# Icelk/fractal-renderer

Hardware: AMD Instinct MI355X
Metric: pixel_iterations_per_sec (higher is better)
Workload: dtype f64

## Files before the change

fractal-renderer_amd/_native.py:

```python
import ctypes as C
import os

PKG_DIR = os.path.dirname(os.path.abspath(__file__))
LIB_PATH = os.path.join(PKG_DIR, "libfractal_hip.so")

FR_OK, FR_ERR_INVALID_ARGUMENT, FR_ERR_BUFFER_TOO_SMALL, FR_ERR_NO_DEVICE, FR_ERR_HIP = 0, 1, 2, 3, 4
STATUS_NAMES = {
    1: "FR_ERR_INVALID_ARGUMENT",
    2: "FR_ERR_BUFFER_TOO_SMALL",
    3: "FR_ERR_NO_DEVICE",
    4: "FR_ERR_HIP",
    5: "FR_ERR_UNSUPPORTED_ALGO",
}


class FractalHipError(RuntimeError):
    def __init__(self, code, message):
        super().__init__("%s: %s" % (STATUS_NAMES.get(code, "fr_status %d" % code), message))
        self.code = code


class Imaginary(C.Structure):

    _fields_ = [("re", C.c_double), ("im", C.c_double)]
# ... 30 lines not shown
        ("limit", C.c_double),
        ("stable_limit", C.c_double),
        ("pos", Imaginary),
        ("scale", Imaginary),
        ("exposure", C.c_double),
        ("inside", C.c_uint8),
        ("smooth", C.c_uint8),
        ("primary_color", RGB),
        ("secondary_color", RGB),
        ("color_weight", C.c_double),
        ("julia_set", Imaginary),
    ]


class fr_render_opts(C.Structure):

    _fields_ = [
        ("size", C.c_uint32),
        ("tile", C.c_int32),
        ("loop_mode", C.c_int32),
        ("palette", C.c_int32),
        ("cycle_shortcut", C.c_int32),
        ("refill_minrun", C.c_int32),
        ("refill_quit16", C.c_int32),
        ("colour_filter", C.c_int32),
    ]


FR_MAX_DEVICES = 16
FR_GATHER_PEER_COPY, FR_GATHER_RCCL = 0, 1


class fr_multi_stats(C.Structure):
    _fields_ = [
        ("n_devices", C.c_uint32),
        ("kernels", C.c_uint32 * FR_MAX_DEVICES),
        ("kernel_ms", C.c_float * FR_MAX_DEVICES),
        ("rows", C.c_uint64 * FR_MAX_DEVICES),
        ("wall_ms", C.c_double),
        ("transfer_span_ms", C.c_float * FR_MAX_DEVICES),
        ("job_ms", C.c_double * FR_MAX_DEVICES),
        ("bytes_moved", C.c_uint64 * FR_MAX_DEVICES),
    ]


class fr_wide_centre(C.Structure):

    _fields_ = [("n_words", C.c_uint32), ("re", C.POINTER(C.c_uint64)), ("im", C.POINTER(C.c_uint64))]


FR_WIDE_MAX_WORDS = 16
FR_BLA_DEFAULT_BITS = 40
_OPTS = C.POINTER(fr_render_opts)
_WIDE = C.POINTER(fr_wide_centre)

PROTOTYPES = {
    "fr_abi_version": (C.c_int, []),
    "fr_build_id": (C.c_char_p, []),
    "fr_render_opts_init": (None, [_OPTS]),
    "fr_render_rows_rgb8_device_opts": (
        C.c_int,
        [C.POINTER(fr_config), C.c_int, C.c_uint32, C.c_uint32, C.c_void_p, C.c_size_t, C.c_void_p, _OPTS],
    ),
    "fr_render_rows_rgba8_device_opts": (
        C.c_int,
        [C.POINTER(fr_config), C.c_int, C.c_uint32, C.c_uint32, C.c_void_p, C.c_size_t, C.c_void_p, _OPTS],
    ),
    "fr_render_rows_rgb8_opts": (
        C.c_int, [C.POINTER(fr_config), C.c_int, C.c_uint32, C.c_uint32, C.c_void_p, C.c_size_t, _OPTS]),
    "fr_render_block_cyclic_range_rgb8_device_opts": (
        C.c_int,
        [C.POINTER(fr_config), C.c_int, C.c_uint32, C.c_uint32, C.c_uint32, C.c_uint32, C.c_int, C.c_void_p, C.c_size_t,
         C.c_void_p, C.POINTER(C.c_uint64), _OPTS],
    ),
    "fr_render_fern_rgb8": (C.c_int, [C.POINTER(fr_config), C.c_uint32, C.c_uint64, C.c_uint32, C.c_void_p, C.c_size_t]),
    "fr_init_devices": (C.c_int, [C.POINTER(C.c_int), C.c_int]),
    "fr_multi_device_count": (C.c_int, [C.POINTER(C.c_int)]),
    "fr_set_multi_root_share": (C.c_int, [C.c_int]),
    "fr_render_rgb8_multi": (C.c_int, [C.POINTER(fr_config), C.c_int, C.c_uint32, C.c_void_p, C.c_size_t]),
    "fr_render_rgb8_multi_device": (
        C.c_int, [C.POINTER(fr_config), C.c_int, C.c_uint32, C.c_int, C.c_void_p, C.c_size_t]),
    "fr_multi_last_stats": (C.c_int, [C.POINTER(fr_multi_stats)]),
    "fr_debug_rccl_selftest": (C.c_int, [C.c_size_t]),
    "fr_debug_rccl_probe": (C.c_int, []),
    "fr_set_dispatch_sampling": (C.c_int, [C.c_int]),
    "fr_debug_sample_view": (C.c_int, [C.POINTER(fr_config), C.c_int, C.POINTER(C.c_double)]),
    "fr_debug_view_choice": (C.c_int, [C.POINTER(fr_config), C.c_int, C.c_uint32, C.c_uint32, C.POINTER(C.c_int),
                                       C.POINTER(C.c_int), C.POINTER(C.c_uint32)]),
    "fr_debug_inject_multi_failure": (C.c_int, [C.c_int, C.c_int]),
    "fr_pin_host_buffer": (C.c_int, [C.c_void_p, C.c_size_t]),
    "fr_unpin_host_buffer": (C.c_int, [C.c_void_p]),
    "fr_last_kernel_name": (C.c_int, [C.c_char_p, C.c_size_t]),
    "fr_set_colour_filter": (C.c_int, [C.c_int]),
    "fr_init": (C.c_int, [C.c_int]),
    "fr_shutdown": (C.c_int, []),
    "fr_device_count": (C.c_int, [C.POINTER(C.c_int)]),
    "fr_device_name": (C.c_int, [C.c_char_p, C.c_size_t]),
    "fr_last_error": (C.c_char_p, []),
    "fr_config_new": (None, [C.POINTER(fr_config), C.c_uint32]),
    "fr_render_rgb8": (C.c_int, [C.POINTER(fr_config), C.c_void_p, C.c_size_t]),
    "fr_render_rows_rgb8": (C.c_int, [C.POINTER(fr_config), C.c_int, C.c_uint32, C.c_uint32, C.c_void_p, C.c_size_t]),
    "fr_render_rows_rgb8_device": (
        C.c_int,
        [C.POINTER(fr_config), C.c_int, C.c_uint32, C.c_uint32, C.c_void_p, C.c_size_t, C.c_void_p],
    ),
    "fr_render_rows_rgba8": (C.c_int, [C.POINTER(fr_config), C.c_int, C.c_uint32, C.c_uint32, C.c_void_p, C.c_size_t]),
    "fr_render_rows_rgba8_device": (
        C.c_int,
        [C.POINTER(fr_config), C.c_int, C.c_uint32, C.c_uint32, C.c_void_p, C.c_size_t, C.c_void_p],
    ),
    "fr_render_block_cyclic_rgb8_device": (
        C.c_int,
        [C.POINTER(fr_config), C.c_int, C.c_uint32, C.c_uint32, C.c_uint32, C.c_void_p, C.c_size_t, C.c_void_p,
         C.POINTER(C.c_uint64)],
    ),
    "fr_render_block_cyclic_range_rgb8_device": (
        C.c_int,
        [C.POINTER(fr_config), C.c_int, C.c_uint32, C.c_uint32, C.c_uint32, C.c_uint32, C.c_int, C.c_void_p, C.c_size_t,
         C.c_void_p, C.POINTER(C.c_uint64)],
    ),
    "fr_render_block_cyclic_rgb8": (
        C.c_int,
        [C.POINTER(fr_config), C.c_int, C.c_uint32, C.c_uint32, C.c_uint32, C.c_void_p, C.c_size_t,
         C.POINTER(C.c_uint64)],
    ),
    "fr_block_cyclic_rows": (C.c_uint64, [C.c_uint32, C.c_uint32, C.c_uint32, C.c_uint32]),
    "fr_pixel": (C.c_int, [C.POINTER(fr_config), C.c_uint32, C.c_uint32, C.POINTER(RGB)]),
    "fr_pixel_p": (C.c_int, [C.POINTER(fr_config), C.c_int, C.c_uint32, C.c_uint32, C.POINTER(RGB)]),
    "fr_recursive": (
        C.c_int,
        [C.c_uint32, Imaginary, Imaginary, C.c_double, C.POINTER(Imaginary), C.POINTER(C.c_uint32)],
    ),
    "fr_recursive_batch": (
        C.c_int,
        [C.c_uint32, C.c_void_p, C.c_void_p, C.c_size_t, C.c_double, C.c_int, C.c_void_p, C.c_void_p],
    ),
    "fr_escape_rows": (C.c_int, [C.POINTER(fr_config), C.c_int, C.c_uint32, C.c_uint32, C.c_void_p, C.c_void_p]),
    "fr_render_rows_dd": (
        C.c_int, [C.POINTER(fr_config), C.POINTER(Imaginary), C.c_uint32, C.c_uint32, C.c_int, C.c_void_p, C.c_size_t]),
    "fr_render_rows_dd_device": (
        C.c_int,
        [C.POINTER(fr_config), C.POINTER(Imaginary), C.c_uint32, C.c_uint32, C.c_int, C.c_void_p, C.c_size_t, C.c_void_p],
    ),
    "fr_escape_rows_dd": (
        C.c_int, [C.POINTER(fr_config), C.POINTER(Imaginary), C.c_uint32, C.c_uint32, C.c_void_p, C.c_void_p]),
    "fr_render_rows_pt": (
        C.c_int, [C.POINTER(fr_config), C.POINTER(Imaginary), C.c_uint32, C.c_uint32, C.c_int, C.c_void_p, C.c_size_t]),
    "fr_render_rows_pt_device": (
        C.c_int,
        [C.POINTER(fr_config), C.POINTER(Imaginary), C.c_uint32, C.c_uint32, C.c_int, C.c_void_p, C.c_size_t, C.c_void_p],
    ),
    "fr_escape_rows_pt": (
        C.c_int, [C.POINTER(fr_config), C.POINTER(Imaginary), C.c_uint32, C.c_uint32, C.c_void_p, C.c_void_p]),
    "fr_debug_reference_orbit": (
        C.c_int, [C.POINTER(fr_config), C.POINTER(Imaginary), C.c_int, C.c_void_p, C.c_size_t, C.POINTER(C.c_uint32)]),
    "fr_ss_workspace_bytes": (
        C.c_int, [C.POINTER(fr_config), C.c_uint32, C.c_uint32, C.c_uint32, C.POINTER(C.c_size_t), C.POINTER(C.c_size_t)]),
    "fr_render_rows_ss_device": (
        C.c_int,
        [C.POINTER(fr_config), C.c_int, C.POINTER(Imaginary), C.c_uint32, C.c_uint32, C.c_uint32, C.c_int, C.c_void_p,
         C.c_size_t, C.c_void_p, C.c_size_t, C.c_void_p, _OPTS],
    ),
    "fr_render_rows_ss": (
        C.c_int,
        [C.POINTER(fr_config), C.c_int, C.POINTER(Imaginary), C.c_uint32, C.c_uint32, C.c_uint32, C.c_int, C.c_void_p,
         C.c_size_t, _OPTS],
    ),
    "fr_box_filter_rgb8": (
        C.c_int, [C.c_void_p, C.c_uint32, C.c_uint32, C.c_uint32, C.c_int, C.c_void_p, C.c_size_t]),
    "fr_box_filter_rgb8_device": (
        C.c_int, [C.c_void_p, C.c_uint32, C.c_uint32, C.c_uint32, C.c_int, C.c_void_p, C.c_size_t, C.c_void_p]),
    "fr_colour_rgb8": (C.c_int, [C.POINTER(fr_config), C.c_void_p, C.c_void_p, C.c_size_t, C.c_void_p, C.c_size_t]),
    "fr_colour_rgb8_device": (
        C.c_int, [C.POINTER(fr_config), C.c_void_p, C.c_void_p, C.c_size_t, C.c_void_p, C.c_size_t, C.c_void_p]),
    "fr_escape_rows_device": (
        C.c_int,
        [C.POINTER(fr_config), C.c_int, C.POINTER(Imaginary), C.c_uint32, C.c_uint32, C.c_int, C.c_void_p, C.c_void_p,
         C.c_void_p, _OPTS],
    ),
    "fr_escape_extend_device": (
        C.c_int,
        [C.POINTER(fr_config), C.c_int, C.POINTER(Imaginary), C.c_uint32, C.c_uint32, C.c_uint32, C.c_int, C.c_void_p,
         C.c_void_p, C.c_void_p, _OPTS],
    ),
    "fr_escape_extend": (
        C.c_int,
        [C.POINTER(fr_config), C.c_int, C.POINTER(Imaginary), C.c_uint32, C.c_uint32, C.c_uint32, C.c_int, C.c_void_p,
         C.c_void_p],
    ),
    "fr_escape_rows_pt_state_device": (
        C.c_int,
        [C.POINTER(fr_config), C.POINTER(Imaginary), C.c_uint32, C.c_uint32, C.c_void_p, C.c_void_p, C.c_void_p, C.c_void_p,
         C.c_void_p],
    ),
    "fr_escape_extend_pt_device": (
        C.c_int,
        [C.POINTER(fr_config), C.POINTER(Imaginary), C.c_uint32, C.c_uint32, C.c_uint32, C.c_void_p, C.c_void_p, C.c_void_p,
         C.c_void_p, C.c_void_p],
    ),
    "fr_escape_rows_pt_state": (
        C.c_int,
        [C.POINTER(fr_config), C.POINTER(Imaginary), C.c_uint32, C.c_uint32, C.c_void_p, C.c_void_p, C.c_void_p, C.c_void_p],
    ),
    "fr_escape_extend_pt": (
        C.c_int,
        [C.POINTER(fr_config), C.POINTER(Imaginary), C.c_uint32, C.c_uint32, C.c_uint32, C.c_void_p, C.c_void_p, C.c_void_p,
         C.c_void_p],
    ),
    "fr_debug_pt_orbit_cache": (C.c_int, [C.POINTER(C.c_uint32)]),
    "fr_wide_from_double": (C.c_int, [C.c_double, C.c_void_p, C.c_uint32]),
    "fr_wide_add_double": (C.c_int, [C.c_void_p, C.c_uint32, C.c_double]),
    "fr_wide_to_double": (C.c_int, [C.c_void_p, C.c_uint32, C.POINTER(C.c_double), C.POINTER(C.c_double)]),
    "fr_wide_from_decimal": (C.c_int, [C.c_char_p, C.c_void_p, C.c_uint32]),
    "fr_render_rows_pt_wide": (
        C.c_int, [C.POINTER(fr_config), _WIDE, C.c_uint32, C.c_uint32, C.c_int, C.c_void_p, C.c_size_t]),
    "fr_render_rows_pt_wide_device": (
        C.c_int, [C.POINTER(fr_config), _WIDE, C.c_uint32, C.c_uint32, C.c_int, C.c_void_p, C.c_size_t, C.c_void_p]),
    "fr_escape_rows_pt_wide": (C.c_int, [C.POINTER(fr_config), _WIDE, C.c_uint32, C.c_uint32, C.c_void_p, C.c_void_p]),
    "fr_escape_rows_pt_wide_state_device": (
        C.c_int,
        [C.POINTER(fr_config), _WIDE, C.c_uint32, C.c_uint32, C.c_void_p, C.c_void_p, C.c_void_p, C.c_void_p, C.c_void_p],
    ),
    "fr_escape_extend_pt_wide_device": (
        C.c_int,
        [C.POINTER(fr_config), _WIDE, C.c_uint32, C.c_uint32, C.c_uint32, C.c_void_p, C.c_void_p, C.c_void_p, C.c_void_p,
         C.c_void_p],
    ),
    "fr_escape_rows_pt_wide_state": (
        C.c_int, [C.POINTER(fr_config), _WIDE, C.c_uint32, C.c_uint32, C.c_void_p, C.c_void_p, C.c_void_p, C.c_void_p]),
    "fr_escape_extend_pt_wide": (
        C.c_int,
        [C.POINTER(fr_config), _WIDE, C.c_uint32, C.c_uint32, C.c_uint32, C.c_void_p, C.c_void_p, C.c_void_p, C.c_void_p],
    ),
    "fr_debug_reference_orbit_wide": (
        C.c_int, [C.POINTER(fr_config), _WIDE, C.c_int, C.c_void_p, C.c_size_t, C.POINTER(C.c_uint32)]),
    "fr_render_rows_pt_bla": (
        C.c_int,
        [C.POINTER(fr_config), C.POINTER(Imaginary), _WIDE, C.c_int, C.c_uint32, C.c_uint32, C.c_int, C.c_void_p, C.c_size_t]),
    "fr_render_rows_pt_bla_device": (
        C.c_int,
        [C.POINTER(fr_config), C.POINTER(Imaginary), _WIDE, C.c_int, C.c_uint32, C.c_uint32, C.c_int, C.c_void_p, C.c_size_t,
         C.c_void_p],
    ),
    "fr_escape_rows_pt_bla": (
        C.c_int, [C.POINTER(fr_config), C.POINTER(Imaginary), _WIDE, C.c_int, C.c_uint32, C.c_uint32, C.c_void_p, C.c_void_p]),
    "fr_escape_rows_pt_bla_device": (
        C.c_int,
        [C.POINTER(fr_config), C.POINTER(Imaginary), _WIDE, C.c_int, C.c_uint32, C.c_uint32, C.c_void_p, C.c_void_p, C.c_void_p],
    ),
    "fr_debug_bla_table": (
        C.c_int,
        [C.POINTER(fr_config), C.POINTER(Imaginary), _WIDE, C.c_int, C.c_int, C.c_uint32, C.c_void_p, C.c_size_t,
         C.POINTER(C.c_uint32)],
    ),
    "fr_debug_bla_count": (
        C.c_int,
        [C.POINTER(fr_config), C.POINTER(Imaginary), _WIDE, C.c_int, C.c_uint32, C.c_uint32, C.POINTER(C.c_uint64),
         C.POINTER(C.c_uint64)],
    ),
    "fr_debug_bla_cache": (C.c_int, [C.POINTER(C.c_uint32)]),
    "fr_render_rows_pt_scaled": (
        C.c_int, [C.POINTER(fr_config), _WIDE, C.c_int, C.c_uint32, C.c_uint32, C.c_int, C.c_void_p, C.c_size_t]),
    "fr_render_rows_pt_scaled_device": (
        C.c_int, [C.POINTER(fr_config), _WIDE, C.c_int, C.c_uint32, C.c_uint32, C.c_int, C.c_void_p, C.c_size_t, C.c_void_p]),
    "fr_escape_rows_pt_scaled": (C.c_int, [C.POINTER(fr_config), _WIDE, C.c_int, C.c_uint32, C.c_uint32, C.c_void_p, C.c_void_p]),
    "fr_escape_rows_pt_scaled_device": (
        C.c_int, [C.POINTER(fr_config), _WIDE, C.c_int, C.c_uint32, C.c_uint32, C.c_void_p, C.c_void_p, C.c_void_p]),
    "fr_debug_bla_table_scaled": (
        C.c_int, [C.POINTER(fr_config), _WIDE, C.c_int, C.c_int, C.c_uint32, C.c_void_p, C.c_size_t, C.POINTER(C.c_uint32)]),
    "fr_debug_pt_scaled_count": (
        C.c_int, [C.POINTER(fr_config), _WIDE, C.c_int, C.c_uint32, C.c_uint32, C.POINTER(C.c_uint64), C.POINTER(C.c_uint64)]),
    "fr_escape_rows_pt_scaled_state_device": (
        C.c_int,
        [C.POINTER(fr_config), _WIDE, C.c_uint32, C.c_uint32, C.c_void_p, C.c_void_p, C.c_void_p, C.c_void_p, C.c_void_p],
    ),
    "fr_escape_extend_pt_scaled_device": (
        C.c_int,
        [C.POINTER(fr_config), _WIDE, C.c_uint32, C.c_uint32, C.c_uint32, C.c_void_p, C.c_void_p, C.c_void_p, C.c_void_p,
         C.c_void_p],
    ),
    "fr_escape_rows_pt_scaled_state": (
        C.c_int, [C.POINTER(fr_config), _WIDE, C.c_uint32, C.c_uint32, C.c_void_p, C.c_void_p, C.c_void_p, C.c_void_p]),
    "fr_escape_extend_pt_scaled": (
        C.c_int,
        [C.POINTER(fr_config), _WIDE, C.c_uint32, C.c_uint32, C.c_uint32, C.c_void_p, C.c_void_p, C.c_void_p, C.c_void_p],
    ),
    "fr_colour_rows_device": (
        C.c_int,
        [C.POINTER(fr_config), C.c_void_p, C.c_int, C.c_void_p, C.c_size_t, C.c_int, C.c_void_p, C.c_size_t, C.c_void_p],
    ),
    "fr_count_iterations": (
        C.c_int,
        [C.POINTER(fr_config), C.c_int, C.c_uint32, C.c_uint32, C.c_uint32, C.c_uint32, C.POINTER(C.c_uint64),
         C.POINTER(C.c_uint64)],
    ),
    "fr_set_profiling": (C.c_int, [C.c_int]),
    "fr_last_kernel_ms": (C.c_int, [C.POINTER(C.c_float)]),
    "fr_set_tile": (C.c_int, [C.c_int]),
    "fr_set_loop_mode": (C.c_int, [C.c_int]),
    "fr_debug_loop_plan": (C.c_int, [C.POINTER(fr_config), C.c_int, C.POINTER(C.c_uint32), C.POINTER(C.c_double),
                                     C.POINTER(C.c_uint32)]),
    "fr_debug_set_spec_maxlen": (C.c_int, [C.c_uint32]),
    "fr_debug_spec_maxlen": (C.c_int, [C.POINTER(fr_config), C.c_int, C.POINTER(C.c_uint32)]),
    "fr_set_palette": (C.c_int, [C.c_int]),
    "fr_set_cycle_shortcut": (C.c_int, [C.c_int]),
    "fr_set_refill_policy": (C.c_int, [C.c_int, C.c_int]),
    "fr_debug_math": (C.c_int, [C.c_int, C.c_void_p, C.c_void_p, C.c_size_t]),
    "fr_debug_set_queue_trace": (C.c_int, [C.c_void_p]),
    "fr_debug_set_two_pass_capacity": (C.c_int, [C.c_uint32]),
}

_lib = None


def load():
    global _lib
    if _lib is not None:
        return _lib
    if not os.path.exists(LIB_PATH):
        raise ImportError(
            "%s is missing — build it first (python -c 'import __graft_entry__ as g; g.build()'); "
            "this package has no CPU fallback" % LIB_PATH
        )
    lib = C.CDLL(LIB_PATH)
    for name, (restype, argtypes) in PROTOTYPES.items():
        fn = getattr(lib, name)
        fn.restype = restype
        fn.argtypes = argtypes
    _lib = lib
    return lib


def check(rc):
    if rc != FR_OK:
        msg = load().fr_last_error()
        raise FractalHipError(rc, msg.decode() if msg else "")
```

fractal-renderer_amd/build.py:

```python
import hashlib
import os
import shutil
import subprocess

PKG_DIR = os.path.dirname(os.path.abspath(__file__))
CSRC = os.path.join(PKG_DIR, "csrc")
LIB_PATH = os.path.join(PKG_DIR, "libfractal_hip.so")
ID_PATH = LIB_PATH + ".id"
KERNEL_SOURCES = ["fr_kernels.hip", "fr_bla.hip", "fr_scaled.hip"]
SOURCES = KERNEL_SOURCES + ["fr_dispatch.hip", "fr_api.hip", "fr_host.hip", "fr_multi.hip", "fr_fern.hip",
                            "fr_dd.hip", "fr_pt.hip", "fr_wide.hip", "fr_ss.hip"]
DEPS = SOURCES + ["fr_kernels.h", "fr_launch.h", "fr_ctx.h", "fr_wide.h", "fr_bla.h", "fr_math.h", "fr_colour.h", "fr_log2_table.inc",
                  os.path.join("..", "..", "include", "fractal_hip.h")]
HIPCC_FLAGS = [
    "--offload-arch=gfx950",
    "-O3",
    "-std=c++17",
    "-ffp-contract=off",
    "-fno-fast-math",
    "-fPIC",
    "-shared",
    "-Wall",
    "-Wextra",
    "-pthread",
]
LINK_FLAGS = ["-ldl"]


def find_hipcc():
    for cand in (os.environ.get("HIPCC"), "/opt/rocm/bin/hipcc", shutil.which("hipcc")):
        if cand and os.path.exists(cand):
            return cand
    raise RuntimeError("hipcc not found (set HIPCC or install ROCm under /opt/rocm)")


def source_id():
    h = hashlib.sha256()
    h.update(" ".join(HIPCC_FLAGS + LINK_FLAGS).encode())
    for d in DEPS:
        h.update(d.encode())
        with open(os.path.join(CSRC, d), "rb") as f:
            h.update(f.read())
    return h.hexdigest()[:16]


def built_id():
    try:
        with open(ID_PATH) as f:
            return f.read().strip()
    except OSError:
        return None


def is_stale():
    return not os.path.exists(LIB_PATH) or built_id() != source_id()


def build_extension(force=False, verbose=False):
    if not force and not is_stale():
        return LIB_PATH
    sid = source_id()
    cmd = ([find_hipcc()] + HIPCC_FLAGS + ['-DFR_BUILD_ID="%s"' % sid, "-o", LIB_PATH]
           + [os.path.join(CSRC, s) for s in SOURCES] + LINK_FLAGS)
    if verbose:
        print(" ".join(cmd))
    if os.path.exists(ID_PATH):
        os.remove(ID_PATH)
    subprocess.run(cmd, check=True, cwd=CSRC)
    with open(ID_PATH, "w") as f:
        f.write(sid + "\n")
    return LIB_PATH


if __name__ == "__main__":
    print(build_extension(force=True, verbose=True))
```

fractal-renderer_amd/csrc/fr_api.hip:

```cpp
#include <hip/hip_runtime.h>

#include <atomic>
#include <cmath>
#include <cstddef>
#include <cstdint>
#include <cstdio>
#include <cstdlib>
#include <cstring>
#include <mutex>
#include <shared_mutex>
#include <string>
#include <vector>

#include "fr_ctx.h"

static_assert(sizeof(fr_config) == 104 && offsetof(fr_config, limit) == 16 && offsetof(fr_config, inside) == 72 &&
                  offsetof(fr_config, primary_color) == 74 && offsetof(fr_config, color_weight) == 80 &&
                  offsetof(fr_config, julia_set) == 88,
              "fr_config must stay the #[repr(C)] image of calc::Config");
static_assert(sizeof(fr_render_opts) == 32, "fr_render_opts is part of the ABI");

namespace fr {

namespace {
// ... 1453 lines not shown
                         uint32_t from_iterations, double *d_z, uint32_t *d_iters, hipStream_t stream) {
    const Centre c{pos_lo, nullptr};
    fr_kparams p;
    rows_params(cfg, o, y0, y1, 0, p);
    int rc = prof_begin(stream);
    if (rc != FR_OK) return rc;
    const char *kname = "";
    if (precision == FR_PRECISION_DD) {
        HIP_TRY(fr_launch_escape_extend_dd(p, c.lo_re(), c.lo_im(), from_iterations, d_z, d_iters, stream, &kname));
    } else {
        plan_loop(cfg, precision, o, p);
        HIP_TRY(fr_launch_escape_extend(p, precision, from_iterations, d_z, d_iters, stream, &kname));
    }
    return prof_end(stream, kname);
}

int fr_escape_extend_device(const fr_config *cfg, int precision, const fr_imaginary *pos_lo, uint32_t y0, uint32_t y1,
                            uint32_t from_iterations, int z_width, void *d_z, void *d_iters, void *hip_stream,
                            const fr_render_opts *opts) {
    Opts o;
    bool work;
    int rc = check_extend(cfg, precision, pos_lo, y0, y1, from_iterations, z_width, d_z, d_iters, opts, o, &work);
    if (rc != FR_OK || !work) return rc;
    LifeShared ls;
    Ctx *ctx;
    rc = primary(&ctx);
    if (rc != FR_OK) return rc;
    return extend_launch(cfg, precision, pos_lo, o, y0, y1, from_iterations, static_cast<double *>(d_z),
                         static_cast<uint32_t *>(d_iters), static_cast<hipStream_t>(hip_stream));
}

int fr_escape_extend(const fr_config *cfg, int precision, const fr_imaginary *pos_lo, uint32_t y0, uint32_t y1,
                     uint32_t from_iterations, int z_width, double *z, uint32_t *iters) {
    Opts o;
    bool work;
    int rc = check_extend(cfg, precision, pos_lo, y0, y1, from_iterations, z_width, z, iters, nullptr, o, &work);
    if (rc != FR_OK || !work) return rc;
    const size_t npx = (size_t)cfg->width * (size_t)(y1 - y0);
    const size_t zb = npx * (size_t)z_width * sizeof(double), ib = npx * sizeof(uint32_t);
    return host_raw(z, zb, iters, ib, nullptr, nullptr, true, [&](Ctx &, double *d_z, uint32_t *d_iters, double *, uint32_t *, hipStream_t stream) {
        return extend_launch(cfg, precision, pos_lo, o, y0, y1, from_iterations, d_z, d_iters, stream);
    });
}

int fr_colour_rows_device(const fr_config *cfg, const void *d_z, int z_width, const void *d_iters, size_t n, int channels,
                          void *d_out, size_t out_len, void *hip_stream) {
    if (!cfg) return fail(FR_ERR_INVALID_ARGUMENT, "cfg is NULL");
    if (z_width != 2 && z_width != 4) return fail(FR_ERR_INVALID_ARGUMENT, "z_width must be 2 (re, im) or 4 (re.hi, re.lo, im.hi, im.lo)");
    const int rc = check_channels(channels);
    if (rc != FR_OK) return rc;
    if (n == 0) return FR_OK;
    if (!d_z || !d_iters || !d_out) return fail(FR_ERR_INVALID_ARGUMENT, "NULL array");
    if (n > SIZE_MAX / 4 || out_len < (size_t)channels * n) return fail(FR_ERR_BUFFER_TOO_SMALL, "out_len < channels*n");
    if ((reinterpret_cast<uintptr_t>(d_z) & 7u) || (reinterpret_cast<uintptr_t>(d_iters) & 3u))
        return fail(FR_ERR_INVALID_ARGUMENT, "d_z must be 8-byte aligned and d_iters 4-byte aligned");
    if (channels == 4 && (reinterpret_cast<uintptr_t>(d_out) & 3u))
        return fail(FR_ERR_INVALID_ARGUMENT, "RGBA8 output must be 4-byte aligned");
    fr_kparams p;
    fill_params(cfg, default_opts(), p);
    HIP_TRY(fr_launch_colour_rows(p, static_cast<const double *>(d_z), (uint32_t)z_width, static_cast<const uint32_t *>(d_iters), n,
                                  (uint32_t)channels, d_out, static_cast<hipStream_t>(hip_stream)));
    return FR_OK;
}

int fr_colour_rgb8(const fr_config *cfg, const double *z_re_im, const uint32_t *iters, size_t n, uint8_t *out,
                   size_t out_len) {
    if (!cfg) return fail(FR_ERR_INVALID_ARGUMENT, "cfg is NULL");
    if (n == 0) return FR_OK;
    if (!z_re_im || !iters || !out) return fail(FR_ERR_INVALID_ARGUMENT, "NULL array");
    if (out_len < 3 * n) return fail(FR_ERR_BUFFER_TOO_SMALL, "out_len < 3*n");
    LifeShared ls;
    Ctx *ctx;
    int rc = primary(&ctx);
    if (rc != FR_OK) return rc;
    std::lock_guard<std::mutex> lk(ctx->mu);
    rc = ctx->reserve(ctx->z, n * 2 * sizeof(double));
    if (rc == FR_OK) rc = ctx->reserve(ctx->iters, n * sizeof(uint32_t));
    if (rc == FR_OK) rc = ctx->reserve(ctx->rgb, 3 * n);
    if (rc != FR_OK) return rc;
    fr_kparams p;
    fill_params(cfg, default_opts(), p);
    HIP_TRY(hipMemcpyAsync(ctx->z.ptr, z_re_im, n * 2 * sizeof(double), hipMemcpyHostToDevice, ctx->stream));
    HIP_TRY(hipMemcpyAsync(ctx->iters.ptr, iters, n * sizeof(uint32_t), hipMemcpyHostToDevice, ctx->stream));
    HIP_TRY(fr_launch_colour(p, static_cast<const double *>(ctx->z.ptr), static_cast<const uint32_t *>(ctx->iters.ptr), n,
                             static_cast<uint8_t *>(ctx->rgb.ptr), ctx->stream));
    HIP_TRY(hipMemcpyAsync(out, ctx->rgb.ptr, 3 * n, hipMemcpyDeviceToHost, ctx->stream));
    HIP_TRY(hipStreamSynchronize(ctx->stream));
    return FR_OK;
}

int fr_colour_rgb8_device(const fr_config *cfg, const void *d_z_re_im, const void *d_iters, size_t n, void *d_out,
                          size_t out_len, void *hip_stream) {
    if (!cfg) return fail(FR_ERR_INVALID_ARGUMENT, "cfg is NULL");
    if (n == 0) return FR_OK;
    if (!d_z_re_im || !d_iters || !d_out) return fail(FR_ERR_INVALID_ARGUMENT, "NULL array");
    if (out_len < 3 * n) return fail(FR_ERR_BUFFER_TOO_SMALL, "out_len < 3*n");
    fr_kparams p;
    fill_params(cfg, default_opts(), p);
    HIP_TRY(fr_launch_colour(p, static_cast<const double *>(d_z_re_im), static_cast<const uint32_t *>(d_iters), n,
                             static_cast<uint8_t *>(d_out), static_cast<hipStream_t>(hip_stream)));
    return FR_OK;
}

int fr_count_iterations(const fr_config *cfg, int precision, uint32_t y0, uint32_t y1, uint32_t sx, uint32_t sy,
                        uint64_t *total, uint64_t *pixels) {
    int rc = check_rows(cfg, y0, y1);
    if (rc == FR_OK) rc = check_precision_or_deep(cfg, precision);
    if (rc != FR_OK) return rc;
    if (!total) return fail(FR_ERR_INVALID_ARGUMENT, "total is NULL");
    if (sx == 0) sx = 1;
    if (sy == 0) sy = 1;
    *total = 0;
    const Opts o = default_opts();
    fr_kparams p;
    fill_params(cfg, o, p);
    p.ncols = (uint32_t)(((uint64_t)cfg->width + sx - 1) / sx);
    p.x_stride = sx;
    const uint64_t yf = ((uint64_t)y0 + sy - 1) / sy * sy;
    p.nrows = yf < y1 ? (uint32_t)((y1 - 1 - yf) / sy + 1) : 0;
    p.y_first = (uint32_t)yf;
    p.block_rows = 1;
    p.y_stride = sy;
    if (pixels) *pixels = (uint64_t)p.ncols * p.nrows;
    if (p.ncols == 0 || p.nrows == 0) return FR_OK;
    LifeShared ls;
    Ctx *ctx;
    rc = primary(&ctx);
    if (rc != FR_OK) return rc;
    std::lock_guard<std::mutex> lk(ctx->mu);
    const size_t slot_bytes = sizeof(unsigned long long) * FR_COUNT_SLOTS;
    rc = ctx->reserve(ctx->misc, slot_bytes);
    if (rc != FR_OK) return rc;
    HIP_TRY(hipMemsetAsync(ctx->misc.ptr, 0, slot_bytes, ctx->stream));
    fr_kout ko{};
    ko.count = static_cast<unsigned long long *>(ctx->misc.ptr);
    if (precision == FR_PRECISION_DD) {
        HIP_TRY(fr_launch_escape_dd(p, 0.0, 0.0, FR_OUT_COUNT, ko, false, ctx->stream, nullptr));
    } else if (precision == FR_PRECISION_PT) {
        rc = launch_pt(*ctx, cfg, Centre{}, p, FR_OUT_COUNT, ko, ctx->stream, nullptr);
        if (rc != FR_OK) return rc;
    } else {
        plan_loop(cfg, precision, o, p);
        HIP_TRY(fr_launch_escape(p, precision, FR_OUT_COUNT, ko, o.tile, ctx->stream, nullptr));
    }
    std::vector<unsigned long long> host(FR_COUNT_SLOTS);
    HIP_TRY(hipMemcpyAsync(host.data(), ctx->misc.ptr, slot_bytes, hipMemcpyDeviceToHost, ctx->stream));
    HIP_TRY(hipStreamSynchronize(ctx->stream));
    unsigned long long sum = 0;
    for (unsigned long long v : host) sum += v;
    *total = sum;
    return FR_OK;
}

int fr_set_profiling(int enabled) {
    Profiling &pr = profiling();
    pr.enabled = enabled != 0;
    if (!enabled) {
        pr.have = false;
        if (pr.e0) {
            (void)hipEventDestroy(pr.e0);
            (void)hipEventDestroy(pr.e1);
            pr.e0 = pr.e1 = nullptr;
        }
    }
    return FR_OK;
}

int fr_last_kernel_ms(float *ms) {
    if (!ms) return fail(FR_ERR_INVALID_ARGUMENT, "ms is NULL");
    Profiling &pr = profiling();
    if (!pr.have) return fail(FR_ERR_INVALID_ARGUMENT, "no profiled kernel on this thread");
    HIP_TRY(hipEventSynchronize(pr.e1));
    HIP_TRY(hipEventElapsedTime(ms, pr.e0, pr.e1));
    return FR_OK;
}

int fr_last_kernel_name(char *buf, size_t buf_len) {
    if (!buf || buf_len == 0) return fail(FR_ERR_INVALID_ARGUMENT, "buf is NULL or empty");
    Profiling &pr = profiling();
    if (!pr.have) return fail(FR_ERR_INVALID_ARGUMENT, "no profiled kernel on this thread");
    snprintf(buf, buf_len, "%s", pr.kernel);
    return FR_OK;
}

int fr_set_tile(int tile) {
    if (!valid_tile(tile)) return fail(FR_ERR_INVALID_ARGUMENT, "tile must be 0, 1, 2, 4, 8, 9, 10 ... 16, 6401, 3202, 1604 or 808");
    g_tile.store(tile);
    return FR_OK;
}

int fr_set_refill_policy(int minrun, int quit16) {
    if (minrun < -1 || quit16 < -1 || quit16 == 0 || quit16 > 16)
        return fail(FR_ERR_INVALID_ARGUMENT, "minrun >= 0, 1 <= quit16 <= 16 (or -1: the kernel's default)");
    g_refill_minrun.store(minrun);
    g_refill_quit16.store(quit16);
    return FR_OK;
}

int fr_set_cycle_shortcut(int enabled) {
    g_cycle_shortcut.store(enabled ? 1 : 0);
    return FR_OK;
}

int fr_set_palette(int enabled) {
    g_palette_enabled.store(enabled ? 1 : 0);
    return FR_OK;
}

int fr_set_colour_filter(int enabled) {
    g_colour_filter.store(enabled == 2 ? 2 : enabled ? 1 : 0);
    return FR_OK;
}

int fr_set_loop_mode(int mode) {
    if (mode != -1 && mode != 0 && mode != 2 && mode != 4 && mode != 5)
        return fail(FR_ERR_INVALID_ARGUMENT, "loop mode must be -1 (auto), 0, 2, 4 or 5");
    g_loop_mode.store(mode);
    return FR_OK;
}

int fr_set_dispatch_sampling(int enabled) {
    g_dispatch_sampling.store(enabled ? 1 : 0);
    return FR_OK;
}

int fr_debug_sample_view(const fr_config *cfg, int precision, double out[8]) {
    if (!cfg || !out) return fail(FR_ERR_INVALID_ARGUMENT, "cfg or out is NULL");
    int rc = check_precision(precision);
    if (rc != FR_OK) return rc;
    LifeShared ls;
    Ctx *ctx;
    rc = primary(&ctx);
    if (rc != FR_OK) return rc;
    fr_kparams p;
    rows_params(cfg, default_opts(), 0, cfg->height, 0, p);
    if (p.ncols == 0 || p.nrows == 0) return fail(FR_ERR_INVALID_ARGUMENT, "empty image");
    double st[7];
    rc = sample_view(*ctx, p, precision, Ctx::kViewChoices, st);
    if (rc != FR_OK) return rc;
    for (int k = 0; k < 6; k++) out[k] = st[k];
    out[6] = st[1] > 0.0 ? st[0] / st[1] : 0.0;
    out[7] = st[6];
    return FR_OK;
}

int fr_debug_loop_plan(const fr_config *cfg, int precision, uint32_t *loop_mode, double *skip_t, uint32_t *spec_quiet) {
    if (!cfg || !loop_mode || !skip_t || !spec_quiet) return fail(FR_ERR_INVALID_ARGUMENT, "NULL argument");
    int rc = check_precision(precision);
    if (rc != FR_OK) return rc;
    const Opts o = default_opts();
    fr_kparams p;
    rows_params(cfg, o, 0, cfg->height, 0, p);
    plan_loop(cfg, precision, o, p);
    *loop_mode = p.loop_mode;
    *skip_t = p.skip_t;
    *spec_quiet = p.loop_spec;
    return FR_OK;
}

int fr_debug_view_choice(const fr_config *cfg, int precision, uint32_t y0, uint32_t y1, int *state, int *choice,
                         uint32_t *strip_tiles) {
    if (!cfg || !state || !choice || !strip_tiles) return fail(FR_ERR_INVALID_ARGUMENT, "NULL argument");
    int rc = check_rows(cfg, y0, y1);
    if (rc == FR_OK) rc = check_precision(precision);
    if (rc != FR_OK) return rc;
    LifeShared ls;
    Ctx *ctx;
    rc = primary(&ctx);
    if (rc != FR_OK) return rc;
    fr_kparams p;
    rows_params(cfg, default_opts(), y0, y1, 0, p);
    const uint64_t key = view_key(cfg, p, precision);
    *state = 0, *choice = -1, *strip_tiles = 0;
    std::lock_guard<std::mutex> lk(ctx->sample_mu);
    for (int k = 0; k < Ctx::kViewChoices; k++) {
        const Ctx::ViewChoice &v = ctx->view_choices[k];
        if (v.key != key || v.state == 0) continue;
        *state = v.state;
        if (v.state == 1 && __atomic_load_n(ctx->sample_result + 8 * k + 7, __ATOMIC_ACQUIRE) == key) *state = 3;
        *choice = v.two_pass;
        *strip_tiles = v.strip_tiles;
        break;
    }
    return FR_OK;
}

int fr_debug_set_spec_maxlen(uint32_t maxlen) {
    g_spec_maxlen.store(maxlen);
    return FR_OK;
}

int fr_debug_spec_maxlen(const fr_config *cfg, int precision, uint32_t *maxlen) {
    if (!cfg || !maxlen) return fail(FR_ERR_INVALID_ARGUMENT, "NULL argument");
    int rc = check_precision(precision);
    if (rc != FR_OK) return rc;
    const Opts o = default_opts();
    fr_kparams p;
    rows_params(cfg, o, 0, cfg->height, 0, p);
    plan_loop(cfg, precision, o, p);
    *maxlen = p.loop_spec_max;
    return FR_OK;
}

int fr_debug_set_queue_trace(void *d_trace) {
    g_queue_trace.store(static_cast<unsigned long long *>(d_trace));
    return FR_OK;
}

int fr_debug_set_two_pass_capacity(uint32_t entries_per_list) {
    g_two_pass_list_entries.store(entries_per_list);
    return FR_OK;
}

int fr_debug_math(int which, const double *in, double *out, size_t n) {
    if (n == 0) return FR_OK;
    if (!in || !out) return fail(FR_ERR_INVALID_ARGUMENT, "NULL array");
    LifeShared ls;
    Ctx *ctx;
    int rc = primary(&ctx);
    if (rc != FR_OK) return rc;
    std::lock_guard<std::mutex> lk(ctx->mu);
    rc = ctx->reserve(ctx->z, 2 * n * sizeof(double));
    if (rc != FR_OK) return rc;
    double *d_in = static_cast<double *>(ctx->z.ptr), *d_out = d_in + n;
    if (which == 4) {
        if (n < 2) return fail(FR_ERR_INVALID_ARGUMENT, "which == 4 needs n >= 2");
        HIP_TRY(fr_launch_nu_scan((uint32_t)in[0], (uint32_t)in[1], d_out, ctx->stream));
        HIP_TRY(hipMemcpyAsync(out, d_out, sizeof(double), hipMemcpyDeviceToHost, ctx->stream));
        HIP_TRY(hipStreamSynchronize(ctx->stream));
        return FR_OK;
    }
    if (which == 6) {
        if (n < 2) return fail(FR_ERR_INVALID_ARGUMENT, "which == 6 needs n >= 2");
        HIP_TRY(fr_launch_cast_scan((uint32_t)in[0], (uint32_t)in[1], d_out, ctx->stream));
        unsigned long long bad = 0;
        HIP_TRY(hipMemcpyAsync(&bad, d_out, sizeof bad, hipMemcpyDeviceToHost, ctx->stream));
        HIP_TRY(hipStreamSynchronize(ctx->stream));
        out[0] = (double)bad;
        return FR_OK;
    }
    HIP_TRY(hipMemcpyAsync(d_in, in, n * sizeof(double), hipMemcpyHostToDevice, ctx->stream));
    HIP_TRY(fr_launch_math_probe(which, d_in, d_out, n, ctx->stream));
    HIP_TRY(hipMemcpyAsync(out, d_out, n * sizeof(double), hipMemcpyDeviceToHost, ctx->stream));
    HIP_TRY(hipStreamSynchronize(ctx->stream));
    return FR_OK;
}

}
```

fractal-renderer_amd/csrc/fr_dispatch.hip:

```cpp
#include "fr_kernels.h"

#include <cmath>

#include "fr_launch.h"

namespace {

#define FR_KNAME(base, k) (precision == 1 ? base "<float, " k ">" : base "<double, " k ">")

const char *first_pass_name(const fr_kparams &p, int precision) {
    const bool spec = fr_first_pass_speculates(p);
#define FR_FIRST_NAMES(SUFFIX)                                                                                                       \
    (p.strip_tiles == 4                                                                                                              \
         ? (p.first_only ? FR_KNAME("escape_first_kernel", "4-tile strips in episodes, every tile finished in place" SUFFIX)         \
                         : FR_KNAME("escape_first_kernel + escape_second_kernel",                                                    \
                                    "4-tile strips, then persistent waves over the survivor lists" SUFFIX))                          \
         : (p.first_only ? FR_KNAME("escape_first_kernel", "7-tile strips in episodes, every tile finished in place" SUFFIX)         \
                         : FR_KNAME("escape_first_kernel + escape_second_kernel",                                                    \
                                    "7-tile strips, then persistent waves over the survivor lists" SUFFIX)))
    return spec ? FR_FIRST_NAMES("; speculative blocks in the later episodes") : FR_FIRST_NAMES("");
#undef FR_FIRST_NAMES
}

bool two_pass_ready(const fr_kparams &p, int mode) {
    return mode == FR_OUT_RGB && p.first_cap != 0 && (p.first_only || (p.surv_counts && p.work_counter));
}

hipError_t run_two_pass(const fr_kparams &p, int precision, int tile, const fr_kout &out, hipStream_t stream, const char *&name) {
    name = tile == 12   ? FR_KNAME("escape_first_v1_kernel + escape_queue_kernel", "round 2's first pass, then persistent waves over the survivor lists")
           : tile == 14 ? FR_KNAME("escape_first_kernel + escape_queue_kernel", "7-tile strips, then round 2's persistent waves over the survivor lists")
                        : first_pass_name(p, precision);
    if (p.ncols == 0 || p.nrows == 0) return hipSuccess;
    const hipError_t e = fr_launch_first_pass(p, precision, tile == 12, out, stream);
    if (e != hipSuccess) return e;
    if (p.first_only) return hipSuccess;
    if (p.debug_ablate & 2u) return hipSuccess;
    return fr_launch_queue(p, precision, 1, out, stream);
}

hipError_t run_strips(const fr_kparams &p, int precision, int mode, uint32_t k_len, const fr_kout &out, hipStream_t stream,
                      const char *&name) {
    const int k = k_len >= 7u ? 7 : k_len >= 4u ? 4 : k_len >= 2u ? 2 : 1;
    name = k == 7   ? FR_KNAME("escape_strip_kernel", "7 tiles")
           : k == 4 ? FR_KNAME("escape_strip_kernel", "4 tiles")
           : k == 2 ? FR_KNAME("escape_strip_kernel", "2 tiles")
                    : FR_KNAME("escape_strip_kernel", "1 tile");
    return fr_launch_strips(p, precision, mode, k, out, stream);
}

hipError_t run_refill(const fr_kparams &p, int precision, int mode, const fr_kout &out, hipStream_t stream, const char *&name) {
    name = FR_KNAME("escape_refill_kernel", "7x2-tile patches");
    return fr_launch_refill(p, precision, mode, out, stream);
}

hipError_t run_refill_or_strips(const fr_kparams &p, int precision, int mode, const fr_kout &out, hipStream_t stream,
                                const char *&name) {
    if (p.algo != 0 && p.algo != 2) return run_strips(p, precision, mode, 7u, out, stream, name);
    return run_refill(p, precision, mode, out, stream, name);
}

hipError_t launch_precision(const fr_kparams &p, int precision, int mode, const fr_kout &out, int tile, hipStream_t stream,
                            const char *&name) {
    if (p.out_in_place && tile > 16) tile = 0;
    switch (tile) {
    case 6401:
    case 3202:
    case 1604:
    case 808:
        name = tile == 6401   ? FR_KNAME("escape_kernel", "64x1")
               : tile == 3202 ? FR_KNAME("escape_kernel", "32x2")
               : tile == 1604 ? FR_KNAME("escape_kernel", "16x4")
                              : FR_KNAME("escape_kernel", "8x8");
        return fr_launch_tile(p, precision, mode, tile, out, stream);
    case 0: {
        const uint64_t tiles = (((uint64_t)p.ncols + 7) / 8) * (((uint64_t)p.nrows + 7) / 8);
        if (two_pass_ready(p, mode)) return run_two_pass(p, precision, 0, out, stream, name);
        if (tiles >= 262144 && ((p.algo == 2 && mode != FR_OUT_RGB) || p.cycle_shortcut)) return run_refill(p, precision, mode, out, stream, name);
        const uint32_t k_len = (mode == FR_OUT_RGB && p.strip_tiles) ? p.strip_tiles : tiles >= 524288 ? 7u : 1u;
        return run_strips(p, precision, mode, k_len, out, stream, name);
    }
    case 1:
    case 2:
    case 4:
    case 8:
        return run_strips(p, precision, mode, (uint32_t)tile, out, stream, name);
    case 13:
    case 16:
    case 12:
    case 14:
    case 15:
    case 11:
        if (two_pass_ready(p, mode)) return run_two_pass(p, precision, tile, out, stream, name);
        return run_refill_or_strips(p, precision, mode, out, stream, name);
    case 10:
        if (mode == FR_OUT_RGB && p.work_counter && fr_wants_work_queue(p, 10)) {
            name = FR_KNAME("escape_queue_kernel", "persistent waves, 64x32-px patches");
            return fr_launch_queue(p, precision, 0, out, stream);
        }
        [[fallthrough]];
    case 9:
        return run_refill_or_strips(p, precision, mode, out, stream, name);
    default:
        return hipErrorInvalidValue;
    }
}

}

hipError_t fr_launch_escape(const fr_kparams &p, int precision, int mode, const fr_kout &out, int tile,
                            hipStream_t stream, const char **kernel_name) {
    const char *name = "";
    const hipError_t e = launch_precision(p, precision, mode, out, tile, stream, name);
    if (kernel_name) *kernel_name = name;
    return e;
}

bool fr_wants_work_queue(const fr_kparams &p, int tile) {
    if (p.cycle_shortcut || (p.algo != 0 && p.algo != 2)) return false;
    if (p.loop_mode == 0 || p.iterations >= (1u << 24)) return false;
    return tile == 10;
}

bool fr_wants_two_pass(fr_kparams &p, int precision, int tile, int hint) {
    p.first_cap = 0;
    p.first_only = 0;
    if (p.cycle_shortcut || (p.algo != 0 && p.algo != 2)) return false;
    if (p.loop_mode == 0 || p.iterations >= (1u << 24)) return false;
    if (p.ncols == 0 || p.nrows == 0 || (uint64_t)p.ncols * p.nrows > 0xFFF00000ull) return false;
    if (p.algo == 2 && tile == 0) {
        const double lo = precision == 1 ? 0x1p-30 : 0x1p-300, hi = precision == 1 ? 0x1p30 : 0x1p400;
        const double jr = precision == 1 ? std::fabs((double)(float)p.julia_re) : std::fabs(p.julia_re);
        const double ji = precision == 1 ? std::fabs((double)(float)p.julia_im) : std::fabs(p.julia_im);
        if (!(jr >= lo && jr <= hi && ji >= lo && ji <= hi)) return false;
    }
    if (tile == 0) {
        const uint64_t tiles = (((uint64_t)p.ncols + 7) / 8) * (((uint64_t)p.nrows + 7) / 8);
        if (tiles < 262144 && hint < 1) return false;
        if (tiles < 4096) return false;
        if (hint == 0 || (hint < 0 && p.algo != 2)) return false;
        if (hint < 0 && p.iterations < 512u) return false;
        p.first_only = hint == 2 ? 1u : 0u;
    } else if (tile == 13 || tile == 16) {
        p.first_only = 1u;
    } else if (tile != 11 && tile != 12 && tile != 14 && tile != 15) {
        return false;
    }
    if (tile == 15 || tile == 16) p.strip_tiles = 4u;
    uint32_t k1 = p.two_pass_cap ? p.two_pass_cap : 64u;
    k1 = (k1 + 3u) & ~3u;
    if (k1 + 8u > p.iterations) return false;
    p.first_cap = k1;
    if (p.first_keep == 0 || p.first_keep > 64) p.first_keep = 48;
    return true;
}

fr_two_pass_layout fr_two_pass_bytes(const fr_kparams &p, int precision, uint32_t sub_capacity) {
    const size_t entries = (size_t)sub_capacity * FR_SURV_QUEUES;
    const size_t pair = precision == 1 ? 8 : 16;
    auto up = [](size_t v) { return (v + 255) & ~(size_t)255; };
    fr_two_pass_layout l{};
    l.z_off = 0;
    l.pos_off = up(entries * pair);
    l.cnt_off = l.pos_off + up(entries * 8);
    l.c_off = l.cnt_off + up(entries * 4);
    l.counts_off = l.c_off + (p.algo == 2 ? 0 : up(entries * pair));
    l.total = l.counts_off + FR_SURV_QUEUES * FR_SURV_COUNT_STRIDE * sizeof(uint32_t);
    return l;
}
```

fractal-renderer_amd/csrc/fr_kernels.h:

```cpp
#ifndef FR_KERNELS_H
#define FR_KERNELS_H

#include <hip/hip_runtime.h>
#include <stdint.h>

struct fr_kparams {
    uint32_t algo;
    uint32_t width, height;
    uint32_t iterations;
    double limit, stable_limit;
    double pos_re, pos_im, scale_re, scale_im;
    double exposure;
    double julia_re, julia_im;
    uint32_t inside, smooth;
    uint32_t prim[3], sec[3];
    double prim_f[3], sec_f[3];
    double iterations_f64, inv_iterations;
    uint32_t ncols, nrows;
    uint32_t x_first, x_stride;
    uint32_t block_rows, y_first, y_stride;
    uint32_t out_in_place;
    uint32_t out_rgba;
    uint32_t loop_mode;
    double skip_t;
    uint32_t loop_spec;
    uint32_t loop_spec_max;
    uint32_t first_no_spec;
    const uint32_t *palette;
    uint32_t palette_entries;
    uint32_t refill_minrun, refill_quit16;
    uint32_t queue_minrun, queue_want;
    uint32_t cycle_shortcut;
    uint32_t colour_filter;
    uint32_t *work_counter;
    double filt_k;
    double filt_d[3];
    uint32_t colour_filter32;
    float filt_k32;
    float filt_c32;
    float filt_d32[3];
    float prim32[3];
    float filt_lo32;
    uint32_t first_cap;
    uint32_t first_keep;
    uint32_t two_pass_cap;
    uint32_t first_only;
    uint32_t second_v1;
    uint32_t first_one_band;
    uint32_t strip_tiles;
    uint32_t debug_ablate;
    uint32_t surv_sub_capacity;
    void *surv_z;
    uint32_t *surv_pos;
    uint32_t *surv_cnt;
    void *surv_c;
    uint32_t *surv_counts;
};

constexpr uint32_t FR_SURV_QUEUES = 64;
constexpr uint32_t FR_SURV_COUNT_STRIDE = 32;
constexpr uint32_t FR_SURV_CHUNK = 64;

constexpr double FR_NU_BRACKET = 0x1p-18;

enum fr_out_mode {
    FR_OUT_RGB = 0,
    FR_OUT_ESCAPE = 1,
    FR_OUT_COUNT = 2
};

constexpr uint32_t FR_COUNT_SLOTS = 512;

struct fr_kout {
    uint8_t *rgb;
    double *z;
    uint32_t *iters;
    unsigned long long *count;
    unsigned long long *trace;
};

hipError_t fr_launch_escape(const fr_kparams &p, int precision, int mode, const fr_kout &out, int tile,
                            hipStream_t stream, const char **kernel_name);

hipError_t fr_launch_escape_dd(const fr_kparams &p, double pos_lo_re, double pos_lo_im, int mode, const fr_kout &out,
                               bool with_lo, hipStream_t stream, const char **kernel_name);

bool fr_wants_work_queue(const fr_kparams &p, int tile);

bool fr_wants_two_pass(fr_kparams &p, int precision, int tile, int hint = -1);
struct fr_two_pass_layout {
    size_t z_off, pos_off, cnt_off, c_off, counts_off, total;
};
fr_two_pass_layout fr_two_pass_bytes(const fr_kparams &p, int precision, uint32_t sub_capacity);

hipError_t fr_launch_view_sample(const fr_kparams &p, int precision, uint32_t side, uint32_t cap_s, uint32_t episode, uint32_t keep,
                                 unsigned long long *counters, unsigned long long *result, unsigned long long tag,
                                 hipStream_t stream);

hipError_t fr_launch_copy_out(const void *src, void *dst, size_t bytes, unsigned int *counter, unsigned long long *flag,
                              unsigned long long seq, hipStream_t stream);

constexpr uint32_t FR_MAX_PALETTE_ENTRIES = 1280;

hipError_t fr_launch_palette(const fr_kparams &p, uint32_t *palette, hipStream_t stream);

hipError_t fr_launch_colour(const fr_kparams &p, const double *z, const uint32_t *iters, size_t n, uint8_t *rgb,
                            hipStream_t stream);

hipError_t fr_launch_escape_extend(const fr_kparams &p, int precision, uint32_t from_iterations, double *z, uint32_t *iters,
                                   hipStream_t stream, const char **kernel_name);
hipError_t fr_launch_escape_extend_dd(const fr_kparams &p, double pos_lo_re, double pos_lo_im, uint32_t from_iterations,
                                      double *z, uint32_t *iters, hipStream_t stream, const char **kernel_name);

hipError_t fr_launch_colour_rows(const fr_kparams &p, const double *z, uint32_t z_width, const uint32_t *iters, size_t n,
                                 uint32_t channels, void *out, hipStream_t stream);

hipError_t fr_launch_box_filter(const void *src, uint32_t width, uint64_t rows, uint32_t s, uint32_t bpp, void *dst,
                                hipStream_t stream);

hipError_t fr_launch_recursive_batch(uint32_t iterations, const double *start, const double *c, size_t n,
                                     double limit, int precision, double *out_pos, uint32_t *out_iters,
                                     hipStream_t stream);

hipError_t fr_launch_math_probe(int which, const double *in, double *out, size_t n, hipStream_t stream);

hipError_t fr_launch_nu_scan(uint32_t lo_bits, uint32_t hi_bits, double *out, hipStream_t stream);

hipError_t fr_launch_cast_scan(uint32_t lo_bits, uint32_t hi_bits, double *out, hipStream_t stream);

#endif
```

fractal-renderer_amd/csrc/fr_kernels.hip:

```cpp
#include "fr_kernels.h"

#include <cmath>

#include <cstdlib>

#include "fr_launch.h"
#include "fr_math.h"

namespace {

#include "fr_colour.h"

constexpr int kWaves = 4;



#define FR_ORBIT_IT_R(SFX, S, D)                           \
    "v_add_" SFX " %[t], %[r2" S "], -%[i2" S "]\n"        \
    "v_add_" SFX " %[x], %[re" S "], %[re" S "]\n"         \
    "v_add_" SFX " %[re" D "], %[t], %[cre]\n"             \
    "v_mul_" SFX " %[x], %[x], %[im" S "]\n"               \
    "v_add_" SFX " %[im" D "], %[x], %[cim]\n"             \
    "v_mul_" SFX " %[r2" D "], %[re" D "], %[re" D "]\n"   \
    "v_mul_" SFX " %[i2" D "], %[im" D "], %[im" D "]\n"
// ... 99 lines not shown
    "s_mov_b32 %[sspec], %[n]\n"                                                   \
    "s_cmp_lt_u32 %[si], %[n]\n"                                                   \
    "s_cbranch_scc1 .Lmain_%=\n"                                                   \
    "s_branch .Ldone_%=\n"                                                         \
    ".LrbB_%=:\n" FR_ORBIT_SPEC_MOVS(MOV)                                          \
    ".LrbA_%=:\n"                                                                  \
    "s_lshl_b32 %[specq], %[specq], 1\n"                                           \
    "s_min_u32 %[specq], %[specq], 0x8000\n"                                       \
    "s_add_u32 %[sspec], %[si], %[specq]\n"                                        \
    "s_cselect_b32 %[sspec], -1, %[sspec]\n"                                       \
    "s_min_u32 %[sspec], %[sspec], %[n]\n"                                         \
    "s_branch .Lmain_%=\n"                                                         \
    FR_ORBIT_RECORD_A("R", "0") FR_ORBIT_RECORD_A("A", "0") FR_ORBIT_RECORD_A("B", "1") \
    FR_ORBIT_RECORD_A("C", "2") FR_ORBIT_RECORD_A("D", "3")                         \
    ".Ldone_%=:\n"                                                                 \
    "s_mov_b64 exec, %[sorig]\n"

template <typename T>
struct UBits {
    typedef uint32_t type;
};
template <>
struct UBits<double> {
    typedef uint64_t type;
};
template <typename T>
__device__ __forceinline__ typename UBits<T>::type uniform_bits(T v) {
    if constexpr (sizeof(T) == 8) {
        const uint64_t b = fr_bits_of(v);
        return (uint64_t)(uint32_t)__builtin_amdgcn_readfirstlane((uint32_t)b) |
               ((uint64_t)(uint32_t)__builtin_amdgcn_readfirstlane((uint32_t)(b >> 32)) << 32);
    } else {
        return (uint32_t)__builtin_amdgcn_readfirstlane(__builtin_bit_cast(uint32_t, v));
    }
}

struct EpisodeCtl {
    uint32_t thr, minrun;
};

template <typename T>
__device__ __forceinline__ uint32_t orbit_run(uint32_t iterations, T &re, T &im, T cre, T cim, T squared, T &r2,
                                              T &i2, EpisodeCtl ctl, uint32_t &completed, uint32_t spec_quiet = 0u) {
    uint32_t it;
    T t, x;
    T re1, im1, r21, i21;
    unsigned long long sorig, sprev, sdiff;
    uint32_t si, stmp, nrem, scnt, sspec;
    uint32_t specq = __builtin_amdgcn_readfirstlane(spec_quiet ? spec_quiet : 0xFFFFFFFFu);
    const uint32_t n = __builtin_amdgcn_readfirstlane(iterations);
    const uint32_t thr = __builtin_amdgcn_readfirstlane(ctl.thr), minrun = __builtin_amdgcn_readfirstlane(ctl.minrun);
#define FR_ORBIT_OPERANDS                                                                                          \
    : [re] "+v"(re), [im] "+v"(im), [r2] "+v"(r2), [i2] "+v"(i2), [it] "=&v"(it), [t] "=&v"(t), [x] "=&v"(x),      \
      [sorig] "=&s"(sorig), [sprev] "=&s"(sprev), [sdiff] "=&s"(sdiff), [si] "=&s"(si), [stmp] "=&s"(stmp),        \
      [nrem] "=&s"(nrem), [scnt] "=&s"(scnt), [re1] "=&v"(re1), [im1] "=&v"(im1), [r21] "=&v"(r21),                \
      [i21] "=&v"(i21), [sspec] "=&s"(sspec), [specq] "+&s"(specq)                                                 \
    : [cre] "v"(cre), [cim] "v"(cim), [lim2] "s"(lim2), [n] "s"(n), [thr] "s"(thr), [minrun] "s"(minrun)           \
    : "vcc", "scc"
    const auto lim2 = uniform_bits<T>(squared);
    if constexpr (sizeof(T) == 8)
        asm volatile(FR_ORBIT_ASM("f64", "v_mov_b64") FR_ORBIT_OPERANDS);
    else
        asm volatile(FR_ORBIT_ASM("f32", "v_mov_b32") FR_ORBIT_OPERANDS);
    (void)re1, (void)im1, (void)r21, (void)i21, (void)sspec;
    completed = si;
    return it;
}

template <typename T>
__device__ __forceinline__ uint32_t orbit(uint32_t iterations, T &re, T &im, T cre, T cim, T squared,
                                          T &r2, T &i2, uint32_t spec_quiet = 0u) {
    r2 = re * re;
    i2 = im * im;
    uint32_t completed;
    return orbit_run<T>(iterations, re, im, cre, cim, squared, r2, i2, EpisodeCtl{0, 0}, completed, spec_quiet);
}

#define FR_SC_IT_R(SFX, S, D)                              \
    "v_add_" SFX " %[t], %[A" S "], -%[B" S "]\n"          \
    "v_mul_" SFX " %[q], %[X" S "], %[Y" S "]\n"           \
    "v_fma_" SFX " %[X" D "], %[t], 0.5, %[c2re]\n"        \
    "v_add_" SFX " %[Y" D "], %[q], %[c2im]\n"             \
    "v_mul_" SFX " %[A" D "], %[X" D "], %[X" D "]\n"      \
    "v_mul_" SFX " %[B" D "], %[Y" D "], %[Y" D "]\n"
#define FR_SC_IT(SFX) FR_SC_IT_R(SFX, "", "")
#define FR_SC_IT_R5(SFX, S) FR_SC_IT_R(SFX, S, S) FR_SC_IT_R(SFX, S, S) FR_SC_IT_R(SFX, S, S) FR_SC_IT_R(SFX, S, S) FR_SC_IT_R(SFX, S, S)
#define FR_SC_ITS2(SFX) FR_SC_IT(SFX) FR_SC_IT(SFX)
#define FR_SC_ITS4(SFX) FR_SC_ITS2(SFX) FR_SC_ITS2(SFX)
#define FR_SC_BY_T_M(STMT)                                 \
    if constexpr (sizeof(T) == 8 && M == 4)                \
        STMT("f64", FR_SC_ITS4("f64"), "4.0");             \
    else if constexpr (sizeof(T) == 8)                     \
        STMT("f64", FR_SC_ITS2("f64"), "2.0");             \
    else if constexpr (M == 4)                             \
        STMT("f32", FR_SC_ITS4("f32"), "4.0");             \
    else                                                   \
        STMT("f32", FR_SC_ITS2("f32"), "2.0")

#define FR_SC_SPEC_ENTRY(MSTR)                                                     \
    "s_cmp_lt_u32 %[si], %[sspec]\n"                                               \
    "s_cbranch_scc1 .Lfast_%=\n"                                                   \
    "s_cmp_lt_u32 %[si], %[n]\n"                                                   \
    "s_cbranch_scc0 .Ldone_%=\n"                                                   \
    "s_sub_u32 %[stmp], %[n], %[si]\n"                                             \
    "s_cmp_ge_u32 %[stmp], " MSTR "\n"                                             \
    "s_cbranch_scc1 .Lspec_%=\n"                                                   \
    "s_mov_b32 %[sspec], %[n]\n"                                                   \
    "s_branch .Lfast_%=\n"
#define FR_SC_NOSPEC_ENTRY                                                         \
    "s_cmp_lt_u32 %[si], %[n]\n"                                                   \
    "s_cbranch_scc1 .Lfast_%=\n"                                                   \
    "s_branch .Ldone_%=\n"
#define FR_SC_SPEC_ARM                                                             \
    "s_add_u32 %[sspec], %[si], %[specq]\n"                                        \
    "s_cselect_b32 %[sspec], -1, %[sspec]\n"                                       \
    "s_min_u32 %[sspec], %[sspec], %[n]\n"
#define FR_SC_SPEC_BLOCK(SFX, MSTR, REST, TAG, S, D, RB, NEXT, EXIT)               \
    ".Lblk" TAG "_%=:\n" FR_SC_IT_R(SFX, S, D)                                     \
    "s_mov_b32 %[stmp], %[nrem]\n"                                                 \
    ".Lmid" TAG "_%=:\n" REST(SFX, D)                                              \
    "s_sub_u32 %[stmp], %[stmp], " MSTR "\n"                                       \
    "s_cmp_lt_u32 %[stmp], " MSTR "\n"                                             \
    "s_cbranch_scc1 .Ltst" TAG "_%=\n"                                             \
    FR_SC_IT_R(SFX, D, D)                                                          \
    "s_branch .Lmid" TAG "_%=\n"                                                   \
    ".Ltst" TAG "_%=:\n"                                                           \
    "v_add_" SFX " %[t], %[A" D "], %[B" D "]\n"                                   \
    "v_cmp_nge_" SFX " vcc, %[t4lim], %[t]\n"                                      \
    "s_cbranch_vccnz " RB "\n"                                                     \
    "s_add_u32 %[si], %[si], %[nrem]\n"                                            \
    "s_lshl_b32 %[nrem], %[nrem], 1\n"                                             \
    "s_min_u32 %[nrem], %[nrem], %[lcap]\n"                                        \
    "s_sub_u32 %[stmp], %[n], %[si]\n"                                             \
    ".Lfit" TAG "_%=:\n"                                                           \
    "s_cmp_le_u32 %[nrem], %[stmp]\n"                                              \
    "s_cbranch_scc1 " NEXT "\n"                                                    \
    "s_lshr_b32 %[nrem], %[nrem], 1\n"                                             \
    "s_cmp_ge_u32 %[nrem], " MSTR "\n"                                             \
    "s_cbranch_scc1 .Lfit" TAG "_%=\n"                                             \
    "s_branch " EXIT "\n"
#define FR_SC_SPEC_BODY(SFX, MOV, MSTR, REST)                                      \
    ".Lspec_%=:\n"                                                                 \
    "s_mov_b32 %[nrem], " MSTR "\n"                                                \
    FR_SC_SPEC_BLOCK(SFX, MSTR, REST, "A", "", "1", ".LrbA_%=", ".LblkB_%=", ".LexA_%=") \
    FR_SC_SPEC_BLOCK(SFX, MSTR, REST, "B", "1", "", ".LrbB_%=", ".LblkA_%=", ".Lspecout_%=") \
    ".LexA_%=:\n"                                                                  \
    MOV " %[X], %[X1]\n" MOV " %[Y], %[Y1]\n" MOV " %[A], %[A1]\n" MOV " %[B], %[B1]\n" \
    ".Lspecout_%=:\n"                                                              \
    "s_mov_b32 %[sspec], %[n]\n"                                                   \
    "s_cmp_lt_u32 %[si], %[n]\n"                                                   \
    "s_cbranch_scc1 .Lfast_%=\n"                                                   \
    "s_branch .Ldone_%=\n"                                                         \
    ".LrbB_%=:\n"                                                                  \
    MOV " %[X], %[X1]\n" MOV " %[Y], %[Y1]\n" MOV " %[A], %[A1]\n" MOV " %[B], %[B1]\n" \
    ".LrbA_%=:\n"                                                                  \
    "s_mov_b32 %[lcap], " MSTR "\n"                                                \
    "s_lshl_b32 %[specq], %[specq], 1\n"                                           \
    "s_min_u32 %[specq], %[specq], 0x8000\n"                                       \
    FR_SC_SPEC_ARM                                                                 \
    "s_branch .Lfast_%=\n"

#define FR_SC_CHECKED_STEP(SFX, TAG)               \
    FR_SC_IT(SFX)                                  \
    "v_add_" SFX " %[t], %[A], %[B]\n"             \
    "s_mov_b64 %[sprev], exec\n"                   \
    "v_cmpx_nlt_" SFX " %[lim4], %[t]\n"           \
    "s_xor_b64 %[sdiff], %[sprev], exec\n"         \
    "s_cbranch_scc1 .Lrec" TAG "_%=\n"             \
    ".Lcont" TAG "_%=:\n"

#define FR_SC_ASM(SFX, MSTR, FAST_ITS, SLOW_STEPS, SLOW_RECORDS, CYC_F, CYC_S, CYC_H, SP_INIT, SP_ARM, SP_ENTRY, SP_BODY)  \
    "s_mov_b64 %[sorig], exec\n"                                                   \
    "v_mov_b32 %[it], %[n]\n"                                                      \
    "s_mov_b32 %[si], 0\n"                                                         \
    SP_INIT                                                                        \
    "s_cbranch_execz .Ldone_%=\n"                                                  \
    "v_add_" SFX " %[t], %[A], %[B]\n"                                                         \
    "s_and_b32 %[nrem], %[n], " MSTR "-1\n"                                        \
    "s_cbranch_scc0 .Lmodesel_%=\n"                                                \
    ".Lrem_%=:\n" FR_SC_CHECKED_STEP(SFX, "R")                                     \
    "s_add_u32 %[si], %[si], 1\n"                                                  \
    "s_cmp_lt_u32 %[si], %[nrem]\n"                                                \
    "s_cbranch_scc1 .Lrem_%=\n"                                                    \
    ".Lmodesel_%=:\n"                                                              \
    "s_cmp_lt_u32 %[si], %[n]\n"                                                   \
    "s_cbranch_scc0 .Ldone_%=\n"                                                   \
    "v_cmp_lt_" SFX " vcc, %[t4lim], %[t]\n"                                       \
    "s_cbranch_vccnz .Lslow_%=\n"                                                  \
    ".Lfast_%=:\n" FAST_ITS                                                        \
    "v_add_" SFX " %[t], %[A], %[B]\n"                                             \
    "v_cmp_lt_" SFX " vcc, %[t4lim], %[t]\n"                                       \
    "s_add_u32 %[si], %[si], " MSTR "\n"                                           \
    "s_cbranch_vccnz .Lfastexit_%=\n"                                              \
    CYC_F                                                                          \
    SP_ENTRY                                                                       \
    ".Lfastexit_%=:\n"                                                             \
    SP_ARM                                                                         \
    "s_mov_b64 %[sprev], exec\n"                                                   \
    "v_cmpx_nlt_" SFX " %[lim4], %[t]\n"                                           \
    "s_xor_b64 %[sdiff], %[sprev], exec\n"                                         \
    "s_cbranch_scc0 .Lfxnorec_%=\n"                                                \
    "s_sub_u32 %[stmp], %[si], 1\n"                                                \
    "s_mov_b64 %[sprev], exec\n"                                                   \
    "s_mov_b64 exec, %[sdiff]\n"                                                   \
    "v_mov_b32 %[it], %[stmp]\n"                                                   \
    "s_mov_b64 exec, %[sprev]\n"                                                   \
    "s_cbranch_execz .Ldone_%=\n"                                                  \
    "s_bcnt1_i32_b64 %[scnt], exec\n"                                              \
    "s_cmp_gt_u32 %[scnt], %[thr]\n"                                               \
    "s_cbranch_scc1 .Lfxnorec_%=\n"                                                \
    "s_cmp_lt_u32 %[si], %[minrun]\n"                                              \
    "s_cbranch_scc0 .Ldone_%=\n"                                                   \
    ".Lfxnorec_%=:\n"                                                              \
    "s_cmp_lt_u32 %[si], %[n]\n"                                                   \
    "s_cbranch_scc0 .Ldone_%=\n"                                                   \
    ".Lslow_%=:\n" SLOW_STEPS                                                      \
    "s_add_u32 %[si], %[si], " MSTR "\n"                                           \
    "s_cmp_lt_u32 %[si], %[n]\n"                                                   \
    "s_cbranch_scc0 .Ldone_%=\n"                                                   \
    CYC_S                                                                          \
    "v_cmp_lt_" SFX " vcc, %[t4lim], %[t]\n"                                       \
    "s_cbranch_vccnz .Lslow_%=\n"                                                  \
    SP_ARM                                                                         \
    "s_branch .Lfast_%=\n"                                                         \
    FR_ORBIT_RECORD("R", "0") SLOW_RECORDS CYC_H SP_BODY                           \
    ".Ldone_%=:\n"                                                                 \
    "s_mov_b64 exec, %[sorig]\n"

#define FR_SC_CYC_CHECK(EQ, TAG)                   \
    EQ " %[scyc], %[X], %[Xs]\n"                   \
    EQ " vcc, %[Y], %[Ys]\n"                       \
    "s_and_b64 %[scyc], %[scyc], vcc\n"            \
    "s_cbranch_scc1 .Lcyc" TAG "_%=\n"             \
    ".Lcyccont" TAG "_%=:\n"                       \
    "s_cmp_ge_u32 %[si], %[snext]\n"               \
    "s_cbranch_scc1 .Lsave" TAG "_%=\n"            \
    ".Lsavecont" TAG "_%=:\n"

#define FR_SC_CYC_SAVE(MOV, TAG)                   \
    ".Lsave" TAG "_%=:\n"                          \
    MOV " %[Xs], %[X]\n"                           \
    MOV " %[Ys], %[Y]\n"                           \
    "v_mov_b32 %[vsaved], %[si]\n"                 \
    "s_lshl_b32 %[snext], %[snext], 1\n"           \
    "s_branch .Lsavecont" TAG "_%=\n"

#define FR_SC_CYC_HANDLER(TAG)                     \
    ".Lcyc" TAG "_%=:\n"                           \
    "s_or_b32 %[stmp], %[si], 0x80000000\n"        \
    "s_mov_b64 %[sprev], exec\n"                   \
    "s_mov_b64 exec, %[scyc]\n"                    \
    "v_mov_b32 %[it], %[stmp]\n"                   \
    "s_andn2_b64 exec, %[sprev], %[scyc]\n"        \
    "s_cbranch_execz .Ldone_%=\n"                  \
    "s_bcnt1_i32_b64 %[scnt], exec\n"              \
    "s_cmp_gt_u32 %[scnt], %[thr]\n"               \
    "s_cbranch_scc1 .Lcyccont" TAG "_%=\n"         \
    "s_cmp_lt_u32 %[si], %[minrun]\n"              \
    "s_cbranch_scc1 .Lcyccont" TAG "_%=\n"         \
    "s_branch .Ldone_%=\n"

#define FR_SC_ASM_M4_(SFX, CYC_F, CYC_S, CYC_H, SP_INIT, SP_ARM, SP_ENTRY, SP_BODY)                 \
    FR_SC_ASM(SFX, "4", FR_SC_ITS4(SFX),                    \
              FR_SC_CHECKED_STEP(SFX, "A") FR_SC_CHECKED_STEP(SFX, "B") FR_SC_CHECKED_STEP(SFX, "C") \
                  FR_SC_CHECKED_STEP(SFX, "D"),                                                     \
              FR_ORBIT_RECORD("A", "0") FR_ORBIT_RECORD("B", "1") FR_ORBIT_RECORD("C", "2")         \
                  FR_ORBIT_RECORD("D", "3"),                                                        \
              CYC_F, CYC_S, CYC_H, SP_INIT, SP_ARM, SP_ENTRY, SP_BODY)
#define FR_SC_ASM_M2_(SFX, CYC_F, CYC_S, CYC_H)                                            \
    FR_SC_ASM(SFX, "2", FR_SC_ITS2(SFX),                                        \
              FR_SC_CHECKED_STEP(SFX, "A") FR_SC_CHECKED_STEP(SFX, "B"),                    \
              FR_ORBIT_RECORD("A", "0") FR_ORBIT_RECORD("B", "1"), CYC_F, CYC_S, CYC_H, "", "", FR_SC_NOSPEC_ENTRY, "")
#define FR_SC_ASM_M4(SFX) FR_SC_ASM_M4_(SFX, "", "", "", "", "", FR_SC_NOSPEC_ENTRY, "")
#define FR_SC_ASM_M2(SFX) FR_SC_ASM_M2_(SFX, "", "", "")
#define FR_SC_ASM_M4_SPEC(SFX, MOV)                                                                 \
    FR_SC_ASM_M4_(SFX, "", "", "", "s_min_u32 %[sspec], %[specq], %[n]\n" "s_max_u32 %[lcap], %[lcap], " FR_SPEC_MSTR "\n", FR_SC_SPEC_ARM, FR_SC_SPEC_ENTRY(FR_SPEC_MSTR), \
                  FR_SC_SPEC_BODY(SFX, MOV, FR_SPEC_MSTR, FR_SC_SPEC_REST))
#define FR_SC_CYC_HANDLERS(MOV) \
    FR_SC_CYC_HANDLER("F") FR_SC_CYC_HANDLER("S") FR_SC_CYC_SAVE(MOV, "F") FR_SC_CYC_SAVE(MOV, "S")
#define FR_SC_ASM_M4_CYC(SFX, EQ, MOV) \
    FR_SC_ASM_M4_(SFX, FR_SC_CYC_CHECK(EQ, "F"), FR_SC_CYC_CHECK(EQ, "S"), FR_SC_CYC_HANDLERS(MOV), "", "", FR_SC_NOSPEC_ENTRY, "")
#define FR_SC_ASM_M2_CYC(SFX, EQ, MOV) \
    FR_SC_ASM_M2_(SFX, FR_SC_CYC_CHECK(EQ, "F"), FR_SC_CYC_CHECK(EQ, "S"), FR_SC_CYC_HANDLERS(MOV))

template <typename T>
struct ScalableRange;
template <>
struct ScalableRange<double> {
    static constexpr double lo = 0x1p-300, hi = 0x1p400;
};
template <>
struct ScalableRange<float> {
    static constexpr float lo = 0x1p-30f, hi = 0x1p30f;
};

template <typename T>
__device__ __forceinline__ bool lane_is_scalable(T re0, T im0, T cre, T cim) {
    constexpr T lo = ScalableRange<T>::lo, hi = ScalableRange<T>::hi;
    auto c_ok = [=](T v) { return __builtin_fabs(v) >= lo && __builtin_fabs(v) <= hi; };
    auto s_ok = [=](T v) { return v == (T)0 || c_ok(v); };
    return c_ok(cre) && c_ok(cim) && s_ok(re0) && s_ok(im0);
}

template <typename T, int M, bool CYC>
__device__ __forceinline__ uint32_t orbit_scaled_run(uint32_t iterations, T &X, T &Y, T &A, T &B, T c2re, T c2im,
                                                     T squared, T skip_t, EpisodeCtl ctl, uint32_t &completed,
                                                     T *pXs = nullptr, T *pYs = nullptr,
                                                     uint32_t *saved_index = nullptr, uint32_t spec_quiet = 0u,
                                                     uint32_t spec_maxlen = 0u) {
    uint32_t it;
    T t, q;
    T X1, Y1, A1, B1;
    uint32_t sspec;
    uint32_t specq = __builtin_amdgcn_readfirstlane(spec_quiet ? spec_quiet : 0xFFFFFFFFu);
    uint32_t lcap = __builtin_amdgcn_readfirstlane(spec_maxlen);
    T Xs = CYC ? *pXs : T(0), Ys = CYC ? *pYs : T(0);
    uint32_t vsaved = 0xFFFFFFFFu;
    uint32_t snext = 32u;
    unsigned long long sorig, sprev, sdiff, scyc;
    uint32_t si, stmp, nrem, scnt;
    const uint32_t n = __builtin_amdgcn_readfirstlane(iterations);
    const uint32_t thr = __builtin_amdgcn_readfirstlane(ctl.thr), minrun = __builtin_amdgcn_readfirstlane(ctl.minrun);
    const T lim4_v = (T)4 * squared, t4_v = (T)4 * skip_t;
#define FR_SC_OUTPUTS                                                                                           \
    [X] "+v"(X), [Y] "+v"(Y), [A] "+v"(A), [B] "+v"(B), [it] "=&v"(it), [t] "=&v"(t), [q] "=&v"(q),             \
        [sorig] "=&s"(sorig), [sprev] "=&s"(sprev), [sdiff] "=&s"(sdiff), [si] "=&s"(si), [stmp] "=&s"(stmp),   \
        [nrem] "=&s"(nrem), [scnt] "=&s"(scnt)
#define FR_SC_INPUTS                                                                                            \
    [c2re] "v"(c2re), [c2im] "v"(c2im), [lim4] "s"(lim4), [t4lim] "s"(t4lim), [n] "s"(n), [thr] "s"(thr),       \
        [minrun] "s"(minrun)
#define FR_SC_OPERANDS : FR_SC_OUTPUTS : FR_SC_INPUTS : "vcc", "scc"
#define FR_SC_OPERANDS_SPEC                                                                                     \
    : FR_SC_OUTPUTS, [X1] "=&v"(X1), [Y1] "=&v"(Y1), [A1] "=&v"(A1), [B1] "=&v"(B1), [sspec] "=&s"(sspec),      \
      [specq] "+&s"(specq), [lcap] "+&s"(lcap)                                                                  \
    : FR_SC_INPUTS                                                                                              \
    : "vcc", "scc"
#define FR_SC_OPERANDS_CYC                                                                                      \
    : FR_SC_OUTPUTS, [scyc] "=&s"(scyc), [Xs] "+v"(Xs), [Ys] "+v"(Ys), [vsaved] "+v"(vsaved), [snext] "+s"(snext) \
    : FR_SC_INPUTS                                                                                              \
    : "vcc", "scc"
    const auto lim4 = uniform_bits<T>(lim4_v), t4lim = uniform_bits<T>(t4_v);
    if constexpr (sizeof(T) == 8) {
        if constexpr (M == 4 && CYC)
            asm volatile(FR_SC_ASM_M4_CYC("f64", "v_cmp_eq_u64", "v_mov_b64") FR_SC_OPERANDS_CYC);
        else if constexpr (M == 4)
            asm volatile(FR_SC_ASM_M4_SPEC("f64", "v_mov_b64") FR_SC_OPERANDS_SPEC);
        else if constexpr (CYC)
            asm volatile(FR_SC_ASM_M2_CYC("f64", "v_cmp_eq_u64", "v_mov_b64") FR_SC_OPERANDS_CYC);
        else
            asm volatile(FR_SC_ASM_M2("f64") FR_SC_OPERANDS);
    } else {
        if constexpr (M == 4 && CYC)
            asm volatile(FR_SC_ASM_M4_CYC("f32", "v_cmp_eq_u32", "v_mov_b32") FR_SC_OPERANDS_CYC);
        else if constexpr (M == 4)
            asm volatile(FR_SC_ASM_M4_SPEC("f32", "v_mov_b32") FR_SC_OPERANDS_SPEC);
        else if constexpr (CYC)
            asm volatile(FR_SC_ASM_M2_CYC("f32", "v_cmp_eq_u32", "v_mov_b32") FR_SC_OPERANDS_CYC);
        else
            asm volatile(FR_SC_ASM_M2("f32") FR_SC_OPERANDS);
    }
    (void)scyc;
    (void)snext;
    (void)X1, (void)Y1, (void)A1, (void)B1, (void)sspec, (void)specq, (void)lcap;
    if constexpr (CYC) {
        *pXs = Xs;
        *pYs = Ys;
        *saved_index = vsaved;
    }
    completed = si;
    return it;
}

template <typename T, int M>
__device__ __forceinline__ uint32_t orbit_scaled(uint32_t iterations, T &re, T &im, T cre, T cim, T squared,
                                                 T skip_t, T &r2, T &i2, uint32_t spec_quiet = 0u, uint32_t spec_maxlen = 0u) {
    T X = re + re, Y = im + im, A = X * X, B = Y * Y;
    uint32_t completed;
    const uint32_t it = orbit_scaled_run<T, M, false>(iterations, X, Y, A, B, cre + cre, cim + cim, squared, skip_t,
                                               EpisodeCtl{0, 0}, completed, nullptr, nullptr, nullptr, spec_quiet, spec_maxlen);
    re = X * (T)0.5;
    im = Y * (T)0.5;
    r2 = re * re;
    i2 = im * im;
    return it;
}

template <typename T>
__device__ __forceinline__ uint32_t orbit_auto(uint32_t loop_mode, uint32_t iterations, T &re, T &im, T cre, T cim,
                                               T squared, T skip_t, T &r2, T &i2, int strip_scalable = -1,
                                               uint32_t spec_quiet = 0u, uint32_t spec_maxlen = 0u) {
    if (loop_mode != 0 && strip_scalable != 0) {
        bool all_ok = strip_scalable == 1;
        if (strip_scalable < 0) all_ok = __ballot(!lane_is_scalable<T>(re, im, cre, cim)) == 0ull;
        if (all_ok) {
            if (loop_mode == 4) return orbit_scaled<T, 4>(iterations, re, im, cre, cim, squared, skip_t, r2, i2, spec_quiet, spec_maxlen);
            return orbit_scaled<T, 2>(iterations, re, im, cre, cim, squared, skip_t, r2, i2);
        }
    }
    return orbit<T>(iterations, re, im, cre, cim, squared, r2, i2, spec_quiet);
}

__device__ __forceinline__ double coord_to_space(double coord, double max, double offset, double pos,
                                                 double scale) {
    return ((coord / max) - offset) / scale + pos;
}

__device__ __forceinline__ void store_pixel(uint32_t ncols, uint32_t out_rgba, uint8_t *base, uint32_t row, uint32_t col,
                                            const uint8_t rgb[3]) {
    const uint64_t k = (uint64_t)row * ncols + col;
    if (out_rgba) {
        reinterpret_cast<uint32_t *>(base)[k] =
            (uint32_t)rgb[0] | ((uint32_t)rgb[1] << 8) | ((uint32_t)rgb[2] << 16) | 0xFF000000u;
    } else {
        uint8_t *o = base + 3ull * k;
        o[0] = rgb[0];
        o[1] = rgb[1];
        o[2] = rgb[2];
    }
}
__device__ __forceinline__ void store_pixel(const fr_kparams &p, uint8_t *base, uint32_t row, uint32_t col, const uint8_t rgb[3]) {
    store_pixel(p.ncols, p.out_rgba, base, row, col, rgb);
}

typedef const __attribute__((address_space(4))) fr_kparams *KArgs;
#define FR_COLD_PARAMS(NAME)                                                          \
    KArgs NAME = (KArgs)__builtin_amdgcn_kernarg_segment_ptr();  \
    asm volatile("" : "+s"(NAME))

__device__ __forceinline__ unsigned long long ballot64(bool b) { return __builtin_amdgcn_ballot_w64(b); }

__device__ __forceinline__ bool lane_in(unsigned long long m) { return __builtin_amdgcn_inverse_ballot_w64(m); }

struct Filter32 {
    float lo, k, c, p0, p1, p2;
};
__device__ __forceinline__ uint32_t cvt_pk_u8_at(float v, uint32_t acc, int K) {
    return __builtin_amdgcn_cvt_pk_u8_f32(v, (uint32_t)K, acc);
}
__device__ __forceinline__ bool colour_fast32(const Filter32 &f, float d32, float itp1, uint32_t &lo) {
    const float l1 = __builtin_amdgcn_logf(d32);
    const float nu32 = __builtin_amdgcn_logf(l1 * 0.25f);
    const float m = (itp1 - nu32) * f.k;
    const float w = __builtin_fmaf(__builtin_fabsf(m), 0x1p-20f, f.c);
    const float ml = m - w, mh = m + w;
    lo = cvt_pk_u8_at(__builtin_fmaf(f.p2, ml, -0.5f), cvt_pk_u8_at(__builtin_fmaf(f.p1, ml, -0.5f), cvt_pk_u8_at(__builtin_fmaf(f.p0, ml, -0.5f), 0u, 0), 1), 2);
    const uint32_t hi = cvt_pk_u8_at(__builtin_fmaf(f.p2, mh, -0.5f), cvt_pk_u8_at(__builtin_fmaf(f.p1, mh, -0.5f), cvt_pk_u8_at(__builtin_fmaf(f.p0, mh, -0.5f), 0u, 0), 1), 2);
    return lo == hi;
}

__device__ __forceinline__ void store_packed(uint8_t *base, uint32_t off, uint32_t packed, uint32_t bpp) {
    if (bpp == 4u) {
        const uint32_t v = packed | 0xFF000000u;
        asm volatile("s_nop 4\n\tglobal_store_dword %0, %1, %2" : : "v"(off), "v"(v), "s"(base) : "memory");
    } else {
        asm volatile("s_nop 4\n\tglobal_store_short %0, %1, %2\n\tglobal_store_byte_d16_hi %0, %1, %2 offset:2" : : "v"(off), "v"(packed), "s"(base) : "memory");
    }
}

struct TileOut {
    uint8_t *base;
    uint32_t lane_off, bpp;
    bool narrow, fast_colour;
};

template <typename T>
__device__ __forceinline__ uint32_t colour_packed(bool valid, bool fast_colour, T re, T im, T r2, T i2, uint32_t iters,
                                                  const double *lds_tab, const uint32_t *palette) {
    uint32_t packed = 0;
    unsigned long long todo = ballot64(valid);
    if (fast_colour) {
        Filter32 f;
        {
            FR_COLD_PARAMS(kp);
            f.lo = kp->filt_lo32, f.k = kp->filt_k32, f.c = kp->filt_c32;
            f.p0 = kp->prim32[0], f.p1 = kp->prim32[2], f.p2 = kp->prim32[1];
        }
        float d32;
        if constexpr (sizeof(T) == 8)
            d32 = (float)(r2 + i2);
        else
            d32 = r2 + i2;
        const unsigned long long outside = ballot64(valid && d32 >= f.lo);
        if (outside != 0ull) {
            uint32_t pk;
            const bool decided = colour_fast32(f, d32, (float)(iters + 1u), pk);
            const bool ok = lane_in(outside) && d32 <= 0x1.ffffep119f && decided;
            packed = ok ? pk : 0u;
            todo &= ~ballot64(ok);
        }
    }
    if (todo != 0ull) {
        bool inside_done = false;
        if (lane_in(todo)) {
            double dist;
            if constexpr (sizeof(T) == 8) {
                dist = (double)(r2 + i2);
            } else {
                const double zre = (double)re, zim = (double)im;
                dist = zre * zre + zim * zim;
            }
            FR_COLD_PARAMS(kp);
            inside_done = !(dist > kp->stable_limit);
            if (inside_done && kp->inside)
                packed = sat_u8_dev(kp->sec_f[0] * dist) | (sat_u8_dev(kp->sec_f[2] * dist) << 8) | (sat_u8_dev(kp->sec_f[1] * dist) << 16);
        }
        todo &= ~ballot64(inside_done);
    }
    if (todo != 0ull) {
        if (lane_in(todo)) {
            FR_COLD_PARAMS(kp);
            const ColourConsts cc = make_colour_consts(*kp);
            uint8_t rgb[3];
            colour_pixel<T>(cc, re, im, r2, i2, iters, lds_tab, palette, rgb);
            packed = (uint32_t)rgb[0] | ((uint32_t)rgb[1] << 8) | ((uint32_t)rgb[2] << 16);
        }
    }
    return packed;
}

template <typename T, int MODE>
__device__ __forceinline__ void render_pixel(const fr_kparams &p, const fr_kout &out, const double *s_tab,
                                             const uint32_t *s_pal, double sre, double sim, bool valid,
                                             uint32_t cx, uint32_t r, uint32_t lane, uint32_t r_out,
                                             int strip_scalable = -1, const TileOut *to = nullptr) {
    double zre = 0.0, zim = 0.0;
    T tre = 0, tim = 0, tr2 = 0, ti2 = 0;
    uint32_t iters = 0;
    const bool escape_algo = p.algo == 0  || p.algo == 2 ;
    if (valid && escape_algo) {
        const double cre = p.algo == 0 ? sre : p.julia_re;
        const double cim = p.algo == 0 ? sim : p.julia_im;
        if constexpr (sizeof(T) == 8) {
            tre = sre;
            tim = sim;
            iters = orbit_auto<double>(p.loop_mode, p.iterations, tre, tim, cre, cim, p.limit * p.limit, p.skip_t,
                                       tr2, ti2, strip_scalable, p.loop_spec, p.loop_spec_max);
            zre = tre;
            zim = tim;
        } else {
            tre = (float)sre, tim = (float)sim;
            const float lim = (float)p.limit;
            iters = orbit_auto<float>(p.loop_mode, p.iterations, tre, tim, (float)cre, (float)cim, lim * lim,
                                      (float)p.skip_t, tr2, ti2, strip_scalable, p.loop_spec, p.loop_spec_max);
            zre = (double)tre;
            zim = (double)tim;
        }
    }

    if constexpr (MODE == FR_OUT_RGB) {
        if (to != nullptr) {
            uint32_t packed = 0;
            if (escape_algo) packed = colour_packed<T>(valid, to->fast_colour, tre, tim, tr2, ti2, iters, s_tab, s_pal);
            if (valid) {
                if (to->narrow) {
                    store_packed(to->base, to->lane_off, packed, to->bpp);
                } else {
                    const uint8_t rgb[3] = {(uint8_t)packed, (uint8_t)(packed >> 8), (uint8_t)(packed >> 16)};
                    store_pixel(p, out.rgb, r_out, cx, rgb);
                }
            }
        } else if (valid) {
            uint8_t rgb[3] = {0, 0, 0};
            if (escape_algo) {
                const ColourConsts cc = make_colour_consts(p);
                colour_pixel<T>(cc, tre, tim, tr2, ti2, iters, s_tab, s_pal, rgb);
            }
            store_pixel(p, out.rgb, r_out, cx, rgb);
        }
    } else if constexpr (MODE == FR_OUT_ESCAPE) {
        if (valid) {
            const uint64_t k = (uint64_t)r * p.ncols + cx;
            if (out.z) {
                out.z[2 * k] = zre;
                out.z[2 * k + 1] = zim;
            }
            if (out.iters) out.iters[k] = iters;
        }
    } else {
        unsigned long long n = 0;
        if (valid && escape_algo) n = iters < p.iterations ? (unsigned long long)iters + 1ull : p.iterations;
        for (int off = 32; off > 0; off >>= 1) n += __shfl_down(n, off, 64);
        if (lane == 0 && n) atomicAdd(out.count + ((blockIdx.x + 131u * blockIdx.y) % FR_COUNT_SLOTS), n);
    }
}

template <typename T, int TW, int TH, int WX, int WY, int MODE>
__global__ __launch_bounds__(64 * kWaves) void escape_kernel(const fr_kparams p, const fr_kout out) {
    static_assert(TW * TH == 64 && WX * WY == kWaves, "one lane per pixel, 4 waves per workgroup");
    constexpr int BW = TW * WX, BH = TH * WY;
    __shared__ double s_tab[FR_LOG2_N * 3];
    __shared__ double s_re[BW];
    __shared__ double s_im[BH];

    const uint32_t tid = threadIdx.x;
    const uint32_t tiles_x = (p.ncols + BW - 1) / BW;
    const uint32_t bx = blockIdx.x % tiles_x, by = blockIdx.x / tiles_x;
    const uint32_t col0 = bx * BW, row0 = by * BH;

    if (MODE == FR_OUT_RGB) {
        const double *gt = &g_log2_tab[0][0];
        for (uint32_t k = tid; k < FR_LOG2_N * 3; k += 64 * kWaves) s_tab[k] = gt[k];
    }
    if (tid < BW + BH) {
        const double width = (double)p.width, height = (double)p.height;
        if (tid < BW) {
            const uint32_t x = p.x_first + (col0 + tid) * p.x_stride;
            s_re[tid] = coord_to_space((double)x, height, (width / height) / 2.0, p.pos_re, p.scale_re);
        } else {
            const uint32_t r = row0 + (tid - BW);
            const uint32_t y = p.y_first + (r / p.block_rows) * p.y_stride + r % p.block_rows;
            s_im[tid - BW] = coord_to_space((double)y, height, 0.5, p.pos_im, p.scale_im);
        }
    }
    __syncthreads();

    const uint32_t wave = tid >> 6, lane = tid & 63;
    const uint32_t lx = (wave % WX) * TW + lane % TW;
    const uint32_t ly = (wave / WX) * TH + lane / TW;
    const uint32_t cx = col0 + lx, r = row0 + ly;
    const bool valid = cx < p.ncols && r < p.nrows;
    render_pixel<T, MODE>(p, out, s_tab, nullptr, s_re[lx], s_im[ly], valid, cx, r, lane, r);
}

template <typename T>
__device__ __forceinline__ bool coords_admissible(bool julia, double julia_re, double julia_im, double coord, bool relevant) {
    constexpr T lo = ScalableRange<T>::lo, hi = ScalableRange<T>::hi;
    const T v = (T)coord;
    const T av = __builtin_fabs(v);
    const bool in_range = av >= lo && av <= hi;
    bool lane_ok;
    if (julia) {
        const T jr = __builtin_fabs((T)julia_re), ji = __builtin_fabs((T)julia_im);
        lane_ok = (v == (T)0 || in_range) && jr >= lo && jr <= hi && ji >= lo && ji <= hi;
    } else {
        lane_ok = in_range;
    }
    return __ballot(relevant && !lane_ok) == 0ull;
}
template <typename T>
__device__ __forceinline__ bool coords_admissible(const fr_kparams &p, double coord, bool relevant) {
    return coords_admissible<T>(p.algo == 2, p.julia_re, p.julia_im, coord, relevant);
}

template <typename T>
__device__ __forceinline__ bool strip_is_scalable(const fr_kparams &p, double coord_lane, uint32_t tile0, uint32_t row0,
                                                  uint32_t lane) {
    const bool relevant = lane >= 56 ? (row0 + (lane - 56) < p.nrows) : (tile0 * 8u + lane < p.ncols);
    return coords_admissible<T>(p, coord_lane, relevant);
}


template <typename T, int MODE, int kStripTiles>
__global__ __launch_bounds__(64) void escape_strip_kernel(const fr_kparams p, const fr_kout out) {
    __shared__ double s_tab[(FR_LOG2_N * 3 * 8 > FR_MAX_PALETTE_ENTRIES * 4 ? FR_LOG2_N * 3 * 8 : FR_MAX_PALETTE_ENTRIES * 4) / 8];
    const uint32_t tid = threadIdx.x;
    const uint32_t *s_pal = nullptr;
    if (MODE == FR_OUT_RGB) {
        if (p.palette != nullptr) {
            uint32_t *dst = reinterpret_cast<uint32_t *>(s_tab);
            for (uint32_t k = tid; k < p.palette_entries; k += 64) dst[k] = p.palette[k];
            s_pal = dst;
        } else if (p.smooth) {
            const double *gt = &g_log2_tab[0][0];
            for (uint32_t k = tid; k < FR_LOG2_N * 3; k += 64) s_tab[k] = gt[k];
        }
        __syncthreads();
    }
    const uint32_t lane = tid;
    const uint32_t row0 = (blockIdx.y + gridDim.y * blockIdx.z) * 8u;
    if (row0 >= p.nrows) return;
    const uint32_t lx = lane & 7u, ly = lane >> 3;
    const uint32_t r = row0 + ly;
    const double width = (double)p.width, height = (double)p.height;

    static_assert(kStripTiles <= 7, "lanes 56-63 are the row lanes");
    const bool row_lane = lane >= 56;
    const uint32_t tile0 = blockIdx.x * kStripTiles;
    uint32_t coord_u;
    if (row_lane) {
        const uint32_t rr = row0 + (lane - 56);
        coord_u = p.y_first + (rr / p.block_rows) * p.y_stride + rr % p.block_rows;
    } else {
        coord_u = p.x_first + (tile0 * 8u + lane) * p.x_stride;
    }
    const double coord_lane = coord_to_space((double)coord_u, height, row_lane ? 0.5 : (width / height) / 2.0,
                                             row_lane ? p.pos_im : p.pos_re, row_lane ? p.scale_im : p.scale_re);
    const double sim = __shfl(coord_lane, 56 + ly, 64);
    uint32_t out_row0 = row0;
    if (p.out_in_place) out_row0 = p.y_first + (row0 / p.block_rows) * p.y_stride + row0 % p.block_rows;
    const uint32_t r_out = out_row0 + ly;
    const int strip_scalable = (p.loop_mode != 0 && strip_is_scalable<T>(p, coord_lane, tile0, row0, lane)) ? 1 : 0;
    TileOut to;
    to.bpp = p.out_rgba ? 4u : 3u;
    to.narrow = (uint64_t)p.ncols * to.bpp * 8u <= 0xFFFFFFFFull;
    to.lane_off = ly * (p.ncols * to.bpp) + lx * to.bpp;
    to.fast_colour = p.colour_filter32 && p.smooth && p.palette == nullptr;
    uint8_t *const strip_base = MODE == FR_OUT_RGB ? out.rgb + ((uint64_t)out_row0 * p.ncols + (uint64_t)tile0 * 8u) * to.bpp : nullptr;

    for (int k = 0; k < kStripTiles; k++) {
        const uint32_t col0 = (tile0 + k) * 8u;
        if (col0 >= p.ncols) break;
        const double sre = __shfl(coord_lane, k * 8 + lx, 64);
        const uint32_t cx = col0 + lx;
        const bool valid = cx < p.ncols && r < p.nrows;
        to.base = strip_base + (size_t)((uint32_t)k * 8u * to.bpp);
        render_pixel<T, MODE>(p, out, s_tab, s_pal, sre, sim, valid, cx, r, lane, r_out, strip_scalable, MODE == FR_OUT_RGB ? &to : nullptr);
    }
}

__device__ __forceinline__ uint32_t wave_max_u32(uint32_t v) {
    for (int off = 32; off > 0; off >>= 1) {
        const uint32_t o = __shfl_xor(v, off, 64);
        v = o > v ? o : v;
    }
    return v;
}

template <typename T>
struct Pair;
template <>
struct Pair<float> {
    typedef float2 type;
};
template <>
struct Pair<double> {
    typedef double2 type;
};

template <typename T>
__device__ __forceinline__ bool coord_is_scalable(bool julia, double coord) {
    constexpr T lo = ScalableRange<T>::lo, hi = ScalableRange<T>::hi;
    const T v = (T)coord;
    const T av = __builtin_fabs(v);
    const bool in_range = av >= lo && av <= hi;
    return julia ? (v == (T)0 || in_range) : in_range;
}

template <typename T, int M, int kStripTiles, int kBands>
__global__ __launch_bounds__(64) void escape_first_v1_kernel(const fr_kparams p, const fr_kout out) {
    __shared__ uint32_t s_palette[FR_MAX_PALETTE_ENTRIES];
    const double *const s_tab = &g_log2_tab[0][0];
    typedef typename Pair<T>::type T2;
    static_assert(kStripTiles <= 8 && kBands <= 8, "one column / one row coordinate per lane");
    const uint32_t lane = threadIdx.x;
    const uint32_t lx = lane & 7u, ly = lane >> 3;
    const uint32_t *s_pal = nullptr;
    uint32_t row0, tile0, ncols, nrows, bpp, lane_pitch;
    double cols, rows;
    bool cols_scalable;
    unsigned long long bad_rows;
    bool narrow;
    {
        FR_COLD_PARAMS(kp);
        const auto &P = *kp;
        if (P.palette != nullptr) {
            const uint32_t n = P.palette_entries;
            const uint32_t *src = P.palette;
            for (uint32_t k = lane; k < n; k += 64) s_palette[k] = src[k];
            s_pal = s_palette;
            __syncthreads();
        }
        row0 = (blockIdx.y + gridDim.y * blockIdx.z) * (8u * kBands);
        nrows = P.nrows, ncols = P.ncols;
        if (row0 >= nrows) return;
        const double width = (double)P.width, height = (double)P.height;
        tile0 = blockIdx.x * kStripTiles;
        const uint32_t block_rows = P.block_rows;
        const uint32_t x = P.x_first + (tile0 * 8u + lane) * P.x_stride;
        cols = coord_to_space((double)x, height, (width / height) / 2.0, P.pos_re, P.scale_re);
        const uint32_t rr = row0 + lane;
        const uint32_t y = P.y_first + (rr / block_rows) * P.y_stride + rr % block_rows;
        rows = coord_to_space((double)y, height, 0.5, P.pos_im, P.scale_im);
        bpp = P.out_rgba ? 4u : 3u;
        narrow = (uint64_t)ncols * bpp * 8u <= 0xFFFFFFFFull;
        lane_pitch = ly * (ncols * bpp) + lx * bpp;
        const bool is_julia = P.algo == 2;
        bool c_ok = true;
        if (is_julia) {
            constexpr T lo = ScalableRange<T>::lo, hi = ScalableRange<T>::hi;
            const T jr = __builtin_fabs((T)P.julia_re), ji = __builtin_fabs((T)P.julia_im);
            c_ok = jr >= lo && jr <= hi && ji >= lo && ji <= hi;
        }
        const bool col_relevant = lane < 8u * kStripTiles && tile0 * 8u + lane < ncols;
        const bool row_relevant = lane < 8u * kBands && rr < nrows;
        cols_scalable = c_ok && __ballot(col_relevant && !coord_is_scalable<T>(is_julia, cols)) == 0ull;
        bad_rows = __ballot(row_relevant && !coord_is_scalable<T>(is_julia, rows));
    }
    const uint32_t k1 = p.first_cap, cap = p.iterations, keep = p.first_keep;
    const bool julia = p.algo == 2;
    const T jre = (T)p.julia_re, jim = (T)p.julia_im;
    const T squared = sizeof(T) == 8 ? (T)(p.limit * p.limit) : (T)((float)p.limit * (float)p.limit);
    const T skip_t = (T)p.skip_t;

  for (int band = 0; band < kBands; band++) {
    const uint32_t rb = row0 + 8u * (uint32_t)band;
    if (rb >= nrows) break;
    const double sim = __shfl(rows, band * 8 + (int)ly, 64);
    const bool strip_scalable = cols_scalable && ((bad_rows >> (8 * band)) & 0xFFull) == 0ull;
    uint32_t out_row0 = rb;
    {
        FR_COLD_PARAMS(kp);
        if (kp->out_in_place) out_row0 = kp->y_first + (rb / kp->block_rows) * kp->y_stride + rb % kp->block_rows;
    }
    const uint32_t r_out = out_row0 + ly;
    uint8_t *const strip_base = out.rgb + ((uint64_t)out_row0 * ncols + (uint64_t)tile0 * 8u) * bpp;
    const uint32_t off_lane = lane_pitch;
    const uint32_t r = rb + ly;
    const uint32_t list = (blockIdx.x + 5u * (rb >> 3)) & (FR_SURV_QUEUES - 1u);

    for (int k = 0; k < kStripTiles; k++) {
        const uint32_t col0 = (tile0 + k) * 8u;
        if (col0 >= ncols) break;
        const double sre = __shfl(cols, k * 8 + (int)lx, 64);
        const uint32_t cx = col0 + lx;
        const bool valid = cx < ncols && r < nrows;
        T re = (T)sre, im = (T)sim, r2 = 0, i2 = 0;
        const T cre = julia ? jre : re, cim = julia ? jim : im;
        uint32_t iters = 0, start = 0;
        bool slow = valid;
        bool handed_over = false;
        if (strip_scalable) {
            slow = false;
            bool running = valid;
            uint32_t done = 0, len = k1;
            unsigned long long sm;
            for (;;) {
                const uint32_t n = cap - done < len ? cap - done : len;
                if (running) {
                    const uint32_t it = orbit_scaled<T, M>(n, re, im, cre, cim, squared, skip_t, r2, i2);
                    if (it < n) iters = done + it, running = false;
                }
                done += n;
                sm = __ballot(running);
                if (sm == 0ull) break;
                if (done == cap) {
                    if (running) iters = cap;
                    sm = 0ull;
                    break;
                }
                if ((uint32_t)__builtin_popcountll(sm) < keep) break;
                if (done >= 8u * k1 && len < 8u * k1) len += len;
            }
            if (sm != 0ull) {
                FR_COLD_PARAMS(kp);
                const uint32_t sub_cap = kp->surv_sub_capacity;
                uint32_t base = 0;
                if (lane == 0) base = atomicAdd(kp->surv_counts + list * FR_SURV_COUNT_STRIDE, (uint32_t)__builtin_popcountll(sm));
                base = __builtin_amdgcn_readfirstlane(base);
                const uint32_t slot = base + __builtin_amdgcn_mbcnt_hi((uint32_t)(sm >> 32), __builtin_amdgcn_mbcnt_lo((uint32_t)sm, 0u));
                if (running) {
                    if (slot < sub_cap) {
                        const size_t e = (size_t)list * sub_cap + slot;
                        T2 zz;
                        zz.x = re, zz.y = im;
                        static_cast<T2 *>(kp->surv_z)[e] = zz;
                        reinterpret_cast<uint2 *>(kp->surv_pos)[e] = make_uint2(cx, r_out);
                        kp->surv_cnt[e] = done;
                        if (!julia) {
                            T2 cc2;
                            cc2.x = cre, cc2.y = cim;
                            static_cast<T2 *>(kp->surv_c)[e] = cc2;
                        }
                        handed_over = true;
                    } else {
                        slow = true, start = done;
                    }
                }
            }
        }
        if (__ballot(slow) != 0ull && slow) {
            const uint32_t rest = cap - start;
            const uint32_t more = orbit<T>(rest, re, im, cre, cim, squared, r2, i2);
            iters = more < rest ? start + more : cap;
        }
        if (valid && !handed_over) {
            FR_COLD_PARAMS(kp);
            const ColourConsts cc = make_colour_consts(*kp);
            uint8_t rgb[3];
            colour_pixel<T>(cc, re, im, r2, i2, iters, s_tab, s_pal, rgb);
            if (narrow) {
                uint8_t *o = strip_base + (size_t)((uint32_t)k * 8u * bpp) + (size_t)off_lane;
                if (bpp == 4u) {
                    *reinterpret_cast<uint32_t *>(o) = (uint32_t)rgb[0] | ((uint32_t)rgb[1] << 8) | ((uint32_t)rgb[2] << 16) | 0xFF000000u;
                } else {
                    o[0] = rgb[0];
                    o[1] = rgb[1];
                    o[2] = rgb[2];
                }
            } else {
                store_pixel(kp->ncols, kp->out_rgba, out.rgb, r_out, cx, rgb);
            }
        }
    }
  }
}

#define FR_FB_ASM(SFX, BLOCK_ITS, MSHIFT)              \
    "s_mov_b64 %[sorig], exec\n"                       \
    "s_mov_b64 exec, %[mask]\n"                        \
    ".Lfb_%=:\n" BLOCK_ITS                             \
    "v_add_" SFX " %[t], %[A], %[B]\n"                 \
    "s_mov_b64 %[sprev], exec\n"                       \
    "v_cmpx_nlt_" SFX " %[t4lim], %[t]\n"              \
    "s_xor_b64 %[sdiff], %[sprev], exec\n"             \
    "s_cbranch_scc1 .Lfbr_%=\n"                        \
    ".Lfbc_%=:\n"                                      \
    "s_sub_u32 %[k], %[k], 1\n"                        \
    "s_cbranch_scc0 .Lfb_%=\n"                         \
    "s_branch .Lfbd_%=\n"                              \
    ".Lfbr_%=:\n"                                      \
    "s_sub_u32 %[stmp], %[n0], %[k]\n"                 \
    "s_lshl_b32 %[stmp], %[stmp], " MSHIFT "\n"        \
    "s_add_u32 %[stmp], %[stmp], %[base]\n"            \
    "s_mov_b64 %[sprev], exec\n"                       \
    "s_mov_b64 exec, %[sdiff]\n"                       \
    "v_cvt_f32_u32 %[cnt], %[stmp]\n"                  \
    "s_mov_b64 exec, %[sprev]\n"                       \
    "s_cbranch_execnz .Lfbc_%=\n"                      \
    ".Lfbd_%=:\n"                                      \
    "s_mov_b64 %[srun], exec\n"                        \
    "s_mov_b64 exec, %[sorig]\n"

#define FR_FBC_ASM(SFX, BLOCK_ITS, STEP)               \
    "s_mov_b64 %[sorig], exec\n"                       \
    "s_mov_b64 exec, %[mask]\n"                        \
    ".Lfc_%=:\n" BLOCK_ITS                             \
    "v_add_" SFX " %[t], %[A], %[B]\n"                 \
    "v_add_f32 %[cnt], %[cnt], " STEP "\n"             \
    "v_cmpx_nlt_" SFX " %[t4lim], %[t]\n"              \
    "s_cbranch_execz .Lfcd_%=\n"                       \
    "s_sub_u32 %[k], %[k], 1\n"                        \
    "s_cbranch_scc0 .Lfc_%=\n"                         \
    ".Lfcd_%=:\n"                                      \
    "s_mov_b64 %[srun], exec\n"                        \
    "s_mov_b64 exec, %[sorig]\n"

#define FR_FB_SPEC_STRETCH                             \
    "s_min_u32 %[k], %[kend], %[specq]\n"              \
    "s_sub_u32 %[kend], %[kend], %[k]\n"               \
    "s_sub_u32 %[k], %[k], 1\n"                        \
    "s_mov_b64 %[squiet], exec\n"
#define FR_FB_SPEC_MOVS(MOV) MOV " %[X], %[X1]\n" MOV " %[Y], %[Y1]\n" MOV " %[A], %[A1]\n" MOV " %[B], %[B1]\n"
#define FR_FB_SPEC_EVENT(SFX, MOV, REST, KB, COUNT, LOOP, DONE)  \
    "s_cmp_eq_u32 %[kend], 0\n"                               \
    "s_cbranch_scc1 " DONE "\n"                               \
    "s_cmp_eq_u64 %[squiet], exec\n"                          \
    "s_cbranch_scc0 .Lfnew_%=\n"                              \
    "s_cmp_lt_u32 %[kend], " KB "\n"                          \
    "s_cbranch_scc1 .Lfnew_%=\n"                              \
    ".Lfsp_%=:\n" FR_SC_IT_R(SFX, "", "1") REST(SFX, "1")     \
    "v_add_" SFX " %[t], %[A1], %[B1]\n"                      \
    "v_cmp_nge_" SFX " vcc, %[t4lim], %[t]\n"                 \
    "s_cbranch_vccnz .LfrbA_%=\n"                             \
    COUNT                                                     \
    "s_sub_u32 %[kend], %[kend], " KB "\n"                    \
    "s_cmp_lt_u32 %[kend], " KB "\n"                          \
    "s_cbranch_scc1 .LfexA_%=\n"                              \
    FR_SC_IT_R(SFX, "1", "") REST(SFX, "")                    \
    "v_add_" SFX " %[t], %[A], %[B]\n"                        \
    "v_cmp_nge_" SFX " vcc, %[t4lim], %[t]\n"                 \
    "s_cbranch_vccnz .LfrbB_%=\n"                             \
    COUNT                                                     \
    "s_sub_u32 %[kend], %[kend], " KB "\n"                    \
    "s_cmp_lt_u32 %[kend], " KB "\n"                          \
    "s_cbranch_scc0 .Lfsp_%=\n"                               \
    "s_branch .Lfrest_%=\n"                                   \
    ".LfexA_%=:\n" FR_FB_SPEC_MOVS(MOV)                       \
    ".Lfrest_%=:\n"   \
    "s_cmp_eq_u32 %[kend], 0\n"                               \
    "s_cbranch_scc1 " DONE "\n"                               \
    "s_branch .Lfnew_%=\n"                                    \
    ".LfrbB_%=:\n" FR_FB_SPEC_MOVS(MOV)                       \
    ".LfrbA_%=:\n"                                            \
    "s_lshl_b32 %[specq], %[specq], 1\n"                      \
    "s_min_u32 %[specq], %[specq], 0x2000\n"                  \
    ".Lfnew_%=:\n" FR_FB_SPEC_STRETCH                         \
    "s_branch " LOOP "\n"

#define FR_FB_SPEC_ASM(SFX, MOV, BLOCK_ITS, MSHIFT, REST, KB) \
    "s_mov_b64 %[sorig], exec\n"                       \
    "s_mov_b64 exec, %[mask]\n"                        \
    "s_mov_b32 %[kend], %[n0]\n"                       \
    FR_FB_SPEC_STRETCH                                 \
    ".Lfb_%=:\n" BLOCK_ITS                             \
    "v_add_" SFX " %[t], %[A], %[B]\n"                 \
    "s_mov_b64 %[sprev], exec\n"                       \
    "v_cmpx_nlt_" SFX " %[t4lim], %[t]\n"              \
    "s_xor_b64 %[sdiff], %[sprev], exec\n"             \
    "s_cbranch_scc1 .Lfbr_%=\n"                        \
    ".Lfbc_%=:\n"                                      \
    "s_sub_u32 %[k], %[k], 1\n"                        \
    "s_cbranch_scc0 .Lfb_%=\n"                         \
    FR_FB_SPEC_EVENT(SFX, MOV, REST, KB, "", ".Lfb_%=", ".Lfbd_%=") \
    ".Lfbr_%=:\n"   \
    "s_add_u32 %[stmp], %[k], %[kend]\n"               \
    "s_sub_u32 %[stmp], %[n0], %[stmp]\n"              \
    "s_lshl_b32 %[stmp], %[stmp], " MSHIFT "\n"        \
    "s_add_u32 %[stmp], %[stmp], %[base]\n"            \
    "s_mov_b64 %[sprev], exec\n"                       \
    "s_mov_b64 exec, %[sdiff]\n"                       \
    "v_cvt_f32_u32 %[cnt], %[stmp]\n"                  \
    "s_mov_b64 exec, %[sprev]\n"                       \
    "s_cbranch_execnz .Lfbc_%=\n"                      \
    ".Lfbd_%=:\n"                                      \
    "s_mov_b64 %[srun], exec\n"                        \
    "s_mov_b64 exec, %[sorig]\n"

#define FR_FBC_SPEC_ASM(SFX, MOV, BLOCK_ITS, STEP, REST, KB, SPECSTEP) \
    "s_mov_b64 %[sorig], exec\n"                       \
    "s_mov_b64 exec, %[mask]\n"                        \
// ... 1223 lines not shown
        if (take_unit(j)) {
            FR_COLD_PARAMS(kp);
            const uint32_t len = __builtin_amdgcn_readlane(list_len, cur_q);
            const size_t base = (size_t)cur_q * kp->surv_sub_capacity + (size_t)j * FR_SURV_CHUNK;
            nx_n = len - j * FR_SURV_CHUNK < FR_SURV_CHUNK ? len - j * FR_SURV_CHUNK : FR_SURV_CHUNK;
            const size_t e = base + (lane < nx_n ? lane : 0u);
            pf_z = static_cast<const T2 *>(kp->surv_z)[e];
            pf_pos = reinterpret_cast<const uint2 *>(kp->surv_pos)[e];
            pf_cnt = kp->surv_cnt[e];
            if (!julia) pf_c = static_cast<const T2 *>(kp->surv_c)[e];
        }
    };
    prefetch_chunk();

    T X = 0, Y = 0, A = 0, B = 0, c2re = j2re, c2im = j2im;
    float cnt = 0.0f;
    uint32_t px = 0, py = 0;
    bool busy = false;
    uint32_t have_chunk = 0, exhausted = 0, next = 0, chunk_n = 0, chunk_maxcnt = 0;
    uint32_t qcount = 0, upper = 0;

    auto finish_and_colour = [&](uint32_t base, uint32_t count) __attribute__((always_inline)) {
        __syncthreads();
        const bool mine = lane < count;
        const uint32_t e = base + (mine ? lane : 0u);
        const T2 xy = q_xy[e];
        const uint4 meta = q_meta[e];
        T fX = xy.x, fY = xy.y, f2re = j2re, f2im = j2im;
        if (!julia) {
            const T2 c2 = q_c2[e];
            f2re = c2.x, f2im = c2.y;
        }
        T fA = fX * fX, fB = fY * fY, ft = fA + fB;
        float fc = __builtin_bit_cast(float, meta.x);
        const bool escaped0 = mine && fc > 0.0f && ft > lim4v;
        bool lv = mine && !escaped0 && fc < capf;
        unsigned long long esc = ballot64(escaped0), live = ballot64(lv);
        while (live != 0ull) {
            uint32_t nf = 64u;
            if (ballot64(lv && capf - fc < 64.0f) != 0ull) {
                live &= ~ballot64(lv && fc >= capf);
                if (live == 0ull) break;
                nf = cap - __builtin_amdgcn_readfirstlane(wave_max_u32(lane_in(live) ? (uint32_t)fc : 0u));
                nf = nf > 64u ? 64u : nf;
            }
            const unsigned long long still = finish_scaled<T>(live, nf, fX, fY, fA, fB, ft, fc, f2re, f2im, lim4);
            esc |= live & ~still;
            live = still;
            lv = lane_in(live);
        }
        const unsigned long long fin = count >= 64u ? ~0ull : (1ull << count) - 1ull;
        uint32_t packed = 0;
        unsigned long long coloured = 0ull;
        if (fast_colour && esc != 0ull) {
            Filter32 f;
            {
                FR_COLD_PARAMS(kp);
                f.lo = kp->filt_lo32, f.k = kp->filt_k32, f.c = kp->filt_c32;
                f.p0 = kp->prim32[0], f.p1 = kp->prim32[2], f.p2 = kp->prim32[1];
            }
            const float d32 = (float)ft * 0.25f;
            const bool sure = d32 >= f.lo && d32 <= 0x1.ffffep119f;
            const bool decided = colour_fast32(f, d32, fc, packed);
            coloured = ballot64(sure && decided) & esc;
        }
        const unsigned long long stayed = fin & ~esc;
        bool inside_done = false;
        if (stayed != 0ull) {
            if (lane_in(stayed)) {
                double dist;
                if constexpr (sizeof(T) == 8) {
                    const T re = fX * (T)0.5, im = fY * (T)0.5;
                    dist = (double)(re * re + im * im);
                } else {
                    const double zre = (double)(fX * (T)0.5), zim = (double)(fY * (T)0.5);
                    dist = zre * zre + zim * zim;
                }
                FR_COLD_PARAMS(kp);
                inside_done = !(dist > kp->stable_limit);
                if (inside_done) {
                    packed = 0u;
                    if (kp->inside)
                        packed = sat_u8_dev(kp->sec_f[0] * dist) | (sat_u8_dev(kp->sec_f[2] * dist) << 8) | (sat_u8_dev(kp->sec_f[1] * dist) << 16);
                }
            }
        }
        const unsigned long long rest = fin & ~coloured & ~ballot64(inside_done);
        if (rest != 0ull) {
            if (lane_in(rest)) {
                const T re = fX * (T)0.5, im = fY * (T)0.5;
                const T r2 = re * re, i2 = im * im;
                const uint32_t iters = lane_in(esc) ? (uint32_t)fc - 1u : cap;
                FR_COLD_PARAMS(kp);
                const ColourConsts cc = make_colour_consts(*kp);
                uint8_t rgb[3];
                colour_pixel<T>(cc, re, im, r2, i2, iters, tab, s_pal, rgb);
                packed = (uint32_t)rgb[0] | ((uint32_t)rgb[1] << 8) | ((uint32_t)rgb[2] << 16);
            }
        }
        if (mine) {
            if (narrow) {
                store_packed(out.rgb, (meta.z * ncols + meta.y) * bpp, packed, bpp);
            } else {
                uint8_t *o = out.rgb + ((uint64_t)meta.z * ncols + meta.y) * bpp;
                if (bpp == 4u) {
                    *reinterpret_cast<uint32_t *>(o) = packed | 0xFF000000u;
                } else {
                    o[0] = (uint8_t)packed, o[1] = (uint8_t)(packed >> 8), o[2] = (uint8_t)(packed >> 16);
                }
            }
        }
        tr_colour++;
        __syncthreads();
    };
    auto push = [&](bool who) __attribute__((always_inline)) {
        const unsigned long long m = ballot64(who);
        if (m == 0ull) return;
        if (who) {
            const uint32_t slot = qcount + __builtin_amdgcn_mbcnt_hi((uint32_t)(m >> 32), __builtin_amdgcn_mbcnt_lo((uint32_t)m, 0u));
            T2 xy;
            xy.x = X, xy.y = Y;
            q_xy[slot] = xy;
            q_meta[slot] = make_uint4(__builtin_bit_cast(uint32_t, cnt), px, py, 0u);
            if (!julia) {
                T2 c2;
                c2.x = c2re, c2.y = c2im;
                q_c2[slot] = c2;
            }
        }
        qcount += (uint32_t)__builtin_popcountll(m);
        if (qcount >= 64u) {
            finish_and_colour(qcount - 64u, 64u);
            qcount -= 64u;
        }
    };

    for (;;) {
        if (!have_chunk && !exhausted) {
            if (nx_n == 0) {
                exhausted = 1;
            } else {
                __syncthreads();
                T2 xy;
                xy.x = pf_z.x + pf_z.x, xy.y = pf_z.y + pf_z.y;
                s_cxy[lane] = xy;
                s_cmeta[lane] = make_uint4(__builtin_bit_cast(uint32_t, (float)pf_cnt), pf_pos.x, pf_pos.y, pf_cnt);
                if (!julia) {
                    T2 c2;
                    c2.x = pf_c.x + pf_c.x, c2.y = pf_c.y + pf_c.y;
                    s_cc2[lane] = c2;
                }
                chunk_maxcnt = ballot64(lane < nx_n && pf_cnt != first_cap) == 0ull
                                   ? first_cap
                                   : __builtin_amdgcn_readfirstlane(wave_max_u32(lane < nx_n ? pf_cnt : 0u));
                __syncthreads();
                chunk_n = nx_n;
                have_chunk = 1;
                next = 0;
                tr_chunks++;
                prefetch_chunk();
            }
        }
        unsigned long long busy_mask = ballot64(busy);
        if (have_chunk && busy_mask != ~0ull) {
            const unsigned long long free_mask = ~busy_mask;
            const uint32_t pix = next + __builtin_amdgcn_mbcnt_hi((uint32_t)(free_mask >> 32), __builtin_amdgcn_mbcnt_lo((uint32_t)free_mask, 0u));
            bool direct = false;
            if (!busy && pix < chunk_n) {
                const T2 xy = s_cxy[pix];
                const uint4 meta = s_cmeta[pix];
                X = xy.x, Y = xy.y, A = X * X, B = Y * Y;
                if (!julia) {
                    const T2 c2 = s_cc2[pix];
                    c2re = c2.x, c2im = c2.y;
                }
                cnt = __builtin_bit_cast(float, meta.x);
                px = meta.y, py = meta.z;
                if (A + B <= t4v && meta.w + (uint32_t)M <= cap)
                    busy = true;
                else
                    direct = true;
            }
            next += (uint32_t)__builtin_popcountll(free_mask);
            if (next >= chunk_n) have_chunk = 0;
            if (upper < chunk_maxcnt) upper = chunk_maxcnt;
            push(direct);
            busy_mask = ballot64(busy);
        }
        if (!have_chunk && !exhausted && busy_mask != ~0ull) continue;
        if (busy_mask == 0ull) {
            if (!have_chunk && exhausted) break;
            continue;
        }
        if (upper + (uint32_t)M > cap) upper = __builtin_amdgcn_readfirstlane(wave_max_u32(busy ? (uint32_t)cnt : 0u));
        const uint32_t nblocks = (cap - upper) / (uint32_t)M;
        const uint32_t nbusy = (uint32_t)__builtin_popcountll(busy_mask);
        uint32_t thr = 0, minblocks = 0;
        if (have_chunk || !exhausted) {
            thr = __builtin_amdgcn_readfirstlane(nbusy > queue_want ? nbusy - queue_want : 0u);
            minblocks = queue_minblocks;
        }
        unsigned long long running;
        const uint32_t blocks = second_block_run<T, M>(busy_mask, nblocks, X, Y, A, B, c2re, c2im, t4lim, cnt, thr, minblocks, running);
        upper += blocks * (uint32_t)M;
        tr_episodes++;
        tr_iters += blocks * (uint32_t)M;
        unsigned long long leave = busy_mask & ~running;
        if (upper + (uint32_t)M > cap) leave |= ballot64(lane_in(running) && (uint32_t)cnt + (uint32_t)M > cap);
        if (leave != 0ull) {
            const bool lv = lane_in(leave);
            if (lv) busy = false;
            push(lv);
        }
    }
    if (qcount) finish_and_colour(0u, qcount);
    if (out.trace && lane == 0) {
        unsigned long long *t = out.trace + (size_t)blockIdx.x * 16;
        t[0] = t_start, t[1] = __builtin_amdgcn_s_memrealtime(), t[2] = tr_chunks, t[3] = tr_episodes, t[4] = tr_colour, t[5] = tr_iters;
        t[6] = t[7] = t[8] = 0ull;
    }
}

template <typename T, int M, int SRC>
hipError_t launch_queue_form(const fr_kparams &p, const fr_kout &out, hipStream_t stream) {
    const uint64_t npx = SRC == 1 ? ((uint64_t)p.surv_sub_capacity + FR_SURV_CHUNK - 1) / FR_SURV_CHUNK
                                  : ((uint64_t)p.ncols + kQPatchW - 1) / kQPatchW;
    const uint64_t npy = SRC == 1 ? FR_SURV_QUEUES : ((uint64_t)p.nrows + kQPatchH - 1) / kQPatchH;
    if (npx * npy == 0) return hipSuccess;
    if (npx * npy > 0xFFF00000ull) return hipErrorInvalidConfiguration;
    size_t dyn = p.palette ? sizeof(uint32_t) * p.palette_entries : 0;
    if (SRC == 1 && !p.second_v1 && p.algo != 2) dyn += (FR_SURV_CHUNK + kQStack) * (sizeof(T) * 2);
    static thread_local int cached_device = -1, cached_cus = 0;
    int dev = 0;
    hipError_t e = hipGetDevice(&dev);
    if (e != hipSuccess) return e;
    if (dev != cached_device) {
        if ((e = hipDeviceGetAttribute(&cached_cus, hipDeviceAttributeMultiprocessorCount, dev)) != hipSuccess) return e;
        cached_device = dev;
    }
    int per_cu = 0;
    if (SRC == 1 && !p.second_v1)
        e = hipOccupancyMaxActiveBlocksPerMultiprocessor(&per_cu, escape_second_kernel<T, M>, 64, dyn);
    else
        e = hipOccupancyMaxActiveBlocksPerMultiprocessor(&per_cu, escape_queue_kernel<T, M, SRC>, 64, dyn);
    if (e != hipSuccess) return e;
    if (per_cu < 1) per_cu = 1;
    if (per_cu > 32) per_cu = 32;
    uint64_t grid = (uint64_t)per_cu * (uint64_t)cached_cus;
    if (grid > npx * npy) grid = npx * npy;
    if (SRC == 1 && !p.second_v1)
        hipLaunchKernelGGL((escape_second_kernel<T, M>), dim3((uint32_t)grid), dim3(64), dyn, stream, p, out);
    else
        hipLaunchKernelGGL((escape_queue_kernel<T, M, SRC>), dim3((uint32_t)grid), dim3(64), dyn, stream, p, out, (uint32_t)npx,
                           (uint32_t)(npx * npy));
    return hipGetLastError();
}

template <typename T, int M, int K, int BANDS, bool SPEC, bool V1>
void launch_first_form(const fr_kparams &p, const fr_kout &out, dim3 grid, hipStream_t stream) {
    if constexpr (V1)
        hipLaunchKernelGGL((escape_first_v1_kernel<T, M, K, BANDS>), grid, dim3(64), 0, stream, p, out);
    else
        hipLaunchKernelGGL((escape_first_kernel<T, M, K, BANDS, SPEC>), grid, dim3(64), 0, stream, p, out);
}

template <typename T, int M, int K, bool SPEC, bool V1>
void launch_first_bands(const fr_kparams &p, const fr_kout &out, dim3 grid, int bands, hipStream_t stream) {
    if constexpr (K == 7) {
        if (bands == 4) return launch_first_form<T, M, K, 4, SPEC, V1>(p, out, grid, stream);
    }
    launch_first_form<T, M, K, 1, SPEC, V1>(p, out, grid, stream);
}

template <typename T, int K>
hipError_t launch_first_pass(const fr_kparams &p, const fr_kout &out, hipStream_t stream, bool v1) {
    const uint64_t gx = ((uint64_t)p.ncols + 8 * K - 1) / (8 * K);
    const uint64_t row_tiles = ((uint64_t)p.nrows + 7) / 8;
    const int bands = (K == 7 && !p.first_one_band && gx * ((row_tiles + 3) / 4) >= 131072) ? 4 : 1;
    const uint64_t row_blocks = (row_tiles + bands - 1) / bands;
    const uint64_t gy = row_blocks < 32768 ? row_blocks : 32768;
    const uint64_t gz = (row_blocks + gy - 1) / gy;
    if (gx > 0x7FFFFFFFull || gz > 65535) return hipErrorInvalidConfiguration;
    const dim3 grid((uint32_t)gx, (uint32_t)gy, (uint32_t)gz);
    if constexpr (K == 7) {
        if (v1 && p.loop_mode == 4) {
            launch_first_bands<T, 4, K, false, true>(p, out, grid, bands, stream);
            return hipGetLastError();
        }
    }
    if (fr_first_pass_speculates(p))
        launch_first_bands<T, 4, K, true, false>(p, out, grid, bands, stream);
    else if (p.loop_mode == 4)
        launch_first_bands<T, 4, K, false, false>(p, out, grid, bands, stream);
    else
        launch_first_bands<T, 2, K, false, false>(p, out, grid, bands, stream);
    return hipGetLastError();
}

template <typename T>
hipError_t launch_first_pass_len(const fr_kparams &p, bool v1, const fr_kout &out, hipStream_t stream) {
    return (p.strip_tiles == 4 && !v1) ? launch_first_pass<T, 4>(p, out, stream, false) : launch_first_pass<T, 7>(p, out, stream, v1);
}

template <typename T, int kStripTiles>
hipError_t launch_strips(const fr_kparams &p, int mode, const fr_kout &out, hipStream_t stream) {
    if (p.ncols == 0 || p.nrows == 0) return hipSuccess;
    const uint64_t gx = ((uint64_t)p.ncols + 8 * kStripTiles - 1) / (8 * kStripTiles);
    const uint64_t row_tiles = ((uint64_t)p.nrows + 7) / 8;
    const uint64_t gy = row_tiles < 32768 ? row_tiles : 32768;
    const uint64_t gz = (row_tiles + gy - 1) / gy;
    if (gx > 0x7FFFFFFFull || gz > 65535) return hipErrorInvalidConfiguration;
    dim3 grid((uint32_t)gx, (uint32_t)gy, (uint32_t)gz), block(64);
#define FR_K(MODE) escape_strip_kernel<T, MODE, kStripTiles>
    FR_LAUNCH_BY_MODE(FR_K);
#undef FR_K
    return hipGetLastError();
}

template <typename T, int TW, int TH, int WX, int WY>
hipError_t launch_tile(const fr_kparams &p, int mode, const fr_kout &out, hipStream_t stream) {
    constexpr int BW = TW * WX, BH = TH * WY;
    const uint64_t tiles_x = ((uint64_t)p.ncols + BW - 1) / BW;
    const uint64_t tiles_y = ((uint64_t)p.nrows + BH - 1) / BH;
    const uint64_t blocks = tiles_x * tiles_y;
    if (blocks == 0) return hipSuccess;
    if (blocks > 0x7FFFFFFFull) return hipErrorInvalidConfiguration;
    dim3 grid((uint32_t)blocks), block(64 * kWaves);
#define FR_K(MODE) escape_kernel<T, TW, TH, WX, WY, MODE>
    FR_LAUNCH_BY_MODE(FR_K);
#undef FR_K
    return hipGetLastError();
}


template <typename T>
__global__ __launch_bounds__(256) void recursive_batch_kernel(uint32_t iterations, const double *start,
                                                             const double *c, size_t n, double limit,
                                                             double *out_pos, uint32_t *out_iters) {
    const size_t k = (size_t)blockIdx.x * 256 + threadIdx.x;
    if (k >= n) return;
    T re = (T)start[2 * k], im = (T)start[2 * k + 1], r2, i2;
    const T lim = (T)limit;
    const uint32_t it = orbit<T>(iterations, re, im, (T)c[2 * k], (T)c[2 * k + 1], lim * lim, r2, i2);
    out_pos[2 * k] = (double)re;
    out_pos[2 * k + 1] = (double)im;
    out_iters[k] = it;
}

template <typename T>
__global__ __launch_bounds__(64) void view_sample_kernel(const fr_kparams p, uint32_t side, uint32_t cap_s, uint32_t episode, uint32_t keep,
                                                         unsigned long long *counters, unsigned long long *result,
                                                         unsigned long long tag) {
    const uint32_t lane = threadIdx.x, lx = lane & 7u, ly = lane >> 3;
    const uint32_t ti = blockIdx.x % side, tj = blockIdx.x / side;
    const uint32_t col0 = (uint32_t)(((uint64_t)(2u * ti + 1u) * p.ncols) / (2u * side)) & ~7u;
    const uint32_t row0 = (uint32_t)(((uint64_t)(2u * tj + 1u) * p.nrows) / (2u * side)) & ~7u;
    const uint32_t cx = col0 + lx, r = row0 + ly;
    const bool valid = cx < p.ncols && r < p.nrows;
    const double width = (double)p.width, height = (double)p.height;
    const uint32_t x = p.x_first + cx * p.x_stride;
    const uint32_t y = p.y_first + (r / p.block_rows) * p.y_stride + r % p.block_rows;
    const double sre = coord_to_space((double)x, height, (width / height) / 2.0, p.pos_re, p.scale_re);
    const double sim = coord_to_space((double)y, height, 0.5, p.pos_im, p.scale_im);
    uint32_t executed = 0;
    if (valid) {
        T re = (T)sre, im = (T)sim, r2, i2;
        const T cre = p.algo == 2 ? (T)p.julia_re : re, cim = p.algo == 2 ? (T)p.julia_im : im;
        const T lim = (T)p.limit;
        const uint32_t it = orbit<T>(cap_s, re, im, cre, cim, lim * lim, r2, i2);
        executed = it < cap_s ? it + 1u : cap_s;
    }
    const uint32_t mx = wave_max_u32(executed);
    unsigned long long sum = executed;
    for (int off = 32; off > 0; off >>= 1) sum += __shfl_down(sum, off, 64);
    const unsigned long long capped = (unsigned long long)__builtin_popcountll(__ballot(valid && executed == cap_s));
    uint32_t e = episode, len = episode, nrun = 0;
    bool hands_over = false;
    while (e < mx) {
        nrun = (uint32_t)__builtin_popcountll(__ballot(executed > e));
        if (nrun < keep) {
            hands_over = nrun > 0u;
            break;
        }
        if (e >= 8u * episode && len < 16u * episode) len += len;
        e += len;
    }
    unsigned long long rest = executed > e ? executed - e : 0u;
    for (int off = 32; off > 0; off >>= 1) rest += __shfl_down(rest, off, 64);
    if (lane == 0) {
        atomicAdd(counters + 0, sum);
        atomicAdd(counters + 1, 64ull * mx);
        atomicAdd(counters + 2, 1ull);
        atomicAdd(counters + 3, capped);
        if (hands_over) {
            atomicAdd(counters + 4, (unsigned long long)nrun);
            atomicAdd(counters + 5, 64ull * (mx - e) - rest);
            atomicAdd(counters + 6, rest);
        }
        __threadfence();
        const unsigned long long done = atomicAdd(counters + 7, 1ull);
        if (done + 1ull == (unsigned long long)gridDim.x) {
            __threadfence();
            for (int k = 0; k < 7; k++) {
                const unsigned long long v = atomicExch(counters + k, 0ull);
                __hip_atomic_store(result + k, v, __ATOMIC_RELAXED, __HIP_MEMORY_SCOPE_SYSTEM);
            }
            atomicExch(counters + 7, 0ull);
            __threadfence_system();
            __hip_atomic_store(result + 7, tag, __ATOMIC_RELEASE, __HIP_MEMORY_SCOPE_SYSTEM);
        }
    }
}

__global__ __launch_bounds__(256) void palette_kernel(const fr_kparams p, uint32_t *palette) {
    const uint32_t i = blockIdx.x * 256 + threadIdx.x;
    if (i > p.iterations) return;
    const ColourConsts cc = make_colour_consts(p);
    uint8_t rgb[3];
    colour_outside_flat(cc, i, rgb);
    palette[i] = (uint32_t)rgb[0] | ((uint32_t)rgb[1] << 8) | ((uint32_t)rgb[2] << 16);
}

__global__ __launch_bounds__(256) void colour_kernel(const fr_kparams p, const double *z, const uint32_t *iters, size_t n,
                                                   uint8_t *rgb) {
    __shared__ double s_tab[FR_LOG2_N * 3];
    const double *gt = &g_log2_tab[0][0];
    for (uint32_t k = threadIdx.x; k < FR_LOG2_N * 3; k += 256) s_tab[k] = gt[k];
    __syncthreads();
    const size_t k = (size_t)blockIdx.x * 256 + threadIdx.x;
    if (k >= n) return;
    uint8_t out[3] = {0, 0, 0};
    if (p.algo == 0 || p.algo == 2) {
        const ColourConsts cc = make_colour_consts(p);
        const double re = z[2 * k], im = z[2 * k + 1];
        colour_of(cc, re * re + im * im, iters[k], s_tab, nullptr, out);
    }
    rgb[3 * k + 0] = out[0];
    rgb[3 * k + 1] = out[1];
    rgb[3 * k + 2] = out[2];
}

__global__ __launch_bounds__(256) void math_probe_kernel(int which, const double *in, double *out, size_t n) {
    __shared__ double s_tab[FR_LOG2_N * 3];
    const double *gt = &g_log2_tab[0][0];
    for (uint32_t k = threadIdx.x; k < FR_LOG2_N * 3; k += 256) s_tab[k] = gt[k];
    __syncthreads();
    const size_t k = (size_t)blockIdx.x * 256 + threadIdx.x;
    if (k >= n) return;
    const double x = in[k];
    double y;
    if (which == 0)
        y = fr_log2_tab(x, s_tab);
    else if (which == 1)
        y = __builtin_sqrt(x);
    else if (which == 3)
        y = (double)sat_u8_dev(x);
    else if (which == 5)
        y = (double)sat_u8_pack<1>((float)x, 0xAABBCCDDu);
    else
        y = x / in[(k + 1) % n];
    out[k] = y;
}

__global__ __launch_bounds__(256) void cast_scan_kernel(uint32_t lo, uint32_t hi, unsigned long long *count) {
    const uint64_t stride = (uint64_t)gridDim.x * 256;
    unsigned long long bad = 0;
    for (uint64_t b = (uint64_t)lo + (uint64_t)blockIdx.x * 256 + threadIdx.x; b <= hi; b += stride) {
        const float f = __builtin_bit_cast(float, (uint32_t)b);
        const uint32_t want = sat_u8_dev(f);
        const uint32_t got = sat_u8_pack<2>(f, sat_u8_pack<1>(f, sat_u8_pack<0>(f, 0xFF000000u)));
        bad += got != (0xFF000000u | want | (want << 8) | (want << 16));
    }
    if (bad) atomicAdd(count, bad);
}

__global__ __launch_bounds__(256) void nu_scan_kernel(uint32_t lo, uint32_t hi, unsigned long long *worst_bits) {
    __shared__ double s_tab[FR_LOG2_N * 3];
    const double *gt = &g_log2_tab[0][0];
    for (uint32_t k = threadIdx.x; k < FR_LOG2_N * 3; k += 256) s_tab[k] = gt[k];
    __syncthreads();
    const uint64_t stride = (uint64_t)gridDim.x * 256;
    double worst = 0.0;
    for (uint64_t b = (uint64_t)lo + (uint64_t)blockIdx.x * 256 + threadIdx.x; b <= hi; b += stride) {
        const float d = __builtin_bit_cast(float, (uint32_t)b);
        const float nu32 = __builtin_amdgcn_logf(__builtin_amdgcn_logf(d) * 0.25f);
        const double nu = fr_log2_tab(fr_log2_tab(__builtin_sqrt((double)d), s_tab) * 0.5, s_tab);
        const double err = __builtin_fabs((double)nu32 - nu);
        worst = err > worst || err != err ? err : worst;
    }
    atomicMax(worst_bits, (unsigned long long)fr_bits_of(worst));
}

__global__ __launch_bounds__(256) void copy_out_kernel(const uint8_t *src, uint8_t *dst, size_t bytes, unsigned int *counter,
                                                      unsigned long long *flag, unsigned long long seq) {
    const size_t head = (16u - (reinterpret_cast<uintptr_t>(dst) & 15u)) & 15u;
    const size_t h = head < bytes ? head : bytes;
    const size_t units = (bytes - h) / 16;
    const uint4 *s4 = reinterpret_cast<const uint4 *>(src + h);
    uint4 *d4 = reinterpret_cast<uint4 *>(dst + h);
    const size_t stride = (size_t)gridDim.x * 256;
    size_t k = (size_t)blockIdx.x * 256 + threadIdx.x;
    for (; k + 3 * stride < units; k += 4 * stride) {
        const uint4 a = s4[k], b = s4[k + stride], c = s4[k + 2 * stride], d = s4[k + 3 * stride];
        d4[k] = a, d4[k + stride] = b, d4[k + 2 * stride] = c, d4[k + 3 * stride] = d;
    }
    for (; k < units; k += stride) d4[k] = s4[k];
    if (blockIdx.x == 0) {
        for (size_t k = threadIdx.x; k < h; k += 256) dst[k] = src[k];
        const size_t t0 = h + units * 16;
        for (size_t k = t0 + threadIdx.x; k < bytes; k += 256) dst[k] = src[k];
    }
    __threadfence_system();
    __syncthreads();
    if (threadIdx.x == 0) {
        const unsigned int done = atomicAdd(counter, 1u);
        if (done + 1u == gridDim.x) {
            atomicExch(counter, 0u);
            __threadfence_system();
            __hip_atomic_store(flag, seq, __ATOMIC_RELEASE, __HIP_MEMORY_SCOPE_SYSTEM);
        }
    }
}

template <typename T>
__global__ __launch_bounds__(64) void escape_extend_kernel(const fr_kparams p, double *z, uint32_t *iters, const uint32_t from) {
    const uint32_t lane = threadIdx.x;
    const uint32_t row0 = (blockIdx.y + gridDim.y * blockIdx.z) * 8u;
    if (row0 >= p.nrows) return;
    const uint32_t col0 = blockIdx.x * 8u;
    const uint32_t lx = lane & 7u, ly = lane >> 3;
    const uint32_t cx = col0 + lx, r = row0 + ly;
    const bool valid = cx < p.ncols && r < p.nrows;
    const uint64_t k = (uint64_t)r * p.ncols + cx;
    uint32_t done = 0;
    if (valid) done = iters[k];
    const bool running = valid && done == from;
    if (ballot64(running) == 0ull) return;

    double cre = p.julia_re, cim = p.julia_im;
    if (p.algo == 0) {
        const bool row_lane = lane >= 8u;
        uint32_t coord_u;
        if (row_lane) {
            const uint32_t rr = row0 + ((lane - 8u) & 7u);
            coord_u = p.y_first + (rr / p.block_rows) * p.y_stride + rr % p.block_rows;
        } else {
            coord_u = p.x_first + (col0 + lane) * p.x_stride;
        }
        const double width = (double)p.width, height = (double)p.height;
        const double coord_lane = coord_to_space((double)coord_u, height, row_lane ? 0.5 : (width / height) / 2.0,
                                                 row_lane ? p.pos_im : p.pos_re, row_lane ? p.scale_im : p.scale_re);
        cre = __shfl(coord_lane, lx, 64);
        cim = __shfl(coord_lane, 8 + ly, 64);
    }
    if (running) {
        const uint32_t n = p.iterations - from;
        uint32_t it, completed;
        if constexpr (sizeof(T) == 8) {
            double re = z[2 * k], im = z[2 * k + 1];
            double r2 = re * re, i2 = im * im;
            it = orbit_run<double>(n, re, im, cre, cim, p.limit * p.limit, r2, i2, EpisodeCtl{0, 0}, completed, p.loop_spec);
            z[2 * k] = re;
            z[2 * k + 1] = im;
        } else {
            float re = (float)z[2 * k], im = (float)z[2 * k + 1];
            float r2 = re * re, i2 = im * im;
            const float lim = (float)p.limit;
            it = orbit_run<float>(n, re, im, (float)cre, (float)cim, lim * lim, r2, i2, EpisodeCtl{0, 0}, completed, p.loop_spec);
            z[2 * k] = (double)re;
            z[2 * k + 1] = (double)im;
        }
        iters[k] = it >= completed ? p.iterations : from + it;
    }
}

__global__ __launch_bounds__(256) void colour_rows_kernel(const fr_kparams p, const double *z, const uint32_t zw, const uint32_t *iters,
                                                        const size_t n, const uint32_t bpp, uint8_t *out) {
    __shared__ double s_tab[FR_LOG2_N * 3];
    const bool escape_algo = p.algo == 0 || p.algo == 2;
    if (escape_algo && p.smooth) {
        const double *gt = &g_log2_tab[0][0];
        for (uint32_t k = threadIdx.x; k < FR_LOG2_N * 3; k += 256) s_tab[k] = gt[k];
        __syncthreads();
    }
    const uint32_t lane = threadIdx.x & 63u;
    const bool dwords = (reinterpret_cast<uintptr_t>(out) & 3u) == 0;
    const uint32_t im_at = zw >> 1;
    for (size_t base = (size_t)blockIdx.x * 256; base < n; base += (size_t)gridDim.x * 256) {
        const size_t k = base + threadIdx.x;
        const bool valid = k < n;
        uint32_t packed = 0;
        if (valid && escape_algo) {
            const double re = z[(size_t)zw * k], im = z[(size_t)zw * k + im_at];
            uint8_t rgb[3] = {0, 0, 0};
            FR_COLD_PARAMS(kp);
            const ColourConsts cc = make_colour_consts(*kp);
            colour_of(cc, re * re + im * im, iters[k], s_tab, nullptr, rgb);
            packed = (uint32_t)rgb[0] | ((uint32_t)rgb[1] << 8) | ((uint32_t)rgb[2] << 16);
        }
        if (bpp == 4u) {
            if (valid) reinterpret_cast<uint32_t *>(out)[k] = packed | 0xFF000000u;
            continue;
        }
        const size_t wave0 = k - lane;
        if (dwords && wave0 + 64 <= n) {
            const uint32_t first = (4u * lane) / 3u, shift = 8u * ((4u * lane) % 3u);
            const uint32_t a = __shfl(packed, first & 63u, 64), b = __shfl(packed, (first + 1u) & 63u, 64);
            const uint64_t both = (uint64_t)a | ((uint64_t)b << 24);
            if (lane < 48u) reinterpret_cast<uint32_t *>(out + 3 * wave0)[lane] = (uint32_t)(both >> shift);
        } else if (valid) {
            uint8_t *o = out + 3 * k;
            o[0] = (uint8_t)packed;
            o[1] = (uint8_t)(packed >> 8);
            o[2] = (uint8_t)(packed >> 16);
        }
    }
}

}

hipError_t fr_launch_escape_extend(const fr_kparams &p, int precision, uint32_t from_iterations, double *z, uint32_t *iters,
                                   hipStream_t stream, const char **kernel_name) {
    if (kernel_name) *kernel_name = precision == 1 ? "escape_extend_kernel<float>" : "escape_extend_kernel<double>";
    if (p.ncols == 0 || p.nrows == 0) return hipSuccess;
    if (p.iterations < from_iterations || (p.algo != 0 && p.algo != 2)) return hipErrorInvalidValue;
    const uint64_t gx = ((uint64_t)p.ncols + 7) / 8;
    const uint64_t row_tiles = ((uint64_t)p.nrows + 7) / 8;
    const uint64_t gy = row_tiles < 32768 ? row_tiles : 32768;
    const uint64_t gz = (row_tiles + gy - 1) / gy;
    if (gx > 0x7FFFFFFFull || gz > 65535) return hipErrorInvalidConfiguration;
    const dim3 grid((uint32_t)gx, (uint32_t)gy, (uint32_t)gz), block(64);
    if (precision == 1)
        hipLaunchKernelGGL(escape_extend_kernel<float>, grid, block, 0, stream, p, z, iters, from_iterations);
    else
        hipLaunchKernelGGL(escape_extend_kernel<double>, grid, block, 0, stream, p, z, iters, from_iterations);
    return hipGetLastError();
}

hipError_t fr_launch_colour_rows(const fr_kparams &p, const double *z, uint32_t z_width, const uint32_t *iters, size_t n,
                                 uint32_t channels, void *out, hipStream_t stream) {
    if (n == 0) return hipSuccess;
    if ((z_width != 2 && z_width != 4) || (channels != 3 && channels != 4)) return hipErrorInvalidValue;
    uint64_t blocks = ((n + 255) / 256 + 3) / 4;
    if (blocks > 0x7FFFFFFFull) blocks = 0x7FFFFFFFull;
    hipLaunchKernelGGL(colour_rows_kernel, dim3((uint32_t)blocks), dim3(256), 0, stream, p, z, z_width, iters, n, channels,
                       static_cast<uint8_t *>(out));
    return hipGetLastError();
}

hipError_t fr_launch_copy_out(const void *src, void *dst, size_t bytes, unsigned int *counter, unsigned long long *flag,
                              unsigned long long seq, hipStream_t stream) {
    if (bytes == 0) return hipErrorInvalidValue;
    if ((reinterpret_cast<uintptr_t>(src) & 15u) != (reinterpret_cast<uintptr_t>(dst) & 15u)) return hipErrorInvalidValue;
    size_t groups = (bytes / 16 + 256 * 4 - 1) / (256 * 4);
    if (groups < 1) groups = 1;
    if (groups > 128) groups = 128;
    hipLaunchKernelGGL(copy_out_kernel, dim3((uint32_t)groups), dim3(256), 0, stream, static_cast<const uint8_t *>(src),
                       static_cast<uint8_t *>(dst), bytes, counter, flag, seq);
    return hipGetLastError();
}

hipError_t fr_launch_nu_scan(uint32_t lo_bits, uint32_t hi_bits, double *out, hipStream_t stream) {
    hipError_t e = hipMemsetAsync(out, 0, sizeof(double), stream);
    if (e != hipSuccess) return e;
    hipLaunchKernelGGL(nu_scan_kernel, dim3(256 * 16), dim3(256), 0, stream, lo_bits, hi_bits,
                       reinterpret_cast<unsigned long long *>(out));
    return hipGetLastError();
}

hipError_t fr_launch_cast_scan(uint32_t lo_bits, uint32_t hi_bits, double *out, hipStream_t stream) {
    hipError_t e = hipMemsetAsync(out, 0, sizeof(double), stream);
    if (e != hipSuccess) return e;
    hipLaunchKernelGGL(cast_scan_kernel, dim3(256 * 16), dim3(256), 0, stream, lo_bits, hi_bits,
                       reinterpret_cast<unsigned long long *>(out));
    return hipGetLastError();
}

hipError_t fr_launch_recursive_batch(uint32_t iterations, const double *start, const double *c, size_t n,
                                     double limit, int precision, double *out_pos, uint32_t *out_iters,
                                     hipStream_t stream) {
    if (n == 0) return hipSuccess;
    const uint64_t blocks = (n + 255) / 256;
    if (blocks > 0x7FFFFFFFull) return hipErrorInvalidConfiguration;
    if (precision == 1)
        hipLaunchKernelGGL(recursive_batch_kernel<float>, dim3((uint32_t)blocks), dim3(256), 0, stream, iterations,
                           start, c, n, limit, out_pos, out_iters);
    else
        hipLaunchKernelGGL(recursive_batch_kernel<double>, dim3((uint32_t)blocks), dim3(256), 0, stream, iterations,
                           start, c, n, limit, out_pos, out_iters);
    return hipGetLastError();
}

hipError_t fr_launch_colour(const fr_kparams &p, const double *z, const uint32_t *iters, size_t n, uint8_t *rgb,
                            hipStream_t stream) {
    if (n == 0) return hipSuccess;
    const uint64_t blocks = (n + 255) / 256;
    if (blocks > 0x7FFFFFFFull) return hipErrorInvalidConfiguration;
    hipLaunchKernelGGL(colour_kernel, dim3((uint32_t)blocks), dim3(256), 0, stream, p, z, iters, n, rgb);
    return hipGetLastError();
}

hipError_t fr_launch_view_sample(const fr_kparams &p, int precision, uint32_t side, uint32_t cap_s, uint32_t episode, uint32_t keep,
                                 unsigned long long *counters, unsigned long long *result, unsigned long long tag,
                                 hipStream_t stream) {
    if (side == 0 || p.ncols == 0 || p.nrows == 0) return hipErrorInvalidValue;
    if (precision == 1)
        hipLaunchKernelGGL(view_sample_kernel<float>, dim3(side * side), dim3(64), 0, stream, p, side, cap_s, episode, keep, counters, result, tag);
    else
        hipLaunchKernelGGL(view_sample_kernel<double>, dim3(side * side), dim3(64), 0, stream, p, side, cap_s, episode, keep, counters, result, tag);
    return hipGetLastError();
}

hipError_t fr_launch_palette(const fr_kparams &p, uint32_t *palette, hipStream_t stream) {
    const uint32_t entries = p.iterations + 1;
    hipLaunchKernelGGL(palette_kernel, dim3((entries + 255) / 256), dim3(256), 0, stream, p, palette);
    return hipGetLastError();
}

hipError_t fr_launch_math_probe(int which, const double *in, double *out, size_t n, hipStream_t stream) {
    if (n == 0) return hipSuccess;
    hipLaunchKernelGGL(math_probe_kernel, dim3((uint32_t)((n + 255) / 256)), dim3(256), 0, stream, which, in, out, n);
    return hipGetLastError();
}


template <typename T>
static hipError_t launch_tile_shape(const fr_kparams &p, int mode, int tile, const fr_kout &out, hipStream_t stream) {
    switch (tile) {
    case 6401:
        return launch_tile<T, 64, 1, 1, 4>(p, mode, out, stream);
    case 3202:
        return launch_tile<T, 32, 2, 2, 2>(p, mode, out, stream);
    case 1604:
        return launch_tile<T, 16, 4, 2, 2>(p, mode, out, stream);
    case 808:
        return launch_tile<T, 8, 8, 2, 2>(p, mode, out, stream);
    default:
        return hipErrorInvalidValue;
    }
}

hipError_t fr_launch_tile(const fr_kparams &p, int precision, int mode, int tile, const fr_kout &out, hipStream_t stream) {
    return precision == 1 ? launch_tile_shape<float>(p, mode, tile, out, stream) : launch_tile_shape<double>(p, mode, tile, out, stream);
}

template <typename T>
static hipError_t launch_strips_len(const fr_kparams &p, int mode, int strip_tiles, const fr_kout &out, hipStream_t stream) {
    switch (strip_tiles) {
    case 7:
        return launch_strips<T, 7>(p, mode, out, stream);
    case 4:
        return launch_strips<T, 4>(p, mode, out, stream);
    case 2:
        return launch_strips<T, 2>(p, mode, out, stream);
    case 1:
        return launch_strips<T, 1>(p, mode, out, stream);
    default:
        return hipErrorInvalidValue;
    }
}

hipError_t fr_launch_strips(const fr_kparams &p, int precision, int mode, int strip_tiles, const fr_kout &out, hipStream_t stream) {
    return precision == 1 ? launch_strips_len<float>(p, mode, strip_tiles, out, stream)
                          : launch_strips_len<double>(p, mode, strip_tiles, out, stream);
}

hipError_t fr_launch_refill(const fr_kparams &p, int precision, int mode, const fr_kout &out, hipStream_t stream) {
    return precision == 1 ? launch_refill<float, 7>(p, mode, out, stream) : launch_refill<double, 7>(p, mode, out, stream);
}

hipError_t fr_launch_first_pass(const fr_kparams &p, int precision, bool v1, const fr_kout &out, hipStream_t stream) {
    return precision == 1 ? launch_first_pass_len<float>(p, v1, out, stream) : launch_first_pass_len<double>(p, v1, out, stream);
}

template <typename T>
static hipError_t launch_queue_src(const fr_kparams &p, int src, const fr_kout &out, hipStream_t stream) {
    if (p.loop_mode == 4) return src == 1 ? launch_queue_form<T, 4, 1>(p, out, stream) : launch_queue_form<T, 4, 0>(p, out, stream);
    return src == 1 ? launch_queue_form<T, 2, 1>(p, out, stream) : launch_queue_form<T, 2, 0>(p, out, stream);
}

hipError_t fr_launch_queue(const fr_kparams &p, int precision, int src, const fr_kout &out, hipStream_t stream) {
    return precision == 1 ? launch_queue_src<float>(p, src, out, stream) : launch_queue_src<double>(p, src, out, stream);
}
```

fractal-renderer_amd/csrc/fr_launch.h:

```cpp
#ifndef FR_LAUNCH_H
#define FR_LAUNCH_H

#include "fr_kernels.h"

hipError_t fr_launch_tile(const fr_kparams &p, int precision, int mode, int tile, const fr_kout &out, hipStream_t stream);
hipError_t fr_launch_strips(const fr_kparams &p, int precision, int mode, int strip_tiles, const fr_kout &out, hipStream_t stream);
hipError_t fr_launch_refill(const fr_kparams &p, int precision, int mode, const fr_kout &out, hipStream_t stream);

hipError_t fr_launch_first_pass(const fr_kparams &p, int precision, bool v1, const fr_kout &out, hipStream_t stream);

hipError_t fr_launch_queue(const fr_kparams &p, int precision, int src, const fr_kout &out, hipStream_t stream);

inline bool fr_first_pass_speculates(const fr_kparams &p) {
    return p.loop_mode == 4 && p.loop_spec != 0 && !(p.first_no_spec && !p.first_only);
}

#endif
```

include/fractal_hip.h:

```cpp
#ifndef FRACTAL_HIP_H
#define FRACTAL_HIP_H

#include <stddef.h>
#include <stdint.h>

#ifdef __cplusplus
extern "C" {
#endif

#define FR_ABI_VERSION 3

typedef enum fr_status {
    FR_OK = 0,
    FR_ERR_INVALID_ARGUMENT = 1,
    FR_ERR_BUFFER_TOO_SMALL = 2,
    FR_ERR_NO_DEVICE = 3,
    FR_ERR_HIP = 4,
    FR_ERR_UNSUPPORTED_ALGO = 5
} fr_status;

typedef enum fr_algo {
    FR_ALGO_MANDELBROT = 0,
    FR_ALGO_BARNSLEY_FERN = 1,
    FR_ALGO_JULIA = 2
// ... 4 lines not shown
    double im;
} fr_imaginary;

typedef struct fr_rgb {
    uint8_t r;
    uint8_t g;
    uint8_t b;
} fr_rgb;

typedef struct fr_config {
    uint32_t algo;
    uint32_t width;
    uint32_t height;
    uint32_t iterations;
    double limit;
    double stable_limit;
    fr_imaginary pos;
    fr_imaginary scale;
    double exposure;
    uint8_t inside;
    uint8_t smooth;
    fr_rgb primary_color;
    fr_rgb secondary_color;
    double color_weight;
    fr_imaginary julia_set;
} fr_config;

#define FR_BLA_DEFAULT_BITS 40
#define FR_PT_MAX_ITERATIONS (1u << 24)
#define FR_WIDE_MAX_WORDS 16
typedef enum fr_precision {
    FR_PRECISION_F64 = 0,
    FR_PRECISION_F32 = 1,
    FR_PRECISION_DD = 2,
    FR_PRECISION_PT = 3
} fr_precision;


int fr_init(int device);
int fr_shutdown(void);
int fr_device_count(int *count);
int fr_device_name(char *buf, size_t buf_len);
const char *fr_last_error(void);
int fr_abi_version(void);
const char *fr_build_id(void);

void fr_config_new(fr_config *cfg, uint32_t algo);


int fr_render_rgb8(const fr_config *cfg, uint8_t *out, size_t out_len);

int fr_render_rows_rgb8(const fr_config *cfg, int precision, uint32_t y0, uint32_t y1, uint8_t *out,
                        size_t out_len);

int fr_render_rows_rgb8_device(const fr_config *cfg, int precision, uint32_t y0, uint32_t y1,
                               void *d_out, size_t out_len, void *hip_stream);

int fr_render_rows_rgba8(const fr_config *cfg, int precision, uint32_t y0, uint32_t y1, uint8_t *out,
                         size_t out_len);
int fr_render_rows_rgba8_device(const fr_config *cfg, int precision, uint32_t y0, uint32_t y1, void *d_out,
                                size_t out_len, void *hip_stream);

int fr_render_block_cyclic_rgb8_device(const fr_config *cfg, int precision, uint32_t block_rows,
                                       uint32_t first_block, uint32_t block_stride, void *d_out,
                                       size_t out_len, void *hip_stream, uint64_t *rows_written);
int fr_render_block_cyclic_range_rgb8_device(const fr_config *cfg, int precision, uint32_t block_rows,
                                             uint32_t first_block, uint32_t block_stride, uint32_t max_blocks,
                                             int dest_is_image, void *d_out, size_t out_len, void *hip_stream,
                                             uint64_t *rows_written);

int fr_render_block_cyclic_rgb8(const fr_config *cfg, int precision, uint32_t block_rows, uint32_t first_block,
                                uint32_t block_stride, uint8_t *out, size_t out_len, uint64_t *rows_written);
uint64_t fr_block_cyclic_rows(uint32_t height, uint32_t block_rows, uint32_t first_block,
                              uint32_t block_stride);


typedef struct fr_render_opts {
    uint32_t size;
    int32_t tile;
    int32_t loop_mode;
    int32_t palette;
    int32_t cycle_shortcut;
    int32_t refill_minrun;
    int32_t refill_quit16;
    int32_t colour_filter;
} fr_render_opts;
void fr_render_opts_init(fr_render_opts *opts);

int fr_render_rows_rgb8_device_opts(const fr_config *cfg, int precision, uint32_t y0, uint32_t y1, void *d_out,
                                    size_t out_len, void *hip_stream, const fr_render_opts *opts);
int fr_render_rows_rgba8_device_opts(const fr_config *cfg, int precision, uint32_t y0, uint32_t y1, void *d_out,
                                     size_t out_len, void *hip_stream, const fr_render_opts *opts);
int fr_render_rows_rgb8_opts(const fr_config *cfg, int precision, uint32_t y0, uint32_t y1, uint8_t *out,
                             size_t out_len, const fr_render_opts *opts);
int fr_render_block_cyclic_range_rgb8_device_opts(const fr_config *cfg, int precision, uint32_t block_rows,
                                                  uint32_t first_block, uint32_t block_stride, uint32_t max_blocks,
                                                  int dest_is_image, void *d_out, size_t out_len, void *hip_stream,
                                                  uint64_t *rows_written, const fr_render_opts *opts);


int fr_init_devices(const int *devices, int n);
int fr_multi_device_count(int *count);

int fr_render_rgb8_multi(const fr_config *cfg, int precision, uint32_t block_rows, uint8_t *out, size_t out_len);

typedef enum fr_gather { FR_GATHER_PEER_COPY = 0, FR_GATHER_RCCL = 1 } fr_gather;
int fr_render_rgb8_multi_device(const fr_config *cfg, int precision, uint32_t block_rows, int gather, void *d_out,
                                size_t out_len);

int fr_set_multi_root_share(int q);

#define FR_MAX_DEVICES 16
typedef struct fr_multi_stats {
    uint32_t n_devices;
    uint32_t kernels[FR_MAX_DEVICES];
    float kernel_ms[FR_MAX_DEVICES];
    uint64_t rows[FR_MAX_DEVICES];
    double wall_ms;
    float transfer_span_ms[FR_MAX_DEVICES];
    double job_ms[FR_MAX_DEVICES];
    uint64_t bytes_moved[FR_MAX_DEVICES];
} fr_multi_stats;
int fr_multi_last_stats(fr_multi_stats *stats);

int fr_debug_rccl_selftest(size_t bytes);
int fr_debug_rccl_probe(void);
int fr_debug_inject_multi_failure(int device_index, int chunk);

int fr_pin_host_buffer(void *ptr, size_t len);
int fr_unpin_host_buffer(void *ptr);


int fr_render_fern_rgb8(const fr_config *cfg, uint32_t threads, uint64_t seed, uint32_t walkers, uint8_t *out,
                        size_t out_len);


int fr_render_rows_dd(const fr_config *cfg, const fr_imaginary *pos_lo, uint32_t y0, uint32_t y1, int channels,
                      uint8_t *out, size_t out_len);
int fr_render_rows_dd_device(const fr_config *cfg, const fr_imaginary *pos_lo, uint32_t y0, uint32_t y1, int channels,
                             void *d_out, size_t out_len, void *hip_stream);
int fr_escape_rows_dd(const fr_config *cfg, const fr_imaginary *pos_lo, uint32_t y0, uint32_t y1, double *z,
                      uint32_t *iters);


int fr_render_rows_pt(const fr_config *cfg, const fr_imaginary *pos_lo, uint32_t y0, uint32_t y1, int channels,
                      uint8_t *out, size_t out_len);
int fr_render_rows_pt_device(const fr_config *cfg, const fr_imaginary *pos_lo, uint32_t y0, uint32_t y1, int channels,
                             void *d_out, size_t out_len, void *hip_stream);
int fr_escape_rows_pt(const fr_config *cfg, const fr_imaginary *pos_lo, uint32_t y0, uint32_t y1, double *z,
                      uint32_t *iters);
int fr_debug_reference_orbit(const fr_config *cfg, const fr_imaginary *pos_lo, int which, double *out, size_t cap,
                             uint32_t *len);


#define FR_SS_MAX 8

int fr_ss_workspace_bytes(const fr_config *cfg, uint32_t supersample, uint32_t y0, uint32_t y1, size_t *min_bytes,
                          size_t *best_bytes);
int fr_render_rows_ss_device(const fr_config *cfg, int precision, const fr_imaginary *pos_lo, uint32_t supersample,
                             uint32_t y0, uint32_t y1, int channels, void *d_out, size_t out_len, void *d_work,
                             size_t work_len, void *hip_stream, const fr_render_opts *opts);
int fr_render_rows_ss(const fr_config *cfg, int precision, const fr_imaginary *pos_lo, uint32_t supersample, uint32_t y0,
                      uint32_t y1, int channels, uint8_t *out, size_t out_len, const fr_render_opts *opts);
int fr_box_filter_rgb8(const uint8_t *src, uint32_t width, uint32_t rows, uint32_t supersample, int channels, uint8_t *out,
                       size_t out_len);
int fr_box_filter_rgb8_device(const void *d_src, uint32_t width, uint32_t rows, uint32_t supersample, int channels,
                              void *d_out, size_t out_len, void *hip_stream);


int fr_pixel(const fr_config *cfg, uint32_t x, uint32_t y, fr_rgb *out);
int fr_pixel_p(const fr_config *cfg, int precision, uint32_t x, uint32_t y, fr_rgb *out);


int fr_recursive(uint32_t iterations, fr_imaginary start, fr_imaginary c, double limit,
                 fr_imaginary *out_pos, uint32_t *out_iters);

int fr_recursive_batch(uint32_t iterations, const fr_imaginary *start, const fr_imaginary *c, size_t n,
                       double limit, int precision, fr_imaginary *out_pos, uint32_t *out_iters);

int fr_escape_rows(const fr_config *cfg, int precision, uint32_t y0, uint32_t y1, double *z_re_im,
                   uint32_t *iters);

int fr_colour_rgb8(const fr_config *cfg, const double *z_re_im, const uint32_t *iters, size_t n, uint8_t *out,
                   size_t out_len);
int fr_colour_rgb8_device(const fr_config *cfg, const void *d_z_re_im, const void *d_iters, size_t n, void *d_out,
                          size_t out_len, void *hip_stream);



int fr_escape_rows_device(const fr_config *cfg, int precision, const fr_imaginary *pos_lo, uint32_t y0, uint32_t y1,
                          int z_width, void *d_z, void *d_iters, void *hip_stream, const fr_render_opts *opts);

int fr_escape_extend_device(const fr_config *cfg, int precision, const fr_imaginary *pos_lo, uint32_t y0, uint32_t y1,
                            uint32_t from_iterations, int z_width, void *d_z, void *d_iters, void *hip_stream,
                            const fr_render_opts *opts);
int fr_escape_extend(const fr_config *cfg, int precision, const fr_imaginary *pos_lo, uint32_t y0, uint32_t y1,
                     uint32_t from_iterations, int z_width, double *z, uint32_t *iters);

int fr_colour_rows_device(const fr_config *cfg, const void *d_z, int z_width, const void *d_iters, size_t n, int channels,
                          void *d_out, size_t out_len, void *hip_stream);



int fr_escape_rows_pt_state_device(const fr_config *cfg, const fr_imaginary *pos_lo, uint32_t y0, uint32_t y1, void *d_z,
                                   void *d_iters, void *d_dz, void *d_m, void *hip_stream);
int fr_escape_extend_pt_device(const fr_config *cfg, const fr_imaginary *pos_lo, uint32_t y0, uint32_t y1,
                               uint32_t from_iterations, void *d_z, void *d_iters, void *d_dz, void *d_m, void *hip_stream);
int fr_escape_rows_pt_state(const fr_config *cfg, const fr_imaginary *pos_lo, uint32_t y0, uint32_t y1, double *z,
                            uint32_t *iters, double *dz, uint32_t *m);
int fr_escape_extend_pt(const fr_config *cfg, const fr_imaginary *pos_lo, uint32_t y0, uint32_t y1, uint32_t from_iterations,
                        double *z, uint32_t *iters, double *dz, uint32_t *m);
int fr_debug_pt_orbit_cache(uint32_t out[4]);


typedef struct fr_wide_centre { uint32_t n_words; const uint64_t *re; const uint64_t *im; } fr_wide_centre;

int fr_wide_from_double(double v, uint64_t *w, uint32_t n);
int fr_wide_add_double(uint64_t *w, uint32_t n, double delta);
int fr_wide_to_double(const uint64_t *w, uint32_t n, double *hi, double *lo);
int fr_wide_from_decimal(const char *text, uint64_t *w, uint32_t n);

int fr_render_rows_pt_wide(const fr_config *cfg, const fr_wide_centre *centre, uint32_t y0, uint32_t y1, int channels,
                           uint8_t *out, size_t out_len);
int fr_render_rows_pt_wide_device(const fr_config *cfg, const fr_wide_centre *centre, uint32_t y0, uint32_t y1, int channels,
                                  void *d_out, size_t out_len, void *hip_stream);
int fr_escape_rows_pt_wide(const fr_config *cfg, const fr_wide_centre *centre, uint32_t y0, uint32_t y1, double *z,
                           uint32_t *iters);
int fr_escape_rows_pt_wide_state_device(const fr_config *cfg, const fr_wide_centre *centre, uint32_t y0, uint32_t y1, void *d_z,
                                        void *d_iters, void *d_dz, void *d_m, void *hip_stream);
int fr_escape_extend_pt_wide_device(const fr_config *cfg, const fr_wide_centre *centre, uint32_t y0, uint32_t y1,
                                    uint32_t from_iterations, void *d_z, void *d_iters, void *d_dz, void *d_m, void *hip_stream);
int fr_escape_rows_pt_wide_state(const fr_config *cfg, const fr_wide_centre *centre, uint32_t y0, uint32_t y1, double *z,
                                 uint32_t *iters, double *dz, uint32_t *m);
int fr_escape_extend_pt_wide(const fr_config *cfg, const fr_wide_centre *centre, uint32_t y0, uint32_t y1, uint32_t from_iterations,
                             double *z, uint32_t *iters, double *dz, uint32_t *m);
int fr_debug_reference_orbit_wide(const fr_config *cfg, const fr_wide_centre *centre, int which, double *out, size_t cap,
                                  uint32_t *len);


int fr_render_rows_pt_bla(const fr_config *cfg, const fr_imaginary *pos_lo, const fr_wide_centre *centre, int bits, uint32_t y0,
                          uint32_t y1, int channels, uint8_t *out, size_t out_len);
int fr_render_rows_pt_bla_device(const fr_config *cfg, const fr_imaginary *pos_lo, const fr_wide_centre *centre, int bits,
                                 uint32_t y0, uint32_t y1, int channels, void *d_out, size_t out_len, void *hip_stream);
int fr_escape_rows_pt_bla(const fr_config *cfg, const fr_imaginary *pos_lo, const fr_wide_centre *centre, int bits, uint32_t y0,
                          uint32_t y1, double *z, uint32_t *iters);
int fr_escape_rows_pt_bla_device(const fr_config *cfg, const fr_imaginary *pos_lo, const fr_wide_centre *centre, int bits,
                                 uint32_t y0, uint32_t y1, void *d_z, void *d_iters, void *hip_stream);
int fr_debug_bla_table(const fr_config *cfg, const fr_imaginary *pos_lo, const fr_wide_centre *centre, int bits, int which,
                       uint32_t level, double *out, size_t cap, uint32_t *len);
int fr_debug_bla_count(const fr_config *cfg, const fr_imaginary *pos_lo, const fr_wide_centre *centre, int bits, uint32_t y0,
                       uint32_t y1, uint64_t *passes, uint64_t *steps);
int fr_debug_bla_cache(uint32_t out[4]);


int fr_render_rows_pt_scaled(const fr_config *cfg, const fr_wide_centre *centre, int bits, uint32_t y0, uint32_t y1, int channels,
                             uint8_t *out, size_t out_len);
int fr_render_rows_pt_scaled_device(const fr_config *cfg, const fr_wide_centre *centre, int bits, uint32_t y0, uint32_t y1,
                                    int channels, void *d_out, size_t out_len, void *hip_stream);
int fr_escape_rows_pt_scaled(const fr_config *cfg, const fr_wide_centre *centre, int bits, uint32_t y0, uint32_t y1, double *z,
                             uint32_t *iters);
int fr_escape_rows_pt_scaled_device(const fr_config *cfg, const fr_wide_centre *centre, int bits, uint32_t y0, uint32_t y1,
                                    void *d_z, void *d_iters, void *hip_stream);
int fr_debug_bla_table_scaled(const fr_config *cfg, const fr_wide_centre *centre, int bits, int which, uint32_t level, double *out,
                              size_t cap, uint32_t *len);
int fr_debug_pt_scaled_count(const fr_config *cfg, const fr_wide_centre *centre, int bits, uint32_t y0, uint32_t y1,
                             uint64_t *passes, uint64_t *steps);

int fr_escape_rows_pt_scaled_state_device(const fr_config *cfg, const fr_wide_centre *centre, uint32_t y0, uint32_t y1, void *d_z,
                                          void *d_iters, void *d_w, void *d_m, void *hip_stream);
int fr_escape_extend_pt_scaled_device(const fr_config *cfg, const fr_wide_centre *centre, uint32_t y0, uint32_t y1,
                                      uint32_t from_iterations, void *d_z, void *d_iters, void *d_w, void *d_m, void *hip_stream);
int fr_escape_rows_pt_scaled_state(const fr_config *cfg, const fr_wide_centre *centre, uint32_t y0, uint32_t y1, double *z,
                                   uint32_t *iters, double *w, uint32_t *m);
int fr_escape_extend_pt_scaled(const fr_config *cfg, const fr_wide_centre *centre, uint32_t y0, uint32_t y1, uint32_t from_iterations,
                               double *z, uint32_t *iters, double *w, uint32_t *m);


int fr_count_iterations(const fr_config *cfg, int precision, uint32_t y0, uint32_t y1, uint32_t sx,
                        uint32_t sy, uint64_t *total, uint64_t *pixels);

int fr_set_profiling(int enabled);
int fr_last_kernel_ms(float *ms);
int fr_last_kernel_name(char *buf, size_t buf_len);

int fr_set_tile(int tile);

int fr_set_dispatch_sampling(int enabled);
int fr_debug_sample_view(const fr_config *cfg, int precision, double out[8]);
int fr_debug_view_choice(const fr_config *cfg, int precision, uint32_t y0, uint32_t y1, int *state, int *choice,
                         uint32_t *strip_tiles);

int fr_set_refill_policy(int minrun, int quit16);

int fr_set_cycle_shortcut(int enabled);

int fr_set_palette(int enabled);

int fr_set_colour_filter(int enabled);

int fr_set_loop_mode(int mode);
int fr_debug_loop_plan(const fr_config *cfg, int precision, uint32_t *loop_mode, double *skip_t, uint32_t *spec_quiet);
int fr_debug_set_spec_maxlen(uint32_t maxlen);
int fr_debug_spec_maxlen(const fr_config *cfg, int precision, uint32_t *maxlen);

int fr_debug_math(int which, const double *in, double *out, size_t n);
int fr_debug_set_queue_trace(void *d_trace);
int fr_debug_set_two_pass_capacity(uint32_t entries_per_list);

#ifdef __cplusplus
}
#endif
#endif
```

Before: 5447 billion.

## Add specialized plain strip kernel for common smooth RGB Mandelbrot configuration

Adds a PLAIN template instance of the strip kernel used when the config is the common case: Mandelbrot, RGB, smooth colouring, no palette, fp32 filter, speculative loop mode. It precomputes limit bit patterns on the host, skips wave-uniform readfirstlane and per-tile branching, takes a no-bounds-check full-tile path, and stages the log2 colour table into LDS only when a slow-path pixel actually needs it. The aim is to cut per-tile overhead and register pressure in the hot strip kernel, at the cost of more template instances and an on-by-default toggle that changes which kernel runs.

```diff
diff --git a/fractal-renderer_amd/_native.py b/fractal-renderer_amd/_native.py
--- a/fractal-renderer_amd/_native.py
+++ b/fractal-renderer_amd/_native.py
@@ -356,6 +356,8 @@
                                      C.POINTER(C.c_uint32)]),
     "fr_debug_set_spec_maxlen": (C.c_int, [C.c_uint32]),
     "fr_debug_spec_maxlen": (C.c_int, [C.POINTER(fr_config), C.c_int, C.POINTER(C.c_uint32)]),
+    "fr_debug_set_strip_plain": (C.c_int, [C.c_int]),
+    "fr_debug_strip_plain": (C.c_int, [C.POINTER(fr_config), C.c_int, C.c_int, C.POINTER(C.c_int)]),
     "fr_set_palette": (C.c_int, [C.c_int]),
     "fr_set_cycle_shortcut": (C.c_int, [C.c_int]),
     "fr_set_refill_policy": (C.c_int, [C.c_int, C.c_int]),
diff --git a/fractal-renderer_amd/build.py b/fractal-renderer_amd/build.py
--- a/fractal-renderer_amd/build.py
+++ b/fractal-renderer_amd/build.py
@@ -10,7 +10,7 @@
 KERNEL_SOURCES = ["fr_kernels.hip", "fr_bla.hip", "fr_scaled.hip"]
 SOURCES = KERNEL_SOURCES + ["fr_dispatch.hip", "fr_api.hip", "fr_host.hip", "fr_multi.hip", "fr_fern.hip",
                             "fr_dd.hip", "fr_pt.hip", "fr_wide.hip", "fr_ss.hip"]
-DEPS = SOURCES + ["fr_kernels.h", "fr_launch.h", "fr_ctx.h", "fr_wide.h", "fr_bla.h", "fr_math.h", "fr_colour.h", "fr_log2_table.inc",
+DEPS = SOURCES + ["fr_kernels.h", "fr_launch.h", "fr_ctx.h", "fr_wide.h", "fr_bla.h", "fr_math.h", "fr_colour.h", "fr_log2_table.inc", "fr_strip_body.inc",
                   os.path.join("..", "..", "include", "fractal_hip.h")]
 HIPCC_FLAGS = [
     "--offload-arch=gfx950",
diff --git a/fractal-renderer_amd/csrc/fr_api.hip b/fractal-renderer_amd/csrc/fr_api.hip
--- a/fractal-renderer_amd/csrc/fr_api.hip
+++ b/fractal-renderer_amd/csrc/fr_api.hip
@@ -1779,6 +1779,25 @@
     return FR_OK;
 }
 
+int fr_debug_set_strip_plain(int on) {
+    fr_strip_plain_set(on != 0);
+    return FR_OK;
+}
+
+int fr_debug_strip_plain(const fr_config *cfg, int precision, int channels, int *plain) {
+    if (!cfg || !plain) return fail(FR_ERR_INVALID_ARGUMENT, "NULL argument");
+    int rc = check_precision(precision);
+    if (rc == FR_OK) rc = check_channels(channels);
+    if (rc != FR_OK) return rc;
+    const Opts o = default_opts();
+    fr_kparams p;
+    rows_params(cfg, o, 0, cfg->height, (unsigned)channels, p);
+    plan_loop(cfg, precision, o, p);
+    const int k = o.tile == 0 ? (int)fr_strip_len_by_size(p) : o.tile == 8 ? 7 : o.tile == 1 ? 1 : 0;
+    *plain = (k != 0 && fr_strip_plain_applies(p, precision, FR_OUT_RGB, k)) ? 1 : 0;
+    return FR_OK;
+}
+
 int fr_debug_set_queue_trace(void *d_trace) {
     g_queue_trace.store(static_cast<unsigned long long *>(d_trace));
     return FR_OK;
diff --git a/fractal-renderer_amd/csrc/fr_dispatch.hip b/fractal-renderer_amd/csrc/fr_dispatch.hip
--- a/fractal-renderer_amd/csrc/fr_dispatch.hip
+++ b/fractal-renderer_amd/csrc/fr_dispatch.hip
@@ -2,9 +2,13 @@
 
 #include <cmath>
 
+#include <atomic>
+
 #include "fr_launch.h"
 
 namespace {
+
+std::atomic<bool> g_strip_plain{true};
 
 #define FR_KNAME(base, k) (precision == 1 ? base "<float, " k ">" : base "<double, " k ">")
 
@@ -41,11 +45,13 @@
 hipError_t run_strips(const fr_kparams &p, int precision, int mode, uint32_t k_len, const fr_kout &out, hipStream_t stream,
                       const char *&name) {
     const int k = k_len >= 7u ? 7 : k_len >= 4u ? 4 : k_len >= 2u ? 2 : 1;
-    name = k == 7   ? FR_KNAME("escape_strip_kernel", "7 tiles")
+    const bool plain = fr_strip_plain_applies(p, precision, mode, k);
+    name = plain    ? (k == 7 ? FR_KNAME("escape_strip_kernel", "7 tiles; plain") : FR_KNAME("escape_strip_kernel", "1 tile; plain"))
+           : k == 7 ? FR_KNAME("escape_strip_kernel", "7 tiles")
            : k == 4 ? FR_KNAME("escape_strip_kernel", "4 tiles")
            : k == 2 ? FR_KNAME("escape_strip_kernel", "2 tiles")
                     : FR_KNAME("escape_strip_kernel", "1 tile");
-    return fr_launch_strips(p, precision, mode, k, out, stream);
+    return fr_launch_strips(p, precision, mode, k, out, stream, plain);
 }
 
 hipError_t run_refill(const fr_kparams &p, int precision, int mode, const fr_kout &out, hipStream_t stream, const char *&name) {
@@ -76,7 +82,7 @@
         const uint64_t tiles = (((uint64_t)p.ncols + 7) / 8) * (((uint64_t)p.nrows + 7) / 8);
         if (two_pass_ready(p, mode)) return run_two_pass(p, precision, 0, out, stream, name);
         if (tiles >= 262144 && ((p.algo == 2 && mode != FR_OUT_RGB) || p.cycle_shortcut)) return run_refill(p, precision, mode, out, stream, name);
-        const uint32_t k_len = (mode == FR_OUT_RGB && p.strip_tiles) ? p.strip_tiles : tiles >= 524288 ? 7u : 1u;
+        const uint32_t k_len = (mode == FR_OUT_RGB && p.strip_tiles) ? p.strip_tiles : fr_strip_len_by_size(p);
         return run_strips(p, precision, mode, k_len, out, stream, name);
     }
     case 1:
@@ -113,6 +119,21 @@
     const hipError_t e = launch_precision(p, precision, mode, out, tile, stream, name);
     if (kernel_name) *kernel_name = name;
     return e;
+}
+
+uint32_t fr_strip_len_by_size(const fr_kparams &p) {
+    const uint64_t tiles = (((uint64_t)p.ncols + 7) / 8) * (((uint64_t)p.nrows + 7) / 8);
+    return tiles >= 524288 ? 7u : 1u;
+}
+
+void fr_strip_plain_set(bool on) { g_strip_plain.store(on); }
+
+bool fr_strip_plain_applies(const fr_kparams &p, int precision, int mode, int strip_tiles) {
+    if (!g_strip_plain.load() || mode != FR_OUT_RGB || (strip_tiles != 7 && strip_tiles != 1)) return false;
+    if (precision != 0 && precision != 1) return false;
+    if (p.algo != 0 || p.out_rgba || !p.smooth || p.palette != nullptr || !p.colour_filter32 || p.cycle_shortcut) return false;
+    if (p.loop_mode != 4 || p.loop_spec == 0) return false;
+    return (uint64_t)p.ncols * 3u * 8u <= 0xFFFFFFFFull;
 }
 
 bool fr_wants_work_queue(const fr_kparams &p, int tile) {
diff --git a/fractal-renderer_amd/csrc/fr_kernels.h b/fractal-renderer_amd/csrc/fr_kernels.h
--- a/fractal-renderer_amd/csrc/fr_kernels.h
+++ b/fractal-renderer_amd/csrc/fr_kernels.h
@@ -57,6 +57,12 @@
     uint32_t *surv_counts;
 };
 
+struct fr_kplain {
+    uint64_t lim4_bits, t4_bits;
+    double half_aspect;
+    uint32_t full_ok;
+};
+
 constexpr uint32_t FR_SURV_QUEUES = 64;
 constexpr uint32_t FR_SURV_COUNT_STRIDE = 32;
 constexpr uint32_t FR_SURV_CHUNK = 64;
@@ -81,6 +87,10 @@
 
 hipError_t fr_launch_escape(const fr_kparams &p, int precision, int mode, const fr_kout &out, int tile,
                             hipStream_t stream, const char **kernel_name);
+
+bool fr_strip_plain_applies(const fr_kparams &p, int precision, int mode, int strip_tiles);
+void fr_strip_plain_set(bool on);
+uint32_t fr_strip_len_by_size(const fr_kparams &p);
 
 hipError_t fr_launch_escape_dd(const fr_kparams &p, double pos_lo_re, double pos_lo_im, int mode, const fr_kout &out,
                                bool with_lo, hipStream_t stream, const char **kernel_name);
diff --git a/fractal-renderer_amd/csrc/fr_kernels.hip b/fractal-renderer_amd/csrc/fr_kernels.hip
--- a/fractal-renderer_amd/csrc/fr_kernels.hip
+++ b/fractal-renderer_amd/csrc/fr_kernels.hip
@@ -425,24 +425,26 @@
     return c_ok(cre) && c_ok(cim) && s_ok(re0) && s_ok(im0);
 }
 
-template <typename T, int M, bool CYC>
+template <typename T, int M, bool CYC, bool PRE = false>
 __device__ __forceinline__ uint32_t orbit_scaled_run(uint32_t iterations, T &X, T &Y, T &A, T &B, T c2re, T c2im,
                                                      T squared, T skip_t, EpisodeCtl ctl, uint32_t &completed,
                                                      T *pXs = nullptr, T *pYs = nullptr,
                                                      uint32_t *saved_index = nullptr, uint32_t spec_quiet = 0u,
-                                                     uint32_t spec_maxlen = 0u) {
+                                                     uint32_t spec_maxlen = 0u, typename UBits<T>::type lim4_pre = 0,
+                                                     typename UBits<T>::type t4_pre = 0) {
     uint32_t it;
     T t, q;
     T X1, Y1, A1, B1;
     uint32_t sspec;
-    uint32_t specq = __builtin_amdgcn_readfirstlane(spec_quiet ? spec_quiet : 0xFFFFFFFFu);
-    uint32_t lcap = __builtin_amdgcn_readfirstlane(spec_maxlen);
+    uint32_t specq = spec_quiet ? spec_quiet : 0xFFFFFFFFu;
+    uint32_t lcap = spec_maxlen;
+    if constexpr (!PRE) specq = __builtin_amdgcn_readfirstlane(specq), lcap = __builtin_amdgcn_readfirstlane(lcap);
     T Xs = CYC ? *pXs : T(0), Ys = CYC ? *pYs : T(0);
     uint32_t vsaved = 0xFFFFFFFFu;
     uint32_t snext = 32u;
     unsigned long long sorig, sprev, sdiff, scyc;
     uint32_t si, stmp, nrem, scnt;
-    const uint32_t n = __builtin_amdgcn_readfirstlane(iterations);
+    const uint32_t n = PRE ? iterations : __builtin_amdgcn_readfirstlane(iterations);
     const uint32_t thr = __builtin_amdgcn_readfirstlane(ctl.thr), minrun = __builtin_amdgcn_readfirstlane(ctl.minrun);
     const T lim4_v = (T)4 * squared, t4_v = (T)4 * skip_t;
 #define FR_SC_OUTPUTS                                                                                           \
@@ -462,7 +464,7 @@
     : FR_SC_OUTPUTS, [scyc] "=&s"(scyc), [Xs] "+v"(Xs), [Ys] "+v"(Ys), [vsaved] "+v"(vsaved), [snext] "+s"(snext) \
     : FR_SC_INPUTS                                                                                              \
     : "vcc", "scc"
-    const auto lim4 = uniform_bits<T>(lim4_v), t4lim = uniform_bits<T>(t4_v);
+    const auto lim4 = PRE ? lim4_pre : uniform_bits<T>(lim4_v), t4lim = PRE ? t4_pre : uniform_bits<T>(t4_v);
     if constexpr (sizeof(T) == 8) {
         if constexpr (M == 4 && CYC)
             asm volatile(FR_SC_ASM_M4_CYC("f64", "v_cmp_eq_u64", "v_mov_b64") FR_SC_OPERANDS_CYC);
@@ -494,13 +496,15 @@
     return it;
 }
 
-template <typename T, int M>
+template <typename T, int M, bool PRE = false>
 __device__ __forceinline__ uint32_t orbit_scaled(uint32_t iterations, T &re, T &im, T cre, T cim, T squared,
-                                                 T skip_t, T &r2, T &i2, uint32_t spec_quiet = 0u, uint32_t spec_maxlen = 0u) {
+                                                 T skip_t, T &r2, T &i2, uint32_t spec_quiet = 0u, uint32_t spec_maxlen = 0u,
+                                                 typename UBits<T>::type lim4_pre = 0, typename UBits<T>::type t4_pre = 0) {
     T X = re + re, Y = im + im, A = X * X, B = Y * Y;
     uint32_t completed;
-    const uint32_t it = orbit_scaled_run<T, M, false>(iterations, X, Y, A, B, cre + cre, cim + cim, squared, skip_t,
-                                               EpisodeCtl{0, 0}, completed, nullptr, nullptr, nullptr, spec_quiet, spec_maxlen);
+    const uint32_t it = orbit_scaled_run<T, M, false, PRE>(iterations, X, Y, A, B, cre + cre, cim + cim, squared, skip_t,
+                                               EpisodeCtl{0, 0}, completed, nullptr, nullptr, nullptr, spec_quiet, spec_maxlen,
+                                               lim4_pre, t4_pre);
     re = X * (T)0.5;
     im = Y * (T)0.5;
     r2 = re * re;
@@ -508,10 +512,16 @@
     return it;
 }
 
-template <typename T>
+template <typename T, bool PLAIN = false>
 __device__ __forceinline__ uint32_t orbit_auto(uint32_t loop_mode, uint32_t iterations, T &re, T &im, T cre, T cim,
                                                T squared, T skip_t, T &r2, T &i2, int strip_scalable = -1,
-                                               uint32_t spec_quiet = 0u, uint32_t spec_maxlen = 0u) {
+                                               uint32_t spec_quiet = 0u, uint32_t spec_maxlen = 0u,
+                                               typename UBits<T>::type lim4_pre = 0, typename UBits<T>::type t4_pre = 0) {
+    if constexpr (PLAIN) {
+        if (strip_scalable != 0)
+            return orbit_scaled<T, 4, true>(iterations, re, im, cre, cim, squared, skip_t, r2, i2, spec_quiet, spec_maxlen, lim4_pre, t4_pre);
+        return orbit<T>(iterations, re, im, cre, cim, squared, r2, i2, spec_quiet);
+    }
     if (loop_mode != 0 && strip_scalable != 0) {
         bool all_ok = strip_scalable == 1;
         if (strip_scalable < 0) all_ok = __ballot(!lane_is_scalable<T>(re, im, cre, cim)) == 0ull;
@@ -587,8 +597,69 @@
 };
 
 template <typename T>
+struct PlainTile {
+    typename UBits<T>::type lim4, t4;
+    unsigned long long valid;
+    double *tab;
+    bool *staged;
+};
+
+template <typename T, bool PLAIN = false>
 __device__ __forceinline__ uint32_t colour_packed(bool valid, bool fast_colour, T re, T im, T r2, T i2, uint32_t iters,
-                                                  const double *lds_tab, const uint32_t *palette) {
+                                                  const double *lds_tab, const uint32_t *palette,
+                                                  unsigned long long vmask = 0ull, double *stage_tab = nullptr, bool *staged = nullptr) {
+    if constexpr (PLAIN) {
+        Filter32 f;
+        {
+            FR_COLD_PARAMS(kp);
+            f.lo = kp->filt_lo32, f.k = kp->filt_k32, f.c = kp->filt_c32;
+            f.p0 = kp->prim32[0], f.p1 = kp->prim32[2], f.p2 = kp->prim32[1];
+        }
+        float d32;
+        if constexpr (sizeof(T) == 8)
+            d32 = (float)(r2 + i2);
+        else
+            d32 = r2 + i2;
+        uint32_t packed = 0;
+        unsigned long long todo = vmask;
+        const unsigned long long outside = vmask & ballot64(d32 >= f.lo);
+        if (outside != 0ull) {
+            uint32_t pk;
+            const bool decided = colour_fast32(f, d32, (float)(iters + 1u), pk);
+            todo &= ~(outside & ballot64(d32 <= 0x1.ffffep119f) & ballot64(decided));
+            packed = pk;
+        }
+        if (todo != 0ull) {
+            double dist;
+            if constexpr (sizeof(T) == 8) {
+                dist = (double)(r2 + i2);
+            } else {
+                const double zre = (double)re, zim = (double)im;
+                dist = zre * zre + zim * zim;
+            }
+            FR_COLD_PARAMS(kp);
+            const unsigned long long in_set = todo & ballot64(!(dist > kp->stable_limit));
+            if (lane_in(in_set))
+                packed = kp->inside ? sat_u8_dev(kp->sec_f[0] * dist) | (sat_u8_dev(kp->sec_f[2] * dist) << 8) | (sat_u8_dev(kp->sec_f[1] * dist) << 16) : 0u;
+            todo &= ~in_set;
+        }
+        if (todo != 0ull) {
+            if (!*staged) {
+                const double *gt = &g_log2_tab[0][0];
+                for (uint32_t k = threadIdx.x; k < FR_LOG2_N * 3; k += 64) stage_tab[k] = gt[k];
+                __syncthreads();
+                *staged = true;
+            }
+            if (lane_in(todo)) {
+                FR_COLD_PARAMS(kp);
+                const ColourConsts cc = make_colour_consts(*kp);
+                uint8_t rgb[3];
+                colour_pixel<T>(cc, re, im, r2, i2, iters, stage_tab, nullptr, rgb);
+                packed = (uint32_t)rgb[0] | ((uint32_t)rgb[1] << 8) | ((uint32_t)rgb[2] << 16);
+            }
+        }
+        return packed;
+    }
     uint32_t packed = 0;
     unsigned long long todo = ballot64(valid);
     if (fast_colour) {
@@ -641,11 +712,45 @@
     return packed;
 }
 
-template <typename T, int MODE>
+template <typename T, int MODE, bool PLAIN = false, bool FULL = false>
 __device__ __forceinline__ void render_pixel(const fr_kparams &p, const fr_kout &out, const double *s_tab,
                                              const uint32_t *s_pal, double sre, double sim, bool valid,
                                              uint32_t cx, uint32_t r, uint32_t lane, uint32_t r_out,
-                                             int strip_scalable = -1, const TileOut *to = nullptr) {
+                                             int strip_scalable = -1, const TileOut *to = nullptr,
+                                             const PlainTile<T> *pt = nullptr) {
+    if constexpr (PLAIN) {
+        static_assert(MODE == FR_OUT_RGB, "the plain instance renders packed r,g,b");
+        T tre = (T)sre, tim = (T)sim, tr2, ti2;
+        T cre = tre, cim = tim;
+        asm("" : "+v"(cre));
+        asm("" : "+v"(cim));
+        uint32_t iters;
+        auto run = [&]() {
+            T squared;
+            if constexpr (sizeof(T) == 8) {
+                squared = p.limit * p.limit;
+            } else {
+                const float lim = (float)p.limit;
+                squared = lim * lim;
+            }
+            iters = orbit_auto<T, true>(4u, p.iterations, tre, tim, cre, cim, squared, (T)p.skip_t, tr2, ti2, strip_scalable,
+                                        p.loop_spec, p.loop_spec_max, pt->lim4, pt->t4);
+        };
+        if constexpr (FULL) {
+            run();
+        } else {
+            tr2 = tre, ti2 = tim, iters = 0;
+            if (lane_in(pt->valid)) run();
+        }
+        const uint32_t packed = colour_packed<T, true>(true, true, tre, tim, tr2, ti2, iters, nullptr, nullptr,
+                                                       FULL ? ~0ull : pt->valid, pt->tab, pt->staged);
+        if constexpr (FULL) {
+            store_packed(to->base, to->lane_off, packed, 3u);
+        } else {
+            if (lane_in(pt->valid)) store_packed(to->base, to->lane_off, packed, 3u);
+        }
+        return;
+    }
     double zre = 0.0, zim = 0.0;
     T tre = 0, tim = 0, tr2 = 0, ti2 = 0;
     uint32_t iters = 0;
@@ -775,60 +880,18 @@
 
 template <typename T, int MODE, int kStripTiles>
 __global__ __launch_bounds__(64) void escape_strip_kernel(const fr_kparams p, const fr_kout out) {
+    constexpr bool PLAIN = false;
+    const fr_kplain pc{};
     __shared__ double s_tab[(FR_LOG2_N * 3 * 8 > FR_MAX_PALETTE_ENTRIES * 4 ? FR_LOG2_N * 3 * 8 : FR_MAX_PALETTE_ENTRIES * 4) / 8];
-    const uint32_t tid = threadIdx.x;
-    const uint32_t *s_pal = nullptr;
-    if (MODE == FR_OUT_RGB) {
-        if (p.palette != nullptr) {
-            uint32_t *dst = reinterpret_cast<uint32_t *>(s_tab);
-            for (uint32_t k = tid; k < p.palette_entries; k += 64) dst[k] = p.palette[k];
-            s_pal = dst;
-        } else if (p.smooth) {
-            const double *gt = &g_log2_tab[0][0];
-            for (uint32_t k = tid; k < FR_LOG2_N * 3; k += 64) s_tab[k] = gt[k];
-        }
-        __syncthreads();
-    }
-    const uint32_t lane = tid;
-    const uint32_t row0 = (blockIdx.y + gridDim.y * blockIdx.z) * 8u;
-    if (row0 >= p.nrows) return;
-    const uint32_t lx = lane & 7u, ly = lane >> 3;
-    const uint32_t r = row0 + ly;
-    const double width = (double)p.width, height = (double)p.height;
-
-    static_assert(kStripTiles <= 7, "lanes 56-63 are the row lanes");
-    const bool row_lane = lane >= 56;
-    const uint32_t tile0 = blockIdx.x * kStripTiles;
-    uint32_t coord_u;
-    if (row_lane) {
-        const uint32_t rr = row0 + (lane - 56);
-        coord_u = p.y_first + (rr / p.block_rows) * p.y_stride + rr % p.block_rows;
-    } else {
-        coord_u = p.x_first + (tile0 * 8u + lane) * p.x_stride;
-    }
-    const double coord_lane = coord_to_space((double)coord_u, height, row_lane ? 0.5 : (width / height) / 2.0,
-                                             row_lane ? p.pos_im : p.pos_re, row_lane ? p.scale_im : p.scale_re);
-    const double sim = __shfl(coord_lane, 56 + ly, 64);
-    uint32_t out_row0 = row0;
-    if (p.out_in_place) out_row0 = p.y_first + (row0 / p.block_rows) * p.y_stride + row0 % p.block_rows;
-    const uint32_t r_out = out_row0 + ly;
-    const int strip_scalable = (p.loop_mode != 0 && strip_is_scalable<T>(p, coord_lane, tile0, row0, lane)) ? 1 : 0;
-    TileOut to;
-    to.bpp = p.out_rgba ? 4u : 3u;
-    to.narrow = (uint64_t)p.ncols * to.bpp * 8u <= 0xFFFFFFFFull;
-    to.lane_off = ly * (p.ncols * to.bpp) + lx * to.bpp;
-    to.fast_colour = p.colour_filter32 && p.smooth && p.palette == nullptr;
-    uint8_t *const strip_base = MODE == FR_OUT_RGB ? out.rgb + ((uint64_t)out_row0 * p.ncols + (uint64_t)tile0 * 8u) * to.bpp : nullptr;
-
-    for (int k = 0; k < kStripTiles; k++) {
-        const uint32_t col0 = (tile0 + k) * 8u;
-        if (col0 >= p.ncols) break;
-        const double sre = __shfl(coord_lane, k * 8 + lx, 64);
-        const uint32_t cx = col0 + lx;
-        const bool valid = cx < p.ncols && r < p.nrows;
-        to.base = strip_base + (size_t)((uint32_t)k * 8u * to.bpp);
-        render_pixel<T, MODE>(p, out, s_tab, s_pal, sre, sim, valid, cx, r, lane, r_out, strip_scalable, MODE == FR_OUT_RGB ? &to : nullptr);
-    }
+#include "fr_strip_body.inc"
+}
+
+template <typename T, int kStripTiles>
+__global__ __launch_bounds__(64) void escape_strip_plain_kernel(const fr_kparams p, const fr_kout out, const fr_kplain pc) {
+    constexpr bool PLAIN = true;
+    constexpr int MODE = FR_OUT_RGB;
+    __shared__ double s_tab[FR_LOG2_N * 3];
+#include "fr_strip_body.inc"
 }
 
 __device__ __forceinline__ uint32_t wave_max_u32(uint32_t v) {
@@ -2658,8 +2721,24 @@
     return (p.strip_tiles == 4 && !v1) ? launch_first_pass<T, 4>(p, out, stream, false) : launch_first_pass<T, 7>(p, out, stream, v1);
 }
 
+template <typename T>
+fr_kplain plain_consts(const fr_kparams &p) {
+    fr_kplain pc{};
+    if constexpr (sizeof(T) == 8) {
+        pc.lim4_bits = fr_bits_of(4.0 * (p.limit * p.limit));
+        pc.t4_bits = fr_bits_of(4.0 * p.skip_t);
+    } else {
+        const float lim = (float)p.limit;
+        pc.lim4_bits = __builtin_bit_cast(uint32_t, 4.0f * (lim * lim));
+        pc.t4_bits = __builtin_bit_cast(uint32_t, 4.0f * (float)p.skip_t);
+    }
+    pc.half_aspect = ((double)p.width / (double)p.height) / 2.0;
+    pc.full_ok = (p.out_in_place && (p.block_rows % 8u) != 0) ? 0u : 1u;
+    return pc;
+}
+
 template <typename T, int kStripTiles>
-hipError_t launch_strips(const fr_kparams &p, int mode, const fr_kout &out, hipStream_t stream) {
+hipError_t launch_strips(const fr_kparams &p, int mode, const fr_kout &out, hipStream_t stream, bool plain = false) {
     if (p.ncols == 0 || p.nrows == 0) return hipSuccess;
     const uint64_t gx = ((uint64_t)p.ncols + 8 * kStripTiles - 1) / (8 * kStripTiles);
     const uint64_t row_tiles = ((uint64_t)p.nrows + 7) / 8;
@@ -2667,6 +2746,14 @@
     const uint64_t gz = (row_tiles + gy - 1) / gy;
     if (gx > 0x7FFFFFFFull || gz > 65535) return hipErrorInvalidConfiguration;
     dim3 grid((uint32_t)gx, (uint32_t)gy, (uint32_t)gz), block(64);
+    if constexpr (kStripTiles == 7 || kStripTiles == 1) {
+        if (plain) {
+            if (mode != FR_OUT_RGB) return hipErrorInvalidValue;
+            hipLaunchKernelGGL((escape_strip_plain_kernel<T, kStripTiles>), grid, block, 0, stream, p, out, plain_consts<T>(p));
+            return hipGetLastError();
+        }
+    }
+    if (plain) return hipErrorInvalidValue;
 #define FR_K(MODE) escape_strip_kernel<T, MODE, kStripTiles>
     FR_LAUNCH_BY_MODE(FR_K);
 #undef FR_K
@@ -3101,24 +3188,24 @@
 }
 
 template <typename T>
-static hipError_t launch_strips_len(const fr_kparams &p, int mode, int strip_tiles, const fr_kout &out, hipStream_t stream) {
+static hipError_t launch_strips_len(const fr_kparams &p, int mode, int strip_tiles, const fr_kout &out, hipStream_t stream, bool plain) {
     switch (strip_tiles) {
     case 7:
-        return launch_strips<T, 7>(p, mode, out, stream);
+        return launch_strips<T, 7>(p, mode, out, stream, plain);
     case 4:
-        return launch_strips<T, 4>(p, mode, out, stream);
+        return launch_strips<T, 4>(p, mode, out, stream, plain);
     case 2:
-        return launch_strips<T, 2>(p, mode, out, stream);
+        return launch_strips<T, 2>(p, mode, out, stream, plain);
     case 1:
-        return launch_strips<T, 1>(p, mode, out, stream);
+        return launch_strips<T, 1>(p, mode, out, stream, plain);
     default:
         return hipErrorInvalidValue;
     }
 }
 
-hipError_t fr_launch_strips(const fr_kparams &p, int precision, int mode, int strip_tiles, const fr_kout &out, hipStream_t stream) {
-    return precision == 1 ? launch_strips_len<float>(p, mode, strip_tiles, out, stream)
-                          : launch_strips_len<double>(p, mode, strip_tiles, out, stream);
+hipError_t fr_launch_strips(const fr_kparams &p, int precision, int mode, int strip_tiles, const fr_kout &out, hipStream_t stream, bool plain) {
+    return precision == 1 ? launch_strips_len<float>(p, mode, strip_tiles, out, stream, plain)
+                          : launch_strips_len<double>(p, mode, strip_tiles, out, stream, plain);
 }
 
 hipError_t fr_launch_refill(const fr_kparams &p, int precision, int mode, const fr_kout &out, hipStream_t stream) {
diff --git a/fractal-renderer_amd/csrc/fr_launch.h b/fractal-renderer_amd/csrc/fr_launch.h
--- a/fractal-renderer_amd/csrc/fr_launch.h
+++ b/fractal-renderer_amd/csrc/fr_launch.h
@@ -4,7 +4,8 @@
 #include "fr_kernels.h"
 
 hipError_t fr_launch_tile(const fr_kparams &p, int precision, int mode, int tile, const fr_kout &out, hipStream_t stream);
-hipError_t fr_launch_strips(const fr_kparams &p, int precision, int mode, int strip_tiles, const fr_kout &out, hipStream_t stream);
+hipError_t fr_launch_strips(const fr_kparams &p, int precision, int mode, int strip_tiles, const fr_kout &out, hipStream_t stream,
+                            bool plain = false);
 hipError_t fr_launch_refill(const fr_kparams &p, int precision, int mode, const fr_kout &out, hipStream_t stream);
 
 hipError_t fr_launch_first_pass(const fr_kparams &p, int precision, bool v1, const fr_kout &out, hipStream_t stream);
diff --git a/fractal-renderer_amd/csrc/fr_strip_body.inc b/fractal-renderer_amd/csrc/fr_strip_body.inc
--- /dev/null
+++ b/fractal-renderer_amd/csrc/fr_strip_body.inc
@@ -0,0 +1,85 @@
+    const uint32_t tid = threadIdx.x;
+    const uint32_t *s_pal = nullptr;
+    if (MODE == FR_OUT_RGB && !PLAIN) {
+        if (p.palette != nullptr) {
+            uint32_t *dst = reinterpret_cast<uint32_t *>(s_tab);
+            for (uint32_t k = tid; k < p.palette_entries; k += 64) dst[k] = p.palette[k];
+            s_pal = dst;
+        } else if (p.smooth) {
+            const double *gt = &g_log2_tab[0][0];
+            for (uint32_t k = tid; k < FR_LOG2_N * 3; k += 64) s_tab[k] = gt[k];
+        }
+        __syncthreads();
+    }
+    const uint32_t lane = tid;
+    const uint32_t row0 = (blockIdx.y + gridDim.y * blockIdx.z) * 8u;
+    if (row0 >= p.nrows) return;
+    const uint32_t lx = lane & 7u, ly = lane >> 3;
+    const uint32_t r = row0 + ly;
+    const double width = (double)p.width, height = (double)p.height;
+
+    static_assert(kStripTiles <= 7, "lanes 56-63 are the row lanes");
+    const bool row_lane = lane >= 56;
+    const uint32_t tile0 = blockIdx.x * kStripTiles;
+    uint32_t coord_u;
+    if (row_lane) {
+        const uint32_t rr = row0 + (lane - 56);
+        coord_u = p.y_first + (rr / p.block_rows) * p.y_stride + rr % p.block_rows;
+    } else {
+        coord_u = p.x_first + (tile0 * 8u + lane) * p.x_stride;
+    }
+    const double coord_lane = coord_to_space((double)coord_u, height, row_lane ? 0.5 : PLAIN ? pc.half_aspect : (width / height) / 2.0,
+                                             row_lane ? p.pos_im : p.pos_re, row_lane ? p.scale_im : p.scale_re);
+    const double sim = __shfl(coord_lane, 56 + ly, 64);
+    uint32_t out_row0 = row0;
+    if (p.out_in_place) out_row0 = p.y_first + (row0 / p.block_rows) * p.y_stride + row0 % p.block_rows;
+    const uint32_t r_out = out_row0 + ly;
+    if constexpr (PLAIN) {
+        constexpr T lo = ScalableRange<T>::lo, hi = ScalableRange<T>::hi;
+        const T av = __builtin_fabs((T)coord_lane);
+        const unsigned long long relevant = (ballot64(tile0 * 8u + lane < p.ncols) & 0x00FFFFFFFFFFFFFFull) |
+                                            (ballot64(row0 + (lane - 56) < p.nrows) & 0xFF00000000000000ull);
+        const int strip_scalable = (relevant & (ballot64(!(av >= lo)) | ballot64(!(av <= hi)))) == 0ull ? 1 : 0;
+        TileOut to;
+        to.bpp = 3u, to.narrow = true, to.fast_colour = true;
+        to.lane_off = ly * (p.ncols * 3u) + lx * 3u;
+        uint8_t *const strip_base = out.rgb + ((uint64_t)out_row0 * p.ncols + (uint64_t)tile0 * 8u) * 3u;
+        bool staged = false;
+        PlainTile<T> pt;
+        pt.lim4 = (typename UBits<T>::type)pc.lim4_bits, pt.t4 = (typename UBits<T>::type)pc.t4_bits;
+        pt.valid = ~0ull, pt.tab = s_tab, pt.staged = &staged;
+        if (pc.full_ok && strip_scalable && (tile0 + kStripTiles) * 8u <= p.ncols && row0 + 8u <= p.nrows) {
+            for (int k = 0; k < kStripTiles; k++) {
+                const double sre = __shfl(coord_lane, k * 8 + lx, 64);
+                to.base = strip_base + (size_t)((uint32_t)k * 24u);
+                render_pixel<T, MODE, true, true>(p, out, nullptr, nullptr, sre, sim, true, 0u, r, lane, r_out, 1, &to, &pt);
+            }
+        } else {
+            for (int k = 0; k < kStripTiles; k++) {
+                const uint32_t col0 = (tile0 + k) * 8u;
+                if (col0 >= p.ncols) break;
+                const double sre = __shfl(coord_lane, k * 8 + lx, 64);
+                pt.valid = ballot64(col0 + lx < p.ncols) & ballot64(r < p.nrows);
+                to.base = strip_base + (size_t)((uint32_t)k * 24u);
+                render_pixel<T, MODE, true, false>(p, out, nullptr, nullptr, sre, sim, true, 0u, r, lane, r_out, strip_scalable, &to, &pt);
+            }
+        }
+    } else {
+        const int strip_scalable = (p.loop_mode != 0 && strip_is_scalable<T>(p, coord_lane, tile0, row0, lane)) ? 1 : 0;
+        TileOut to;
+        to.bpp = p.out_rgba ? 4u : 3u;
+        to.narrow = (uint64_t)p.ncols * to.bpp * 8u <= 0xFFFFFFFFull;
+        to.lane_off = ly * (p.ncols * to.bpp) + lx * to.bpp;
+        to.fast_colour = p.colour_filter32 && p.smooth && p.palette == nullptr;
+        uint8_t *const strip_base = MODE == FR_OUT_RGB ? out.rgb + ((uint64_t)out_row0 * p.ncols + (uint64_t)tile0 * 8u) * to.bpp : nullptr;
+
+        for (int k = 0; k < kStripTiles; k++) {
+            const uint32_t col0 = (tile0 + k) * 8u;
+            if (col0 >= p.ncols) break;
+            const double sre = __shfl(coord_lane, k * 8 + lx, 64);
+            const uint32_t cx = col0 + lx;
+            const bool valid = cx < p.ncols && r < p.nrows;
+            to.base = strip_base + (size_t)((uint32_t)k * 8u * to.bpp);
+            render_pixel<T, MODE>(p, out, s_tab, s_pal, sre, sim, valid, cx, r, lane, r_out, strip_scalable, MODE == FR_OUT_RGB ? &to : nullptr);
+        }
+    }
diff --git a/include/fractal_hip.h b/include/fractal_hip.h
--- a/include/fractal_hip.h
+++ b/include/fractal_hip.h
@@ -330,6 +330,8 @@
 int fr_debug_loop_plan(const fr_config *cfg, int precision, uint32_t *loop_mode, double *skip_t, uint32_t *spec_quiet);
 int fr_debug_set_spec_maxlen(uint32_t maxlen);
 int fr_debug_spec_maxlen(const fr_config *cfg, int precision, uint32_t *maxlen);
+int fr_debug_set_strip_plain(int on);
+int fr_debug_strip_plain(const fr_config *cfg, int precision, int channels, int *plain);
 
 int fr_debug_math(int which, const double *in, double *out, size_t n);
 int fr_debug_set_queue_trace(void *d_trace);
```

Result: faster. 5527 billion, median of 6 (+1.5%).
